# phylo42/IPK

Hardware: AMD Instinct MI355X
Metric: scored phylo-k-mers/sec (higher is better)
Workload: dtype f32

## Files before the change

ipk_amd/csrc/ipkgpu.hip:

```cpp
#include <cstring>
#include <hip/hip_runtime.h>
#include <rocprim/rocprim.hpp>

#include <algorithm>
#include <cmath>
#include <cstdarg>
#include <cstdio>
#include <cstring>
#include <new>
#include <string>
#include <type_traits>
#include <unordered_map>
#include <memory>
#include <vector>

#include "../../include/ipkgpu.h"
#include "dcla_device.hpp"
#include "kernels_score.hpp"
#include "kernels_quad.hpp"
#include "kernels_compact.hpp"
#include "kernels_keymajor.hpp"
#include "kernels_reduce_pipe.hpp"
#include "kernels_filter.hpp"
#include "kernels_dbfile.hpp"
// ... 393 lines not shown
    ctx->pend.sw.reset();
    for (hipEvent_t e : ctx->events.free_ev) (void)hipEventDestroy(e);
    ctx->events.free_ev.clear();
    if (ctx->h_rb) (void)hipHostFree(ctx->h_rb);
    if (ctx->up_done) (void)hipEventDestroy(ctx->up_done);
    (void)hipStreamDestroy(ctx->stream);
    delete ctx;
}

int ipkgpu_set_option(ipkgpu_ctx* ctx, const char* name, int64_t value)
{
    if (!ctx || !name) return IPKGPU_ERR_INVALID;
    if (!strcmp(name, "workspace_bytes")) {
        if (value <= 0) return fail(ctx, IPKGPU_ERR_INVALID, "workspace_bytes must be positive");
        ctx->workspace_bytes = value;
        return IPKGPU_OK;
    }
    if (!strcmp(name, "device_budget_bytes")) {
        if (value < 0) return fail(ctx, IPKGPU_ERR_INVALID, "device_budget_bytes must not be negative (0 = no budget)");
        ctx->budget = value;
        return IPKGPU_OK;
    }
    if (!strcmp(name, "release_workspaces")) {
        HIP_TRY(ctx, hipSetDevice(ctx->device));
        HIP_TRY(ctx, hipStreamSynchronize(ctx->stream));
        ctx->up_pending = false;
        for (DevBuf* b : all_workspaces(ctx)) if (b->p) { (void)dev_free(ctx, b->p, b->cap); b->p = nullptr; b->cap = 0; }
        drop_cache(ctx);
        ctx->mask_valid = false; ctx->pend.active = false; ctx->pend.sw.reset();
        return IPKGPU_OK;
    }
    if (!strcmp(name, "slice_long_lists")) {
        if (value != 0 && value != 1) return fail(ctx, IPKGPU_ERR_INVALID, "slice_long_lists is 0 or 1");
        ctx->opt_slice = value;
        return IPKGPU_OK;
    }
    if (!strcmp(name, "variant")) { ctx->opt_variant = value; return IPKGPU_OK; }
    if (!strcmp(name, "debug_flags")) { ctx->opt_flags = value; return IPKGPU_OK; }
    if (!strcmp(name, "debug_pool_chunks")) { ctx->opt_pool_chunks = value; return IPKGPU_OK; }
    if (!strcmp(name, "debug_pool_limit_bytes")) { ctx->opt_pool_limit = value; return IPKGPU_OK; }
    if (!strcmp(name, "debug_wg_chunks2")) { ctx->opt_wg_chunks2 = value; return IPKGPU_OK; }
    if (!strcmp(name, "debug_rounds")) { ctx->opt_rounds = value; return IPKGPU_OK; }
    if (!strcmp(name, "debug_kmc_pass")) { ctx->opt_kmc_pass = value; return IPKGPU_OK; }
    if (!strcmp(name, "debug_prefix_mats")) { ctx->opt_prefix_mats = value; return IPKGPU_OK; }
    return fail(ctx, IPKGPU_ERR_INVALID, "unknown option '%s'", name);
}

}

namespace {

constexpr int TW = 128;
constexpr int NW = 8;

#ifndef IPK_QCAP
#define IPK_QCAP 160
#endif
#ifndef IPK_AACAP
#define IPK_AACAP 512
#endif
#ifndef IPK_QCAP12
#define IPK_QCAP12 384
#endif
#ifndef IPK_QNW12
#define IPK_QNW12 4
#endif
#ifndef IPK_QTW12
#define IPK_QTW12 32
#endif
template <int SIGMA, int K> constexpr int fast_cap()
{
    if (SIGMA == 4) return K <= 10 ? IPK_QCAP : IPK_QCAP12;
    return IPK_AACAP;
}

template <int SIGMA, int K, bool POS = false>
int launch_score(ipkgpu_ctx* ctx, const ScoreParams& p)
{
    constexpr int CAP = fast_cap<SIGMA, K>();
    constexpr size_t lds = TileGeo<SIGMA, K, TW>::HEAD_BYTES + (size_t)NW * wave_scratch_entries<SIGMA, K, CAP>() * 8;
    static_assert(lds <= 160 * 1024, "fast-path LDS budget");
    auto kern = score_tiles_kernel<SIGMA, K, CAP, TW, NW, POS>;
    if (lds > 64 * 1024)
        HIP_TRY(ctx, hipFuncSetAttribute(reinterpret_cast<const void*>(kern), hipFuncAttributeMaxDynamicSharedMemorySize, (int)lds));
    const uint64_t blocks = (uint64_t)p.n_batch_mats * p.tiles_per_mat;
    if (blocks > 0x7fffffffull) return fail(ctx, IPKGPU_ERR_INVALID, "batch too large for one launch");
    hipLaunchKernelGGL(kern, dim3((uint32_t)blocks), dim3(NW * 64), lds, ctx->stream, p);
    HIP_TRY(ctx, hipGetLastError());
    return IPKGPU_OK;
}

template <int SIGMA, int K, bool POS = false>
int launch_overflow(ipkgpu_ctx* ctx, const ScoreParams& p)
{
    if constexpr (Geo<SIGMA, K, 1 << 30>::DIRECT || ipow(SIGMA, K - K / 2) <= (uint32_t)fast_cap<SIGMA, K>()) {
        (void)ctx; (void)p;
        return IPKGPU_OK;
    } else {
        constexpr size_t lds = TileGeo<SIGMA, K, 1>::HEAD_BYTES + (size_t)wave_scratch_entries<SIGMA, K, big_capf<SIGMA, K>()>() * 8;
        static_assert(lds <= 160 * 1024, "big-list LDS budget");
        auto kern = score_overflow_kernel<SIGMA, K, POS>;
        if (lds > 64 * 1024)
            HIP_TRY(ctx, hipFuncSetAttribute(reinterpret_cast<const void*>(kern), hipFuncAttributeMaxDynamicSharedMemorySize, (int)lds));
        const uint32_t per_cu = (uint32_t)std::max<size_t>(1, std::min<size_t>(32 / OVF_NW, (160 * 1024) / (lds + 64)));
        hipLaunchKernelGGL(kern, dim3(ctx->num_cu * per_cu), dim3(OVF_NW * 64), lds, ctx->stream, p);
        HIP_TRY(ctx, hipGetLastError());
        return IPKGPU_OK;
    }
}

template <int SIGMA, int K, bool POS>
int launch_both(ipkgpu_ctx* ctx, const ScoreParams& p)
{
    RC_TRY((launch_score<SIGMA, K, POS>(ctx, p)));
    return launch_overflow<SIGMA, K, POS>(ctx, p);
}


template <int SIGMA, int K> constexpr uint32_t stream_tbl()
{
    constexpr uint64_t T = ipow(SIGMA, K);
    if (Geo<SIGMA, K, 1 << 30>::DIRECT) return 0;
    if (SIGMA == 4 && K >= 13) return 0;
    if (SIGMA == 4) return T <= 16384 ? (uint32_t)T : (K <= 10 ? 16384u : 32768u);
    if (K <= 3) return (uint32_t)T;
    if (K <= 5) return 32000u;
    return 0;
}

template <int SIGMA, int K> constexpr int stream_nw() { return NW; }
template <int SIGMA, int K> constexpr int stream_tw() { return TW; }

template <int SIGMA, int K>
int launch_stream_pass1(ipkgpu_ctx* ctx, const StreamParams& sp, uint32_t n_wg)
{
    constexpr uint32_t TBL = stream_tbl<SIGMA, K>();
    if constexpr (TBL == 0) { (void)sp; (void)n_wg; return fail(ctx, IPKGPU_ERR_INVALID, "stream variant unsupported for this sigma/k"); }
    else {
        constexpr int CAP = fast_cap<SIGMA, K>();
        constexpr uint32_t T = ipow(SIGMA, K);
        constexpr uint32_t NB = (T + TBL - 1) / TBL;
        constexpr int SNW = stream_nw<SIGMA, K>(), STW = stream_tw<SIGMA, K>();
        constexpr size_t lds = TileGeo<SIGMA, K, STW>::HEAD_BYTES + (size_t)SNW * stream_wave_scratch<SIGMA, K, CAP>() * 8 + (size_t)SNW * 2 * NB * SUB * 4;
        static_assert(lds <= 160 * 1024, "stream pass-1 LDS budget");
        auto kern = score_stream_kernel<SIGMA, K, CAP, STW, SNW, TBL>;
        if (lds > 64 * 1024)
            HIP_TRY(ctx, hipFuncSetAttribute(reinterpret_cast<const void*>(kern), hipFuncAttributeMaxDynamicSharedMemorySize, (int)lds));
        hipLaunchKernelGGL(kern, dim3(n_wg), dim3(SNW * 64), lds, ctx->stream, sp);
        HIP_TRY(ctx, hipGetLastError());
        return IPKGPU_OK;
    }
}

template <int SIGMA, int K>
int launch_stream_overflow(ipkgpu_ctx* ctx, const StreamParams& sp)
{
    constexpr uint32_t TBL = stream_tbl<SIGMA, K>();
    if constexpr (TBL == 0 || ipow(SIGMA, K - K / 2) <= (uint32_t)fast_cap<SIGMA, K>()) {
        (void)ctx; (void)sp;
        return IPKGPU_OK;
    } else {
        constexpr uint32_t NB = (uint32_t)((ipow(SIGMA, K) + TBL - 1) / TBL);
        constexpr size_t lds = TileGeo<SIGMA, K, 1>::HEAD_BYTES + (size_t)wave_scratch_entries<SIGMA, K, big_capf<SIGMA, K>()>() * 8 +
                               (size_t)OVF_NW * 2 * NB * SUB * 4;
        static_assert(lds + 64 <= 160 * 1024, "big-list (stream) LDS budget");
        auto kern = score_overflow_stream_kernel<SIGMA, K, TBL>;
        if (lds > 64 * 1024)
            HIP_TRY(ctx, hipFuncSetAttribute(reinterpret_cast<const void*>(kern), hipFuncAttributeMaxDynamicSharedMemorySize, (int)lds));
        const uint32_t per_cu = (uint32_t)std::max<size_t>(1, std::min<size_t>(32 / OVF_NW, (160 * 1024) / (lds + 64)));
        hipLaunchKernelGGL(kern, dim3(ctx->num_cu * per_cu), dim3(OVF_NW * 64), lds, ctx->stream, sp);
        HIP_TRY(ctx, hipGetLastError());
        return IPKGPU_OK;
    }
}

#ifndef IPK_RPIPE_DEFAULT
#define IPK_RPIPE_DEFAULT 1
#endif
#ifndef IPK_RPIPE_D
#define IPK_RPIPE_D 2
#endif
template <int SIGMA, int K>
int launch_stream_pass2(ipkgpu_ctx* ctx, uint32_t n_gb, uint64_t T, uint32_t* table, bool compress)
{
    constexpr uint32_t TBL = stream_tbl<SIGMA, K>();
    if constexpr (TBL == 0) { (void)n_gb; (void)T; (void)table; (void)compress; return fail(ctx, IPKGPU_ERR_INVALID, "stream variant unsupported"); }
    else {
        constexpr uint32_t NB = (uint32_t)((ipow(SIGMA, K) + TBL - 1) / TBL);
        constexpr int NT = TBL <= 16384 ? 512 : 1024;
        const size_t lds = compress ? (size_t)comp_padded_slots<TBL, NT>() * 4 + (NT / 64 + 1) * 4 : (size_t)TBL * 4;
        auto launch = [&](auto kern) -> int {
            if (lds > 64 * 1024)
                HIP_TRY(ctx, hipFuncSetAttribute(reinterpret_cast<const void*>(kern), hipFuncAttributeMaxDynamicSharedMemorySize, (int)lds));
            hipLaunchKernelGGL(kern, dim3(n_gb), dim3(NT), lds, ctx->stream, ctx->pool.as<uint2>(),
                               ctx->gboff.as<uint64_t>(), ctx->clist.as<uint2>(), NB, T, table, ctx->mask.as<uint32_t>(), ctx->mask_words,
                               ctx->cvals.as<uint2>(), ctx->coff.as<uint64_t>(), ctx->rank.as<uint32_t>(), ctx->vaddr.as<uint64_t>(), ctx->ucnt.as<uint32_t>());
            HIP_TRY(ctx, hipGetLastError());
            return IPKGPU_OK;
        };
        if constexpr (TBL * 4 > 80 * 1024) {
            if (compress && ((IPK_RPIPE_DEFAULT != 0) != ((ctx->opt_flags & 2048) != 0))) {
                constexpr int PD = IPK_RPIPE_D;
                auto kern = reduce_buckets_pipe_kernel<TBL, NT, PD>;
                HIP_TRY(ctx, hipFuncSetAttribute(reinterpret_cast<const void*>(kern), hipFuncAttributeMaxDynamicSharedMemorySize, (int)lds));
                hipLaunchKernelGGL(kern, dim3(std::min<uint32_t>(n_gb, (uint32_t)ctx->num_cu)), dim3(NT), lds, ctx->stream, ctx->pool.as<uint2>(),
                                   ctx->gboff.as<uint64_t>(), ctx->clist.as<uint2>(), n_gb, NB, T, ctx->mask.as<uint32_t>(), ctx->mask_words,
                                   ctx->cvals.as<uint2>(), ctx->coff.as<uint64_t>(), ctx->rank.as<uint32_t>(), ctx->vaddr.as<uint64_t>(), ctx->ucnt.as<uint32_t>());
                HIP_TRY(ctx, hipGetLastError());
                return IPKGPU_OK;
            }
        }
        return compress ? launch(reduce_buckets_kernel<TBL, NT, true>) : launch(reduce_buckets_kernel<TBL, NT, false>);
    }
}

template <int SIGMA, int K> size_t stream_lds() {
    constexpr uint32_t TBL = stream_tbl<SIGMA, K>();
    if constexpr (TBL == 0) return 0;
    else {
        constexpr int CAP = fast_cap<SIGMA, K>();
        constexpr uint32_t NB = (uint32_t)((ipow(SIGMA, K) + TBL - 1) / TBL);
        return TileGeo<SIGMA, K, stream_tw<SIGMA, K>()>::HEAD_BYTES + (size_t)stream_nw<SIGMA, K>() * stream_wave_scratch<SIGMA, K, CAP>() * 8 +
               (size_t)stream_nw<SIGMA, K>() * 2 * NB * SUB * 4;
    }
}
template <int SIGMA, int K> uint32_t stream_nb() {
    constexpr uint32_t TBL = stream_tbl<SIGMA, K>();
    if constexpr (TBL == 0) return 0; else return (uint32_t)((ipow(SIGMA, K) + TBL - 1) / TBL);
}

template <int SIGMA, int K> constexpr bool quad_ok() { return QuadGeo<SIGMA, K>::OK && stream_tbl<SIGMA, K>() != 0; }
#ifndef IPK_QNW
#define IPK_QNW 4
#endif
#ifndef IPK_QTW
#define IPK_QTW 40
#endif
template <int SIGMA, int K> constexpr int quad_nw() { return K <= 10 ? IPK_QNW : IPK_QNW12; }
template <int SIGMA, int K> constexpr int quad_tw() { return K <= 10 ? IPK_QTW : IPK_QTW12; }
#ifndef IPK_QROWLANE12
#define IPK_QROWLANE12 1
#endif
#ifndef IPK_QROWLANE
#define IPK_QROWLANE 0
#endif
template <int SIGMA, int K> constexpr bool quad_rowlane() { return K <= 10 ? IPK_QROWLANE != 0 : IPK_QROWLANE12 != 0; }
#ifndef IPK_QONEWIN12
#define IPK_QONEWIN12 1
#endif
template <int SIGMA, int K> constexpr bool quad_onewin() { return K >= 11 && IPK_QONEWIN12 != 0 && quad_rowlane<SIGMA, K>(); }
template <int SIGMA, int K> size_t quad_lds()
{
    if constexpr (!quad_ok<SIGMA, K>()) return 0;
    else {
        constexpr int CAP = fast_cap<SIGMA, K>();
        constexpr uint32_t TBL = stream_tbl<SIGMA, K>();
        constexpr uint32_t NB = (uint32_t)((ipow(SIGMA, K) + TBL - 1) / TBL);
        return QuadTile<SIGMA, K, quad_tw<SIGMA, K>()>::HEAD_BYTES + (size_t)quad_nw<SIGMA, K>() * quad_wave_entries<SIGMA, K, CAP, quad_onewin<SIGMA, K>()>() * 8 +
               (size_t)quad_nw<SIGMA, K>() * NB * 8;
    }
}
template <int SIGMA, int K, bool COUNT_ONLY = false>
int launch_quad_pass1(ipkgpu_ctx* ctx, const StreamParams& sp, uint32_t n_wg)
{
    if constexpr (!quad_ok<SIGMA, K>()) { (void)sp; (void)n_wg; return fail(ctx, IPKGPU_ERR_INVALID, "quad kernel unsupported for this sigma/k"); }
    else {
        constexpr int CAP = fast_cap<SIGMA, K>();
        constexpr uint32_t TBL = stream_tbl<SIGMA, K>();
        constexpr int QNW = quad_nw<SIGMA, K>(), QTW = quad_tw<SIGMA, K>();
        const size_t lds = quad_lds<SIGMA, K>();
        auto kern = score_quad_kernel<SIGMA, K, CAP, QTW, QNW, TBL, COUNT_ONLY, quad_rowlane<SIGMA, K>(), quad_onewin<SIGMA, K>()>;
        if (lds > 64 * 1024)
            HIP_TRY(ctx, hipFuncSetAttribute(reinterpret_cast<const void*>(kern), hipFuncAttributeMaxDynamicSharedMemorySize, (int)lds));
        hipLaunchKernelGGL(kern, dim3(n_wg), dim3(QNW * 64), lds, ctx->stream, sp);
        HIP_TRY(ctx, hipGetLastError());
        return IPKGPU_OK;
    }
}

#ifndef IPK_XPNW
#define IPK_XPNW 11
#endif
#ifndef IPK_XPTW
#define IPK_XPTW 128
#endif
constexpr int XP_TW = IPK_XPTW;
template <int SIGMA, int K> constexpr int xp_nw() { return SIGMA == 20 ? IPK_XPNW : 11; }
template <int SIGMA, int K> constexpr uint32_t xp_tbl()
{
    if (SIGMA == 20 && K == 6) return 16000u;
    if (SIGMA == 4 && K >= 13) return 32768u;
    return stream_tbl<SIGMA, K>();
}
template <int SIGMA, int K, int KK = K> uint32_t xp_nb() {
    constexpr uint32_t TBL = xp_tbl<SIGMA, K>();
    if constexpr (TBL == 0) return 0; else return (uint32_t)((ipow(SIGMA, KK) + TBL - 1) / TBL);
}
template <int SIGMA, int K, int KK = K> size_t xp_lds() {
    constexpr uint32_t TBL = xp_tbl<SIGMA, K>();
    if constexpr (TBL == 0) return 0;
    else {
        constexpr int CAP = fast_cap<SIGMA, K>();
        constexpr uint32_t NB = (uint32_t)((ipow(SIGMA, KK) + TBL - 1) / TBL);
        return TileGeo<SIGMA, K, XP_TW>::HEAD_BYTES + (size_t)xp_nw<SIGMA, K>() * stream_wave_scratch<SIGMA, K, CAP>() * 8 + (size_t)NB * 4;
    }
}
template <int SIGMA, int K, bool WRITE, int KK = K, bool POS = false>
int launch_xp(ipkgpu_ctx* ctx, const XpParams& xp, uint32_t n_wg)
{
    constexpr uint32_t TBL = xp_tbl<SIGMA, K>();
    if constexpr (TBL == 0) { (void)xp; (void)n_wg; return fail(ctx, IPKGPU_ERR_INVALID, "exact-partition variant unsupported for this sigma/k"); }
    else {
        constexpr int CAP = fast_cap<SIGMA, K>();
        constexpr uint32_t NB = (uint32_t)((ipow(SIGMA, KK) + TBL - 1) / TBL);
        constexpr size_t lds = TileGeo<SIGMA, K, XP_TW>::HEAD_BYTES + (size_t)xp_nw<SIGMA, K>() * stream_wave_scratch<SIGMA, K, CAP>() * 8 + (size_t)NB * 4;
        static_assert(lds <= 160 * 1024, "exact-partition LDS budget");
        static_assert((TileGeo<SIGMA, K, XP_TW>::HEAD_BYTES + (size_t)xp_nw<SIGMA, K>() * stream_wave_scratch<SIGMA, K, CAP>() * 8) % 8 == 0, "cursor alignment");
        auto kern = score_xp_kernel<SIGMA, K, CAP, XP_TW, xp_nw<SIGMA, K>(), TBL, WRITE, KK, POS>;
        if (lds > 64 * 1024)
            HIP_TRY(ctx, hipFuncSetAttribute(reinterpret_cast<const void*>(kern), hipFuncAttributeMaxDynamicSharedMemorySize, (int)lds));
        hipLaunchKernelGGL(kern, dim3(n_wg), dim3(xp_nw<SIGMA, K>() * 64), lds, ctx->stream, xp);
        HIP_TRY(ctx, hipGetLastError());
        return IPKGPU_OK;
    }
}
template <int SIGMA, int K, bool WRITE, int KK = K, bool POS = false>
int launch_xp_overflow(ipkgpu_ctx* ctx, const XpParams& xp)
{
    constexpr uint32_t TBL = xp_tbl<SIGMA, K>();
    if constexpr (TBL == 0 || ipow(SIGMA, K - K / 2) <= (uint32_t)fast_cap<SIGMA, K>()) {
        (void)ctx; (void)xp;
        return IPKGPU_OK;
    } else {
        constexpr size_t lds = TileGeo<SIGMA, K, 1>::HEAD_BYTES + (size_t)wave_scratch_entries<SIGMA, K, big_capf<SIGMA, K>()>() * 8;
        static_assert(lds + 64 <= 160 * 1024, "big-list (exact partition) LDS budget");
        auto kern = score_overflow_xp_kernel<SIGMA, K, TBL, WRITE, KK, POS>;
        if (lds > 64 * 1024)
            HIP_TRY(ctx, hipFuncSetAttribute(reinterpret_cast<const void*>(kern), hipFuncAttributeMaxDynamicSharedMemorySize, (int)lds));
        const uint32_t per_cu = (uint32_t)std::max<size_t>(1, std::min<size_t>(32 / OVF_NW, (160 * 1024) / (lds + 64)));
        hipLaunchKernelGGL(kern, dim3(ctx->num_cu * per_cu), dim3(OVF_NW * 64), lds, ctx->stream, xp);
        HIP_TRY(ctx, hipGetLastError());
        return IPKGPU_OK;
    }
}
template <int SIGMA, int K, bool COMPRESS, int KK = K>
int launch_xp_reduce(ipkgpu_ctx* ctx, uint32_t n_gb, uint32_t S, uint64_t T, const uint64_t* off, uint32_t* table)
{
    constexpr uint32_t TBL = xp_tbl<SIGMA, K>();
    if constexpr (TBL == 0) { (void)n_gb; (void)S; (void)T; (void)off; (void)table; return fail(ctx, IPKGPU_ERR_INVALID, "exact-partition variant unsupported"); }
    else {
        constexpr uint32_t NB = (uint32_t)((ipow(SIGMA, KK) + TBL - 1) / TBL);
        static_assert(!COMPRESS || NB == 1 || TBL % 64 == 0, "a 64-slot block must not straddle two buckets");
        constexpr int NT = TBL <= 16384 ? 512 : 1024;
        constexpr size_t lds = COMPRESS ? (size_t)comp_padded_slots<TBL, NT>() * 4 + (NT / 64 + 1) * 4 : (size_t)TBL * 4;
        auto kern = reduce_ranges_kernel<TBL, NT, COMPRESS>;
        if (lds > 64 * 1024)
            HIP_TRY(ctx, hipFuncSetAttribute(reinterpret_cast<const void*>(kern), hipFuncAttributeMaxDynamicSharedMemorySize, (int)lds));
        hipLaunchKernelGGL(kern, dim3(n_gb), dim3(NT), lds, ctx->stream, ctx->pool.as<uint2>(), off, S, NB, T, table,
                           ctx->mask.as<uint32_t>(), ctx->mask_words, ctx->rank.as<uint32_t>(), ctx->vaddr.as<uint64_t>(), ctx->ucnt.as<uint32_t>());
        HIP_TRY(ctx, hipGetLastError());
        return IPKGPU_OK;
    }
}
template <int SIGMA, int K>
int launch_xp_reduce_pos(ipkgpu_ctx* ctx, uint32_t n_gb, uint32_t S, uint64_t T, const uint64_t* off, uint32_t nwin)
{
    constexpr uint32_t TBL = xp_tbl<SIGMA, K>();
    if constexpr (TBL == 0) { (void)n_gb; (void)S; (void)T; (void)off; (void)nwin; return fail(ctx, IPKGPU_ERR_INVALID, "exact-partition variant unsupported"); }
    else {
        constexpr uint32_t NB = (uint32_t)((ipow(SIGMA, K) + TBL - 1) / TBL);
        static_assert(NB == 1 || TBL % 64 == 0, "a 64-slot block must not straddle two buckets");
        constexpr int NT = pos_sub_slots<TBL>() <= 4096 ? 256 : 1024;
        constexpr size_t lds = (size_t)pos_sub_blocks<TBL>() * 64 * 8 + (pos_sub_blocks<TBL>() + 1) * 4;
        static_assert(lds <= 160 * 1024, "positions reduce LDS budget");
        auto kern = reduce_ranges_pos_kernel<TBL, NT>;
        if (lds > 64 * 1024)
            HIP_TRY(ctx, hipFuncSetAttribute(reinterpret_cast<const void*>(kern), hipFuncAttributeMaxDynamicSharedMemorySize, (int)lds));
        hipLaunchKernelGGL(kern, dim3(n_gb), dim3(NT), lds, ctx->stream, ctx->pool.as<uint2>(), ctx->seq.as<uint32_t>(), off, S, NB, T, nwin,
                           ctx->mask_words, ctx->pvals.as<uint32_t>(), ctx->pvaddr.as<uint64_t>());
        HIP_TRY(ctx, hipGetLastError());
        return IPKGPU_OK;
    }
}
template <int V> using int_c = std::integral_constant<int, V>;

template <int SIGMA, int K, int KMAX, class F> int with_k(ipkgpu_ctx* ctx, uint32_t k, F& f)
{
    if (k == (uint32_t)K) return f(int_c<SIGMA>{}, int_c<K>{});
    if constexpr (K < KMAX) return with_k<SIGMA, K + 1, KMAX>(ctx, k, f);
    else return fail(ctx, IPKGPU_ERR_INVALID, "unsupported sigma/k (%u/%u)", (uint32_t)SIGMA, k);
}
template <class F> int with_sigma_k(ipkgpu_ctx* ctx, uint32_t sigma, uint32_t k, F&& f)
{
    if (sigma == 4) return with_k<4, 2, 14>(ctx, k, f);
    if (sigma == 20) return with_k<20, 2, 6>(ctx, k, f);
    return fail(ctx, IPKGPU_ERR_INVALID, "unsupported sigma/k (%u/%u)", sigma, k);
}

bool keyrange_supported(uint32_t sigma, uint32_t k, uint32_t lead)
{
    return sigma == 4 && lead >= 1 && k > lead && k - lead >= 13 && k - lead <= 14 && k <= 16;
}
template <class F> int with_xp_shape(ipkgpu_ctx* ctx, uint32_t sigma, uint32_t k, uint32_t lead, F&& f)
{
    if (!lead) return with_sigma_k(ctx, sigma, k, [&](auto S_, auto K_) { return f(S_, K_, K_); });
    if (sigma == 4) {
        switch (k * 8 + lead) {
            case 14 * 8 + 1: return f(int_c<4>{}, int_c<14>{}, int_c<13>{});
            case 15 * 8 + 1: return f(int_c<4>{}, int_c<15>{}, int_c<14>{});
            case 15 * 8 + 2: return f(int_c<4>{}, int_c<15>{}, int_c<13>{});
            case 16 * 8 + 2: return f(int_c<4>{}, int_c<16>{}, int_c<14>{});
            case 16 * 8 + 3: return f(int_c<4>{}, int_c<16>{}, int_c<13>{});
        }
    }
    return fail(ctx, IPKGPU_ERR_INVALID, "unsupported key range");
}

struct Geometry {
    uint32_t fast_cap = 0;
    uint32_t stream_nb = 0, stream_tbl = 0;
    uint32_t stream_nw = NW, stream_tw = TW;
    size_t stream_lds = 0;
    bool quad = false;
    uint32_t quad_nw = NW, quad_tw = TW;
    size_t quad_lds = 0;
    uint32_t xp_nb = 0, xp_tbl = 0;
    size_t xp_lds = 0;
};

int fill_geometry(ipkgpu_ctx* ctx, uint32_t sigma, uint32_t k, uint32_t lead, Geometry& g)
{
    if (!lead)
        RC_TRY(with_sigma_k(ctx, sigma, k, [&](auto S_, auto K_) {
            g.fast_cap = fast_cap<S_, K_>();
            g.stream_nb = stream_nb<S_, K_>(); g.stream_tbl = stream_tbl<S_, K_>();
            g.stream_nw = stream_nw<S_, K_>(); g.stream_tw = stream_tw<S_, K_>(); g.stream_lds = stream_lds<S_, K_>();
            g.quad = quad_ok<S_, K_>();
            g.quad_nw = quad_nw<S_, K_>(); g.quad_tw = quad_tw<S_, K_>(); g.quad_lds = quad_lds<S_, K_>();
            return IPKGPU_OK;
        }));
    return with_xp_shape(ctx, sigma, k, lead, [&](auto S_, auto K_, auto KK_) {
        g.xp_nb = xp_nb<S_, K_, KK_>(); g.xp_tbl = xp_tbl<S_, K_>(); g.xp_lds = xp_lds<S_, K_, KK_>();
        return IPKGPU_OK;
    });
}

#ifndef IPK_KMC_RUNS_DEFAULT
#define IPK_KMC_RUNS_DEFAULT 1
#endif
#ifndef IPK_KMC_PASS
#define IPK_KMC_PASS 256
#endif
#define KM_LAUNCH(KERN, CAPV, ...)                                                                                        \
    do {                                                                                                                  \
        if (P == 1) hipLaunchKernelGGL((KERN<true, CAPV>), dim3((uint32_t)(per_xcd * 8)), dim3(256), 0, ctx->stream, __VA_ARGS__); \
        else hipLaunchKernelGGL((KERN<false, CAPV>), dim3((uint32_t)(per_xcd * 8)), dim3(256), 0, ctx->stream, __VA_ARGS__);     \
    } while (0)

CompTable comp_table(const ipkgpu_ctx* ctx)
{
    CompTable ct;
    ct.mask = ctx->mask.as<uint32_t>(); ct.rank = ctx->rank.as<uint32_t>(); ct.vaddr = ctx->vaddr.as<uint64_t>();
    ct.pool = ctx->comp_own_vals ? ctx->cvals.as<uint2>() : ctx->pool.as<uint2>();
    ct.off = ctx->comp_own_vals ? ctx->coff.as<uint64_t>() : ctx->gboff.as<uint64_t>(); ct.mask_words = ctx->mask_words;
    ct.NB = ctx->comp_nb; ct.stride = ctx->comp_stride; ct.TBL = ctx->comp_tbl;
    return ct;
}

}

namespace {

constexpr int IPKGPU_RETRY_SMALLER = 100;
constexpr int IPKGPU_RETRY_AGAIN = 101;
#ifndef IPK_OVF_POOL_RATIO
#define IPK_OVF_POOL_RATIO 500
#endif

enum class PassKind { tiles, stream, quad, xp };
struct Pass {
    PassKind kind = PassKind::tiles;
    bool positions = false;
    bool compress = false;
    bool seq = false;
    double slot_bytes() const { return positions ? 8.0 : kind == PassKind::xp && compress ? 0.3125 : 4.0; }
};

Pass choose_pass(int64_t variant, uint32_t sigma, uint32_t lead, bool positions, bool km_positions, const Geometry& g)
{
    Pass ps;
    ps.positions = positions;
    if (positions) return ps;
    if (km_positions) { ps.kind = PassKind::xp; ps.compress = true; ps.seq = true; return ps; }
    const int64_t v = variant;
    if (g.xp_nb != 0 && (v == 3 || v == 4 || (v == 0 && g.stream_nb == 0) || lead != 0)) {
        ps.kind = PassKind::xp;
        ps.compress = v != 3;
    } else if (g.stream_nb != 0 && g.stream_nb <= 2048 && (v == 0 || v == 2 || v == 5 || v == 6 || v == 7)) {
        ps.kind = v != 2 && g.quad ? PassKind::quad : PassKind::stream;
        ps.compress = v == 6 || (v == 0 && g.stream_tbl == 32768u && sigma == 4);
    }
    return ps;
}

struct Plan {
    uint32_t n_mats = 0, sites = 0, sigma = 0, k = 0;
    float eps = 0;
    std::vector<uint32_t> group_ids;
    std::vector<uint32_t> slot_of;
    uint32_t n_groups = 0, nwin = 0, tiles_per_mat = 0, chunks_per_group = 0;
    uint64_t table_size = 0, gpb = 1;
    uint32_t lead = 0, lead_c = 0;
    Geometry geo;
    Pass pass;
    const uint32_t* mat_rank = nullptr;
};

int make_plan(ipkgpu_ctx* ctx, const void* logp, uint32_t n_mats, uint32_t sites, uint32_t sigma,
              const uint32_t* mat_group, uint32_t k, float log_eps, Plan& pl, uint32_t lead = 0, uint32_t lead_c = 0,
              bool positions = false, bool km_positions = false)
{
    if (!logp || !mat_group) return fail(ctx, IPKGPU_ERR_INVALID, "null input pointer");
    if (sigma != 4 && sigma != 20) return fail(ctx, IPKGPU_ERR_INVALID, "unsupported alphabet size %u (4 or 20)", sigma);
    if (lead == 0 && (k < 2 || k > ipkgpu_max_k(sigma)))
        return fail(ctx, IPKGPU_ERR_INVALID, "k=%u out of range [2, %u] for sigma=%u", k, ipkgpu_max_k(sigma), sigma);
    if (lead != 0 && !keyrange_supported(sigma, k, lead))
        return fail(ctx, IPKGPU_ERR_INVALID, "no key-range pass of k=%u with %u leading symbols for sigma=%u", k, lead, sigma);
    pl.lead = lead; pl.lead_c = lead_c;
    if (n_mats == 0) return fail(ctx, IPKGPU_ERR_INVALID, "no matrices");
    if (sites < k) return fail(ctx, IPKGPU_ERR_INVALID, "alignment has %u sites, fewer than k=%u", sites, k);
    pl.n_mats = n_mats; pl.sites = sites; pl.sigma = sigma; pl.k = k; pl.eps = log_eps;
    RC_TRY(fill_geometry(ctx, sigma, k, lead, pl.geo));
    if (km_positions && (lead != 0 || pl.geo.xp_nb == 0))
        return fail(ctx, IPKGPU_ERR_INVALID, "no positioned database for sigma=%u k=%u: the call takes the exact partition, which needs more than 64 keys "
                                             "and no key-range pass", sigma, k);
    pl.pass = choose_pass(ctx->opt_variant, sigma, lead, positions, km_positions, pl.geo);
    pl.slot_of.resize(n_mats);
    std::unordered_map<uint32_t, uint32_t> index;
    index.reserve(n_mats);
    for (uint32_t i = 0; i < n_mats; ++i) {
        auto it = index.find(mat_group[i]);
        if (it == index.end()) {
            it = index.emplace(mat_group[i], (uint32_t)pl.group_ids.size()).first;
            pl.group_ids.push_back(mat_group[i]);
        }
        pl.slot_of[i] = it->second;
    }
    pl.n_groups = (uint32_t)pl.group_ids.size();
    pl.table_size = ipow(sigma, (int)(k - lead));
    pl.chunks_per_group = (uint32_t)((pl.table_size + CHUNK - 1) / CHUNK);
    pl.nwin = sites - k + 1;
    {
        const double ppw = ctx->pairs_per_window > 0 ? ctx->pairs_per_window : 256.0;
        const double pool_per_group = (double)n_mats / (double)pl.n_groups * (double)pl.nwin * ppw * (pl.pass.seq ? 16.0 : 8.0) * 1.25;
        const double per_group = (double)pl.table_size * pl.pass.slot_bytes() + pool_per_group;
        pl.gpb = std::max<uint64_t>(1, (uint64_t)((double)ctx->workspace_bytes / per_group));
    }
    pl.gpb = std::min<uint64_t>(pl.gpb, pl.n_groups);
    while (pl.gpb > 1 && pl.gpb * pl.chunks_per_group > 0x7fffffffull) pl.gpb /= 2;
    pl.tiles_per_mat = (pl.nwin + TW - 1) / TW;
    return IPKGPU_OK;
}

int run_prefix(ipkgpu_ctx* ctx, const Plan& pl, const float* logp_dev)
{
    RC_TRY(ensure(ctx, ctx->best, (size_t)pl.n_mats * (pl.sites + 1) * 4));
    HIP_TRY(ctx, hipMemsetAsync(ctx->small, 0, SMALL_BYTES, ctx->stream));
    uint32_t M = 1;
    while (M < 8 && (pl.n_mats + M - 1) / M > (uint32_t)ctx->num_cu * 4) M *= 2;
    if (ctx->opt_prefix_mats == 1 || ctx->opt_prefix_mats == 2 || ctx->opt_prefix_mats == 4 || ctx->opt_prefix_mats == 8) M = (uint32_t)ctx->opt_prefix_mats;
    const dim3 grid((pl.n_mats + M - 1) / M);
#define IPK_PREFIX(SG, MM) hipLaunchKernelGGL((prefix_max_kernel<SG, MM>), grid, dim3(256), 0, ctx->stream, logp_dev, pl.n_mats, pl.sites, ctx->best.as<float>())
    if (pl.sigma == 4) { if (M == 1) IPK_PREFIX(4, 1); else if (M == 2) IPK_PREFIX(4, 2); else if (M == 4) IPK_PREFIX(4, 4); else IPK_PREFIX(4, 8); }
    else { if (M == 1) IPK_PREFIX(20, 1); else if (M == 2) IPK_PREFIX(20, 2); else if (M == 4) IPK_PREFIX(20, 4); else IPK_PREFIX(20, 8); }
#undef IPK_PREFIX
    HIP_TRY(ctx, hipGetLastError());
    return IPKGPU_OK;
}

int scan_u32(ipkgpu_ctx* ctx, const uint32_t* in, uint64_t n, uint64_t* out);

int score_batch_xp(ipkgpu_ctx* ctx, const Plan& pl, const float* logp_dev, uint32_t gb, ScoreParams& p)
{
    const uint32_t XNB = pl.geo.xp_nb;
    const bool compress = pl.pass.compress;
    const uint32_t tiles_per_mat = (pl.nwin + XP_TW - 1) / XP_TW;
    const size_t lds_bytes = pl.geo.xp_lds;
    const uint64_t wg_per_cu = std::max<uint64_t>(1, std::min<uint64_t>(32 / (pl.sigma == 20 ? IPK_XPNW : 11), (160 * 1024) / std::max<size_t>(lds_bytes, 1)));
    const uint64_t slots = (uint64_t)ctx->num_cu * wg_per_cu;
    const uint32_t S = (uint32_t)std::max<uint64_t>(1, std::min<uint64_t>((slots * 4) / gb, tiles_per_mat));
    const uint64_t n_gb = (uint64_t)gb * XNB;
    const uint32_t stride = S + 1;
    const uint64_t n_units = n_gb * stride;
    if (n_gb > 0x7fffffffull || (uint64_t)gb * S > 0x7fffffffull) return fail(ctx, IPKGPU_ERR_INVALID, "batch too large for one launch");
    RC_TRY(ensure(ctx, ctx->gbcnt, n_units * 4));
    RC_TRY(ensure(ctx, ctx->gboff, (n_units + 1) * 8));
    RC_TRY(ensure(ctx, ctx->gbcur, n_gb * 4));
    HIP_TRY(ctx, hipMemsetAsync(ctx->gbcnt.p, 0, n_units * 4, ctx->stream));
    HIP_TRY(ctx, hipMemsetAsync(ctx->gbcur.p, 0, n_gb * 4, ctx->stream));

    XpParams xp;
    StreamParams& sp = xp.s;
    sp.logp = logp_dev; sp.best = ctx->best.as<float>();
    sp.gm_off = ctx->gm.as<uint32_t>(); sp.gm_list = ctx->gm.as<uint32_t>() + gb + 1;
    sp.sites = pl.sites; sp.nwin = pl.nwin; sp.tiles_per_mat = tiles_per_mat; sp.S = S;
    sp.eps = pl.eps;
    sp.pool = nullptr; sp.pool_cap = 0; sp.pool_next = nullptr; sp.desc = nullptr; sp.pool_ovf = nullptr; sp.pre_chunks = 0;
    sp.emitted = p.emitted; sp.ovf_queue = p.ovf_queue; sp.ovf_count = p.ovf_count; sp.mat_slot = p.mat_slot; sp.big_ovf = p.big_ovf;
    sp.slice_lists = p.slice_lists;
    sp.flags = (uint32_t)(ctx->opt_flags) & 4u;
    xp.cnt = ctx->gbcnt.as<uint32_t>();
    xp.off = ctx->gboff.as<uint64_t>();
    xp.stride = stride;
    xp.ovcur = ctx->gbcur.as<uint32_t>();
    xp.start = nullptr;
    xp.lead_c = pl.lead_c;

    const bool seq = pl.pass.seq;
    auto xp_kernel = [&](bool write) {
        if (write && seq)
            return with_sigma_k(ctx, pl.sigma, pl.k, [&](auto S_, auto K_) { return launch_xp<S_, K_, true, K_, true>(ctx, xp, gb * S); });
        return with_xp_shape(ctx, pl.sigma, pl.k, pl.lead, [&](auto S_, auto K_, auto KK_) {
            return write ? launch_xp<S_, K_, true, KK_>(ctx, xp, gb * S) : launch_xp<S_, K_, false, KK_>(ctx, xp, gb * S);
        });
    };
    auto xp_overflow = [&](bool write) {
        if (write && seq)
            return with_sigma_k(ctx, pl.sigma, pl.k, [&](auto S_, auto K_) { return launch_xp_overflow<S_, K_, true, K_, true>(ctx, xp); });
        return with_xp_shape(ctx, pl.sigma, pl.k, pl.lead, [&](auto S_, auto K_, auto KK_) {
            return write ? launch_xp_overflow<S_, K_, true, KK_>(ctx, xp) : launch_xp_overflow<S_, K_, false, KK_>(ctx, xp);
        });
    };
    Stopwatch sw(ctx->stream, &ctx->events);
    const int ev_a = sw.mark();
    RC_TRY(xp_kernel(false));
    const int ev_a2 = sw.mark();
    RC_TRY(xp_overflow(false));
    RC_TRY(scan_u32(ctx, xp.cnt, n_units, ctx->gboff.as<uint64_t>()));
    uint64_t total = 0;
    HIP_TRY(ctx, hipMemcpyAsync(&total, ctx->gboff.as<uint64_t>() + n_units, 8, hipMemcpyDeviceToHost, ctx->stream));
    HIP_TRY(ctx, hipStreamSynchronize(ctx->stream));
    {
        const size_t free_b = mem_free_bytes(ctx);
        const bool over_limit = ctx->opt_pool_limit > 0 && total * 8 > (uint64_t)ctx->opt_pool_limit;
        const uint64_t side = seq ? total * 8 + 512 : 0;
        const uint64_t side_have = seq ? ctx->seq.cap + ctx->pvals.cap : 0;
        if (over_limit || (total * 8 > ctx->pool.cap && total * 8 > free_b + ctx->pool.cap) ||
            (side > side_have && total * 8 + side > free_b + ctx->pool.cap + side_have)) {
            if (gb > 1) return IPKGPU_RETRY_SMALLER;
            return fail(ctx, IPKGPU_ERR_NOMEM, "the pair pool of ONE branch group (%llu pairs) does not fit device memory", (unsigned long long)total);
        }
    }
// ... 47 lines not shown
    ctx->acc_main_ms += sw.ms(ev_a, ev_a2) + sw.ms(ev_c, ev_d0);
    ctx->acc_count_ms += sw.ms(ev_a, ev_a2); ctx->acc_write_ms += sw.ms(ev_c, ev_d0);
    ctx->acc_reduce_ms += sw.ms(ev_d, ev_e);
    ctx->main_kernel = "score_xp_kernel";
    return IPKGPU_OK;
}

int stream_batch_check(ipkgpu_ctx* ctx)
{
    ipkgpu_ctx::Pending& pd = ctx->pend;
    if (!pd.active) return IPKGPU_OK;
    pd.active = false;
    std::unique_ptr<Stopwatch> sw(pd.sw.release());
    const uint32_t n_ovf = ctx->h_rb[SMALL_OVF_COUNT / 4], pool_exhausted = ctx->h_rb[SMALL_POOL_OVF / 4];
    if (pool_exhausted) {
        if (pd.cap >= pd.max_chunks) {
            ctx->pool_want_min = 0;
            if (pd.gb > 1) return IPKGPU_RETRY_SMALLER;
            return fail(ctx, IPKGPU_ERR_NOMEM, "the pair pool of ONE branch group is exhausted at the device-memory limit");
        }
        ctx->pool_want_min = pd.cap * 2;
        return IPKGPU_RETRY_AGAIN;
    }
    ctx->pool_want_min = 0;
    memcpy(&ctx->emitted_host, ctx->h_rb + SMALL_EMITTED / 4, 8);
    ctx->emitted_fetched = true;
    ctx->spec_skip_wait = !(n_ovf > 0 && (uint64_t)n_ovf * IPK_OVF_POOL_RATIO >= pd.windows && pd.pool_ovf_ok);
    if (sw) { ctx->acc_main_ms += sw->ms(pd.ev_a, pd.ev_b); ctx->acc_reduce_ms += sw->ms(pd.ev_c, pd.ev_d); }
    return IPKGPU_OK;
}

int arm_capped(ipkgpu_ctx* ctx, uint32_t sigma, uint32_t k, ScoreParams& p)
{
    static_assert(SMALL_SLICED + 4 == SMALL_BIG_OVF, "the count and the flag are cleared and read together");
    const bool capped_lists = sigma == 4 && k >= 13;
    p.big_ovf = capped_lists ? small_at(ctx, SMALL_BIG_OVF) : nullptr;
    p.slice_lists = capped_lists && ctx->opt_slice ? 1u : 0u;
    if (capped_lists) HIP_TRY(ctx, hipMemsetAsync(p.big_ovf - 1, 0, 8, ctx->stream));
    return IPKGPU_OK;
}

int check_capped(ipkgpu_ctx* ctx, uint32_t k, const ScoreParams& p)
{
    if (!p.big_ovf) return IPKGPU_OK;
    uint32_t word[2] = {0, 0};
    HIP_TRY(ctx, hipMemcpyAsync(word, p.big_ovf - 1, 8, hipMemcpyDeviceToHost, ctx->stream));
    HIP_TRY(ctx, hipStreamSynchronize(ctx->stream));
    ctx->sliced_windows += word[0];
    const uint32_t hit = word[1];
    if (hit) return fail(ctx, IPKGPU_ERR_INVALID, "a window's half list exceeds %d entries: beyond the capacity of this engine at k = %u "
                                                  "(the lists of k >= 13 are capped; lower omega's reach or k)", BIG_CAP_ENTRIES, k);
    return IPKGPU_OK;
}

int score_batch_impl(ipkgpu_ctx* ctx, const Plan& pl, const float* logp_dev, uint32_t g0, uint32_t gb, bool defer)
{
    const uint32_t n_mats = pl.n_mats;
    uint32_t nb = 0;
    for (uint32_t i = 0; i < n_mats; ++i) nb += (pl.slot_of[i] >= g0 && pl.slot_of[i] < g0 + gb);
    const size_t gm_words = (size_t)gb + 1 + nb;
    void* stage = nullptr;
    RC_TRY(upload_stage(ctx, ((size_t)n_mats * 2 + gm_words) * 4, &stage));
    uint32_t* mat_list_h = reinterpret_cast<uint32_t*>(stage);
    uint32_t* mat_slot_h = mat_list_h + n_mats;
    uint32_t* gm = mat_slot_h + n_mats;
    nb = 0;
    for (uint32_t i = 0; i < n_mats; ++i) {
        mat_slot_h[i] = 0;
        if (pl.slot_of[i] >= g0 && pl.slot_of[i] < g0 + gb) { mat_list_h[nb++] = i; mat_slot_h[i] = pl.slot_of[i] - g0; }
    }
    for (uint32_t i = nb; i < n_mats; ++i) mat_list_h[i] = 0;
    for (size_t i = 0; i < gm_words; ++i) gm[i] = 0;
    for (uint32_t i = 0; i < n_mats; ++i)
        if (pl.slot_of[i] >= g0 && pl.slot_of[i] < g0 + gb) gm[pl.slot_of[i] - g0 + 1]++;
    for (uint32_t g = 0; g < gb; ++g) gm[g + 1] += gm[g];
    {
        std::vector<uint32_t> cur(gm, gm + gb);
        for (uint32_t i = 0; i < n_mats; ++i)
            if (pl.slot_of[i] >= g0 && pl.slot_of[i] < g0 + gb) gm[(size_t)gb + 1 + cur[pl.slot_of[i] - g0]++] = i;
    }
    RC_TRY(ensure(ctx, ctx->idx, (size_t)n_mats * 8));
    RC_TRY(ensure(ctx, ctx->ovfq, (size_t)nb * pl.nwin * 8));
    RC_TRY(ensure(ctx, ctx->gm, gm_words * 4));
    HIP_TRY(ctx, hipMemcpyAsync(ctx->idx.p, mat_list_h, (size_t)n_mats * 8, hipMemcpyHostToDevice, ctx->stream));
    HIP_TRY(ctx, hipMemcpyAsync(ctx->gm.p, gm, gm_words * 4, hipMemcpyHostToDevice, ctx->stream));
    RC_TRY(upload_staged(ctx));

    const Pass& ps = pl.pass;
    ScoreParams p;
    p.logp = logp_dev;
    p.best = ctx->best.as<float>();
    p.mat_list = ctx->idx.as<uint32_t>();
    p.mat_slot = ctx->idx.as<uint32_t>() + n_mats;
    p.n_batch_mats = nb; p.sites = pl.sites; p.nwin = pl.nwin; p.tiles_per_mat = pl.tiles_per_mat;
    p.eps = pl.eps;
    p.table = ctx->table.p;
    p.mat_rank = pl.mat_rank;
    p.table_size = pl.table_size;
    p.emitted = small_at<unsigned long long>(ctx, SMALL_EMITTED);
    p.ovf_queue = ctx->ovfq.as<unsigned long long>();
    p.ovf_count = small_at(ctx, SMALL_OVF_COUNT);
    p.flags = (uint32_t)(!ps.positions && ctx->opt_variant == 99 ? 1 : 0);
    p.mask = nullptr; p.mask_words = 0;
    RC_TRY(arm_capped(ctx, pl.sigma, pl.k, p));
    ctx->mask_valid = false;
    ctx->table_compressed = false;
    ctx->comp_own_vals = false;
    const bool use_stream = ps.kind == PassKind::stream || ps.kind == PassKind::quad;
    const bool use_quad = ps.kind == PassKind::quad;
    if (!use_stream) {
        HIP_TRY(ctx, hipMemsetAsync(p.emitted, 0, 8, ctx->stream));
        HIP_TRY(ctx, hipMemsetAsync(p.ovf_count, 0, 4, ctx->stream));
    }
    if (ps.kind == PassKind::tiles) {
        const size_t table_bytes = (size_t)gb * pl.table_size * (ps.positions ? 8 : 4);
        RC_TRY(ensure(ctx, ctx->table, table_bytes));
        p.table = ctx->table.p;
        HIP_TRY(ctx, hipMemsetAsync(ctx->table.p, 0, table_bytes, ctx->stream));
        Stopwatch sw(ctx->stream, &ctx->events);
        const int a = sw.mark();
        RC_TRY(with_sigma_k(ctx, pl.sigma, pl.k, [&](auto S_, auto K_) {
            if (ps.positions) return launch_both<S_, K_, true>(ctx, p);
            if constexpr (S_ == 4 && K_ > 12) return fail(ctx, IPKGPU_ERR_INVALID, "unsupported sigma/k (%u/%u)", pl.sigma, pl.k);
            else return launch_both<S_, K_, false>(ctx, p);
        }));
        const int b = sw.mark();
        HIP_TRY(ctx, hipStreamSynchronize(ctx->stream));
        ctx->acc_main_ms += sw.ms(a, b);
        ctx->main_kernel = "score_tiles_kernel";
        return check_capped(ctx, pl.k, p);
    }

    ctx->mask_words = 2 * ((pl.table_size + 63) / 64);
    RC_TRY(ensure(ctx, ctx->mask, (size_t)gb * ctx->mask_words * 4));
    p.mask = ctx->mask.as<uint32_t>(); p.mask_words = ctx->mask_words;
    if (ps.kind == PassKind::xp) {
        if (!ps.compress) {
            RC_TRY(ensure(ctx, ctx->table, (size_t)gb * pl.table_size * 4));
            p.table = ctx->table.p;
        }
        const int rc = score_batch_xp(ctx, pl, logp_dev, gb, p);
        return rc ? rc : check_capped(ctx, pl.k, p);
    }

    const bool pool_ovf_ok = gb < (1u << 22) && n_mats < (1u << 21) && pl.nwin < (1u << 21);
    bool s_compress = pool_ovf_ok && ps.compress;
    const uint32_t NBK = pl.geo.stream_nb, TBL = pl.geo.stream_tbl;
    const uint32_t SNW = use_quad ? pl.geo.quad_nw : pl.geo.stream_nw;
    const uint32_t STW = use_quad ? pl.geo.quad_tw : pl.geo.stream_tw;
    const uint32_t s_tiles_per_mat = (pl.nwin + STW - 1) / STW;
    auto pass1 = [&](const StreamParams& sp, uint32_t n_wg, bool count_only) {
        return with_sigma_k(ctx, pl.sigma, pl.k, [&](auto S_, auto K_) {
            if (!use_quad) return launch_stream_pass1<S_, K_>(ctx, sp, n_wg);
            return count_only ? launch_quad_pass1<S_, K_, true>(ctx, sp, n_wg) : launch_quad_pass1<S_, K_, false>(ctx, sp, n_wg);
        });
    };

    const uint64_t windows = (uint64_t)nb * pl.nwin;
    if (ctx->pairs_per_window <= 0) {
        const uint32_t n_s = std::min<uint32_t>(gb, std::max<uint32_t>(2, gb / 64));
        const uint32_t stride_g = gb / n_s;
        std::vector<uint32_t> sgm((size_t)n_s + 1, 0), slist;
        for (uint32_t j = 0; j < n_s; ++j) {
            const uint32_t g = j * stride_g;
            for (uint32_t m = gm[g]; m < gm[g + 1]; ++m) slist.push_back(gm[(size_t)gb + 1 + m]);
            sgm[j + 1] = (uint32_t)slist.size();
        }
        std::vector<uint32_t> both(sgm);
        both.insert(both.end(), slist.begin(), slist.end());
        RC_TRY(ensure(ctx, ctx->tmp_a, both.size() * 4));
        HIP_TRY(ctx, hipMemcpyAsync(ctx->tmp_a.p, both.data(), both.size() * 4, hipMemcpyHostToDevice, ctx->stream));
        HIP_TRY(ctx, hipMemsetAsync(p.emitted, 0, 8, ctx->stream));
        HIP_TRY(ctx, hipMemsetAsync(p.ovf_count, 0, 4, ctx->stream));
        StreamParams ss;
        ss.logp = logp_dev; ss.best = ctx->best.as<float>();
        ss.gm_off = ctx->tmp_a.as<uint32_t>(); ss.gm_list = ctx->tmp_a.as<uint32_t>() + n_s + 1;
        ss.sites = pl.sites; ss.nwin = pl.nwin; ss.tiles_per_mat = s_tiles_per_mat;
        ss.S = (uint32_t)std::max<uint64_t>(1, std::min<uint64_t>(s_tiles_per_mat, (uint64_t)ctx->num_cu * 4 / n_s));
        ss.eps = pl.eps;
        ss.pool = nullptr; ss.pool_cap = 0; ss.pool_next = nullptr; ss.desc = nullptr; ss.pool_ovf = nullptr; ss.pre_chunks = 0;
        ss.emitted = p.emitted; ss.ovf_queue = p.ovf_queue; ss.ovf_count = p.ovf_count; ss.mat_slot = p.mat_slot;
        ss.flags = 2u;
        RC_TRY(pass1(ss, n_s * ss.S, true));
        unsigned long long se = 0; uint32_t so = 0;
        HIP_TRY(ctx, hipMemcpyAsync(&se, p.emitted, 8, hipMemcpyDeviceToHost, ctx->stream));
        HIP_TRY(ctx, hipMemcpyAsync(&so, p.ovf_count, 4, hipMemcpyDeviceToHost, ctx->stream));
        HIP_TRY(ctx, hipStreamSynchronize(ctx->stream));
        const uint64_t s_windows = (uint64_t)slist.size() * pl.nwin;
        const double cap_pairs = 0.25 * (double)pl.geo.fast_cap * (double)pl.geo.fast_cap;
        if (s_windows) ctx->pairs_per_window = std::max(1.0, ((double)se + (double)so * cap_pairs) / (double)s_windows * 1.15);
    }
    const double ppw_est = ctx->pairs_per_window > 0 ? ctx->pairs_per_window : 256.0;
    if (!s_compress && pool_ovf_ok && ctx->opt_variant == 0 && pl.table_size >= (1u << 16) &&
        (double)windows * ppw_est < 0.5 * (double)gb * (double)pl.table_size)
        s_compress = true;
    if (!s_compress) {
        RC_TRY(ensure(ctx, ctx->table, (size_t)gb * pl.table_size * 4));
        p.table = ctx->table.p;
    }
    const size_t lds_bytes = use_quad ? pl.geo.quad_lds : pl.geo.stream_lds;
    const uint64_t wg_per_cu = std::max<uint64_t>(1, std::min<uint64_t>(32 / SNW, (160 * 1024) / std::max<size_t>(lds_bytes, 1)));
    const uint64_t slots = (uint64_t)ctx->num_cu * wg_per_cu;
    const uint32_t CH = chunk_pairs_rt(TBL);
    const uint64_t expected_chunks = (uint64_t)((double)windows * ppw_est / CH);
#ifndef IPK_WG_CHUNKS2
#define IPK_WG_CHUNKS2 2
#endif
    const uint64_t wg_chunks2 = ctx->opt_wg_chunks2 > 0 ? (uint64_t)ctx->opt_wg_chunks2 : (uint64_t)IPK_WG_CHUNKS2;
    const uint64_t max_wg = std::max<uint64_t>(slots, expected_chunks * 2 / wg_chunks2 / ((uint64_t)SNW * NBK * SUB));
#ifndef IPK_ROUNDS
#define IPK_ROUNDS 8
#endif
    const uint64_t rounds = std::max<uint64_t>(1, std::min<uint64_t>(ctx->opt_rounds > 0 ? (uint64_t)ctx->opt_rounds : (uint64_t)IPK_ROUNDS, max_wg / slots));
    uint64_t S64 = std::max<uint64_t>(1, (slots * rounds) / gb);
    uint32_t S = (uint32_t)std::max<uint64_t>(1, std::min<uint64_t>(S64, s_tiles_per_mat));
    const uint32_t n_wg = gb * S;
    const uint64_t n_waves = (uint64_t)n_wg * SNW;
    const uint64_t n_gb = (uint64_t)gb * NBK;

    const size_t free_b = mem_free_bytes(ctx);
    uint64_t max_chunks = std::min<uint64_t>(0xFFFFFFF0ull, (uint64_t)(free_b + ctx->pool.cap + ctx->desc.cap) * 9 / 10 / (CH * 8 + 8));
    if (ctx->opt_pool_limit > 0) max_chunks = std::min<uint64_t>(max_chunks, (uint64_t)ctx->opt_pool_limit / (CH * 8 + 8));
    const double ppw = ctx->pairs_per_window > 0 ? ctx->pairs_per_window : 256.0;
    const uint64_t ovf_waves = (uint64_t)ctx->num_cu * 4 * OVF_NW;
    const uint64_t slack = 2 * (n_waves + ovf_waves) * NBK * SUB + (n_waves + ovf_waves) * ALLOC_BATCH + 1024;
    uint64_t want = (uint64_t)((double)windows * ppw * 1.25 / CH) + slack;
    {
        const uint64_t have = std::min<uint64_t>(std::max<uint64_t>(ctx->pool.cap / (CH * 8), 1) - 1, ctx->desc.cap / 8);
        const uint64_t need = (uint64_t)((double)windows * ppw * 1.1 / CH) + (n_waves + ovf_waves) * (NBK * SUB + ALLOC_BATCH) + 1024;
        if (have >= need) want = have;
    }
    want = std::max<uint64_t>(want, ctx->pool_want_min);
    for (int attempt = 0; attempt < 6; ++attempt) {
        uint64_t cap = std::min<uint64_t>(want, max_chunks);
        const bool forced = attempt == 0 && ctx->opt_pool_chunks > 0 && ctx->pool_want_min == 0;
        if (forced) cap = (uint64_t)ctx->opt_pool_chunks;
        else if (cap < n_waves * NBK * SUB) {
            if (gb > 1) return IPKGPU_RETRY_SMALLER;
            return fail(ctx, IPKGPU_ERR_NOMEM, "the pair pool of ONE branch group does not fit device memory");
        }
        RC_TRY(ensure(ctx, ctx->pool, (cap + 1) * CH * 8));
        RC_TRY(ensure(ctx, ctx->desc, cap * 8));
        if (!forced) cap = std::min<uint64_t>(ctx->pool.cap / (CH * 8) - 1, ctx->desc.cap / 8);
        RC_TRY(ensure(ctx, ctx->gbcnt, 2 * n_gb * 4));
        uint32_t* const d_gbcur = ctx->gbcnt.as<uint32_t>() + n_gb;
        RC_TRY(ensure(ctx, ctx->gboff, (n_gb + 1) * 8));
        uint32_t* d_pool_next = small_at(ctx, SMALL_POOL_NEXT);
        uint32_t* d_pool_ovf = small_at(ctx, SMALL_POOL_OVF);
        const bool pre_ok = use_quad && n_waves * NBK + 1024 <= cap && !(ctx->opt_flags & 32);
        const uint32_t pre_chunks = pre_ok ? (uint32_t)(n_waves * NBK) : 0u;
        uint32_t* d_tile_next = nullptr;
        if (use_quad && !(ctx->opt_flags & 128) && ((uint64_t)nb * s_tiles_per_mat >= 4ull * gb * S || (ctx->opt_flags & 256))) {
            RC_TRY(ensure(ctx, ctx->tile_next, (size_t)gb * 4));
            d_tile_next = ctx->tile_next.as<uint32_t>();
        }
        hipLaunchKernelGGL(small_reset_kernel, dim3((std::max<uint32_t>(gb, SMALL_XP_TOO_BIG / 4) + 255) / 256), dim3(256), 0, ctx->stream,
                           reinterpret_cast<uint32_t*>(ctx->small), pre_chunks, d_tile_next, gb, S);
        HIP_TRY(ctx, hipGetLastError());
        HIP_TRY(ctx, hipMemsetAsync(ctx->desc.p, 0, cap * 8, ctx->stream));

        StreamParams sp;
        sp.logp = logp_dev; sp.best = ctx->best.as<float>();
        sp.gm_off = ctx->gm.as<uint32_t>(); sp.gm_list = ctx->gm.as<uint32_t>() + gb + 1;
        sp.sites = pl.sites; sp.nwin = pl.nwin; sp.tiles_per_mat = s_tiles_per_mat; sp.S = S;
        sp.eps = pl.eps;
        sp.pool = ctx->pool.as<uint2>(); sp.pool_cap = (uint32_t)cap; sp.pool_next = d_pool_next;
        sp.desc = ctx->desc.as<unsigned long long>(); sp.pool_ovf = d_pool_ovf;
        sp.emitted = p.emitted; sp.ovf_queue = p.ovf_queue; sp.ovf_count = p.ovf_count; sp.mat_slot = p.mat_slot;
        sp.flags = (uint32_t)(ctx->opt_flags);
        sp.pre_chunks = pre_chunks;
        sp.tile_next = d_tile_next;
        std::unique_ptr<Stopwatch> sw_own(new Stopwatch(ctx->stream, &ctx->events));
        Stopwatch& sw = *sw_own;
        const int ev_a = sw.mark();
        RC_TRY(pass1(sp, n_wg, false));
        const int ev_b = sw.mark();
        const bool spec = ctx->spec_skip_wait && !s_compress && !(ctx->opt_flags & 64);
        uint32_t n_ovf = 0;
        uint32_t h[2] = {0, 0};
        if (!spec) {
            HIP_TRY(ctx, hipMemcpyAsync(ctx->h_rb, ctx->small, SMALL_BYTES, hipMemcpyDeviceToHost, ctx->stream));
            HIP_TRY(ctx, hipStreamSynchronize(ctx->stream));
            n_ovf = ctx->h_rb[SMALL_OVF_COUNT / 4]; h[0] = ctx->h_rb[SMALL_POOL_NEXT / 4]; h[1] = ctx->h_rb[SMALL_POOL_OVF / 4];
        }
        const bool ovf_in_pool = n_ovf > 0 && ((uint64_t)n_ovf * IPK_OVF_POOL_RATIO >= windows || s_compress) && pool_ovf_ok;
        if (ovf_in_pool) {
            RC_TRY(ensure(ctx, ctx->tmp_a, (size_t)n_ovf * 8));
            RC_TRY(ensure(ctx, ctx->tmp_b, (size_t)n_ovf * 8));
            hipLaunchKernelGGL(ovf_group_keys_kernel, dim3((n_ovf + 255) / 256), dim3(256), 0, ctx->stream,
                               p.ovf_queue, n_ovf, p.mat_slot, ctx->tmp_a.as<unsigned long long>());
            HIP_TRY(ctx, hipGetLastError());
            size_t tmp_bytes = 0;
            HIP_TRY(ctx, rocprim::radix_sort_keys(nullptr, tmp_bytes, ctx->tmp_a.as<unsigned long long>(), ctx->tmp_b.as<unsigned long long>(),
                                                  (size_t)n_ovf, 0, 64, ctx->stream));
            RC_TRY(ensure(ctx, ctx->tmp_c, tmp_bytes));
            HIP_TRY(ctx, rocprim::radix_sort_keys(ctx->tmp_c.p, tmp_bytes, ctx->tmp_a.as<unsigned long long>(), ctx->tmp_b.as<unsigned long long>(),
                                                  (size_t)n_ovf, 0, 64, ctx->stream));
            StreamParams so = sp;
            so.ovf_queue = ctx->tmp_b.as<unsigned long long>();
            if (use_quad) so.emitted = small_at<unsigned long long>(ctx, SMALL_OVF_EMITTED);
            RC_TRY(with_sigma_k(ctx, pl.sigma, pl.k, [&](auto S_, auto K_) { return launch_stream_overflow<S_, K_>(ctx, so); }));
        }
        if (ovf_in_pool) {
            HIP_TRY(ctx, hipMemcpyAsync(ctx->h_rb, ctx->small, SMALL_BYTES, hipMemcpyDeviceToHost, ctx->stream));
            HIP_TRY(ctx, hipStreamSynchronize(ctx->stream));
            h[0] = ctx->h_rb[SMALL_POOL_NEXT / 4]; h[1] = ctx->h_rb[SMALL_POOL_OVF / 4];
        }
        if (h[1] != 0) {
            if (cap >= max_chunks) {
                if (gb > 1) return IPKGPU_RETRY_SMALLER;
                return fail(ctx, IPKGPU_ERR_NOMEM, "the pair pool of ONE branch group is exhausted at the device-memory limit");
            }
            want = std::max<uint64_t>(cap * 2, want);
            continue;
        }
        const uint32_t n_used = spec ? (uint32_t)cap : (uint32_t)std::min<uint64_t>(h[0], cap);
        const uint32_t* n_used_dev = spec ? d_pool_next : nullptr;
        HIP_TRY(ctx, hipMemsetAsync(ctx->gbcnt.p, 0, 2 * n_gb * 4, ctx->stream));
        RC_TRY(ensure(ctx, ctx->clist, ((uint64_t)n_used + 16) * 8));
        if (s_compress) {
            RC_TRY(ensure(ctx, ctx->croom, 2 * n_gb * 4));
            HIP_TRY(ctx, hipMemsetAsync(ctx->croom.p, 0, n_gb * 4, ctx->stream));
        }
        if (n_used) {
            hipLaunchKernelGGL(chunk_hist_kernel, dim3(std::min<uint32_t>((n_used + 255) / 256, 2048u)), dim3(256), 0, ctx->stream,
                               ctx->desc.as<unsigned long long>(), n_used, ctx->gbcnt.as<uint32_t>(),
                               use_quad ? p.emitted : (unsigned long long*)nullptr, s_compress ? ctx->croom.as<uint32_t>() : (uint32_t*)nullptr,
                               n_used_dev);
            HIP_TRY(ctx, hipGetLastError());
        }
        RC_TRY(scan_u32(ctx, ctx->gbcnt.as<uint32_t>(), n_gb, ctx->gboff.as<uint64_t>()));
        if (s_compress) {
            hipLaunchKernelGGL(comp_slice_room_kernel, dim3((uint32_t)((n_gb + 255) / 256)), dim3(256), 0, ctx->stream,
                               ctx->croom.as<uint32_t>(), (uint32_t)n_gb, NBK, pl.table_size, TBL, ctx->croom.as<uint32_t>() + n_gb);
            HIP_TRY(ctx, hipGetLastError());
            RC_TRY(ensure(ctx, ctx->coff, (n_gb + 1) * 8));
            RC_TRY(scan_u32(ctx, ctx->croom.as<uint32_t>() + n_gb, n_gb, ctx->coff.as<uint64_t>()));
            const uint64_t max_vals = std::min<uint64_t>((uint64_t)n_used * CH, (uint64_t)gb * pl.table_size);
            RC_TRY(ensure(ctx, ctx->cvals, (max_vals / 2 + n_gb + 1) * 8 + 256));
            RC_TRY(ensure(ctx, ctx->rank, (size_t)gb * (ctx->mask_words / 2) * 4));
            RC_TRY(ensure(ctx, ctx->vaddr, (size_t)gb * (ctx->mask_words / 2) * 8));
            RC_TRY(ensure(ctx, ctx->ucnt, n_gb * 4));
        }
        if (n_used) {
            const uint64_t n_grid = spec ? std::min<uint64_t>(n_used, expected_chunks * 2 + n_waves * NBK + 4096) : n_used;
            hipLaunchKernelGGL(chunk_scatter_kernel, dim3((uint32_t)std::min<uint64_t>((n_grid + 255) / 256, 1u << 16)), dim3(256), 0, ctx->stream,
                               ctx->desc.as<unsigned long long>(), n_used, ctx->gboff.as<uint64_t>(), d_gbcur,
                               ctx->clist.as<uint2>(), n_used_dev);
            HIP_TRY(ctx, hipGetLastError());
        }
        const int ev_c = sw.mark();
        RC_TRY(with_sigma_k(ctx, pl.sigma, pl.k, [&](auto S_, auto K_) {
            return launch_stream_pass2<S_, K_>(ctx, (uint32_t)n_gb, pl.table_size, ctx->table.as<uint32_t>(), s_compress);
        }));
        const int ev_d = sw.mark();
        if ((spec || n_ovf > 0) && !ovf_in_pool)
            RC_TRY(with_sigma_k(ctx, pl.sigma, pl.k, [&](auto S_, auto K_) { return launch_overflow<S_, K_, false>(ctx, p); }));
        if (s_compress) {
            ctx->table_compressed = true; ctx->comp_own_vals = true;
            ctx->comp_nb = NBK; ctx->comp_stride = 1; ctx->comp_tbl = TBL;
        }
        ctx->mask_valid = true;
        ctx->main_kernel = use_quad ? "score_quad_kernel" : "score_stream_kernel";
        HIP_TRY(ctx, hipMemcpyAsync(ctx->h_rb, ctx->small, SMALL_BYTES, hipMemcpyDeviceToHost, ctx->stream));
        ipkgpu_ctx::Pending& pd = ctx->pend;
        pd.sw.reset(sw_own.release());
        pd.ev_a = ev_a; pd.ev_b = ev_b; pd.ev_c = ev_c; pd.ev_d = ev_d;
        pd.cap = cap; pd.max_chunks = max_chunks; pd.windows = windows; pd.gb = gb; pd.pool_ovf_ok = pool_ovf_ok; pd.use_quad = use_quad;
        pd.active = true;
        if (defer) return IPKGPU_OK;
        HIP_TRY(ctx, hipStreamSynchronize(ctx->stream));
        const int rcf = stream_batch_check(ctx);
        if (rcf == IPKGPU_RETRY_AGAIN) { want = std::max<uint64_t>(want, ctx->pool_want_min); continue; }
        return rcf;
    }
    return fail(ctx, IPKGPU_ERR_NOMEM, "pair pool could not be sized");
}

int score_batch_finish(ipkgpu_ctx* ctx, const Plan& pl, uint32_t g0, uint32_t gb, uint64_t* emitted_acc)
{
    if (ctx->pend.active) RC_TRY(stream_batch_check(ctx));
    unsigned long long e = ctx->emitted_host;
    if (!ctx->emitted_fetched) {
        HIP_TRY(ctx, hipMemcpyAsync(ctx->h_rb, small_at(ctx, SMALL_EMITTED), 8, hipMemcpyDeviceToHost, ctx->stream));
        HIP_TRY(ctx, hipStreamSynchronize(ctx->stream));
        memcpy(&e, ctx->h_rb, 8);
    }
    *emitted_acc += e;
    if (pl.pass.positions) return IPKGPU_OK;
    uint64_t nb = 0;
    for (uint32_t i = 0; i < pl.n_mats; ++i) nb += (pl.slot_of[i] >= g0 && pl.slot_of[i] < g0 + gb);
    if (nb) ctx->pairs_per_window = (double)e / ((double)nb * pl.nwin);
    return IPKGPU_OK;
}

int score_batch(ipkgpu_ctx* ctx, const Plan& pl, const float* logp_dev, uint32_t g0, uint32_t gb, uint64_t* emitted_acc, bool defer = false)
{
    ctx->emitted_fetched = false;
    ctx->pend.active = false; ctx->pend.sw.reset();
    RC_TRY(score_batch_impl(ctx, pl, logp_dev, g0, gb, defer));
    if (ctx->pend.active) return IPKGPU_OK;
    return score_batch_finish(ctx, pl, g0, gb, emitted_acc);
}

#if defined(__HIP_DEVICE_COMPILE__)
#define IPK_GLOBAL_U32(p) ((ipkgpu::global_u32_ptr)(p))
#else
#define IPK_GLOBAL_U32(p) (p)
#endif
struct ScanU32In {
    const uint32_t* in; uint64_t n;
    __host__ __device__ uint64_t operator()(uint64_t i) const { return i < n ? (uint64_t)IPK_GLOBAL_U32(in)[i] : 0ull; }
};
struct ScanNonzeroIn {
    const uint32_t* in; uint64_t n;
    __host__ __device__ uint64_t operator()(uint64_t i) const { return i < n ? (uint64_t)(IPK_GLOBAL_U32(in)[i] != 0u) : 0ull; }
};
int scan_nonzero_u32(ipkgpu_ctx* ctx, const uint32_t* in, uint64_t n, uint64_t* out)
{
    if (n == 0) { HIP_TRY(ctx, hipMemsetAsync(out, 0, 8, ctx->stream)); return IPKGPU_OK; }
    auto it = rocprim::make_transform_iterator(rocprim::make_counting_iterator<uint64_t>(0), ScanNonzeroIn{in, n});
    size_t bytes = 0;
    HIP_TRY(ctx, rocprim::exclusive_scan(nullptr, bytes, it, out, (uint64_t)0, (size_t)(n + 1), rocprim::plus<uint64_t>(), ctx->stream));
    RC_TRY(ensure(ctx, ctx->scan_sums, bytes));
    HIP_TRY(ctx, rocprim::exclusive_scan(ctx->scan_sums.p, bytes, it, out, (uint64_t)0, (size_t)(n + 1), rocprim::plus<uint64_t>(), ctx->stream));
    return IPKGPU_OK;
}
struct ScanRowsIn {
    const uint32_t* const* rows; uint64_t slots, n;
    __host__ __device__ uint64_t operator()(uint64_t i) const
    {
#if defined(__HIP_DEVICE_COMPILE__)
        typedef const uint32_t* const __attribute__((address_space(1)))* rows_ptr;
        return i < n ? (uint64_t)IPK_GLOBAL_U32(((rows_ptr)rows)[i / slots])[i % slots] : 0ull;
#else
        return i < n ? (uint64_t)rows[i / slots][i % slots] : 0ull;
#endif
    }
};
int scan_rows_u32(ipkgpu_ctx* ctx, const uint32_t* const* rows, uint32_t S, uint64_t slots, uint64_t* out)
{
    const uint64_t n = (uint64_t)S * slots;
    if (n == 0) { HIP_TRY(ctx, hipMemsetAsync(out, 0, 8, ctx->stream)); return IPKGPU_OK; }
    auto it = rocprim::make_transform_iterator(rocprim::make_counting_iterator<uint64_t>(0), ScanRowsIn{rows, slots, n});
    size_t bytes = 0;
    HIP_TRY(ctx, rocprim::exclusive_scan(nullptr, bytes, it, out, (uint64_t)0, (size_t)(n + 1), rocprim::plus<uint64_t>(), ctx->stream));
    RC_TRY(ensure(ctx, ctx->scan_sums, bytes));
    HIP_TRY(ctx, rocprim::exclusive_scan(ctx->scan_sums.p, bytes, it, out, (uint64_t)0, (size_t)(n + 1), rocprim::plus<uint64_t>(), ctx->stream));
    return IPKGPU_OK;
}
int scan_u32(ipkgpu_ctx* ctx, const uint32_t* in, uint64_t n, uint64_t* out)
{
    if (n == 0) { HIP_TRY(ctx, hipMemsetAsync(out, 0, 8, ctx->stream)); return IPKGPU_OK; }
    auto it = rocprim::make_transform_iterator(rocprim::make_counting_iterator<uint64_t>(0), ScanU32In{in, n});
    size_t bytes = 0;
    HIP_TRY(ctx, rocprim::exclusive_scan(nullptr, bytes, it, out, (uint64_t)0, (size_t)(n + 1), rocprim::plus<uint64_t>(), ctx->stream));
    RC_TRY(ensure(ctx, ctx->scan_sums, bytes));
    HIP_TRY(ctx, rocprim::exclusive_scan(ctx->scan_sums.p, bytes, it, out, (uint64_t)0, (size_t)(n + 1), rocprim::plus<uint64_t>(), ctx->stream));
    return IPKGPU_OK;
}

int group_major(ipkgpu_ctx* ctx, const float* logp_dev, uint32_t n_mats, uint32_t sites, uint32_t sigma, const uint32_t* mat_group,
                uint32_t k, float log_eps, bool positions, ipkgpu_result** out)
{
    if (!ctx) return IPKGPU_ERR_INVALID;
    if (!out) return fail(ctx, IPKGPU_ERR_INVALID, "null out pointer");
    *out = nullptr;
    Plan pl;
    RC_TRY(make_plan(ctx, logp_dev, n_mats, sites, sigma, mat_group, k, log_eps, pl, 0, 0, positions));
    HIP_TRY(ctx, hipSetDevice(ctx->device));
    const uint32_t n_groups = pl.n_groups, cpg = pl.chunks_per_group;
    if (positions) {
        if ((uint64_t)n_mats * pl.nwin >= 0xFFFFFFFFull) return fail(ctx, IPKGPU_ERR_INVALID, "too many windows per group for the position code");
        std::vector<uint32_t> rank(n_mats), seen(n_groups, 0);
        for (uint32_t i = 0; i < n_mats; ++i) rank[i] = seen[pl.slot_of[i]]++;
        RC_TRY(ensure(ctx, ctx->branch, (size_t)n_mats * 4));
        HIP_TRY(ctx, hipMemcpy(ctx->branch.p, rank.data(), (size_t)n_mats * 4, hipMemcpyHostToDevice));
        pl.mat_rank = ctx->branch.as<uint32_t>();
    }

    ipkgpu_result* res = new (std::nothrow) ipkgpu_result();
    if (!res) return fail(ctx, IPKGPU_ERR_NOMEM, "out of host memory");
    res->ctx = ctx;
    res->group_ids = pl.group_ids;
    res->offsets.assign((size_t)n_groups + 1, 0);
    struct Guard { ipkgpu_result* r; ~Guard() { if (r) ipkgpu_result_free(r); } } guard{res};
    void** const arrays[3] = {(void**)&res->d_keys, (void**)&res->d_scores, (void**)&res->d_positions};
    const int n_arrays = positions ? 3 : 2;

    RC_TRY(ensure(ctx, ctx->counts, (size_t)(pl.gpb * cpg) * 4));
    RC_TRY(ensure(ctx, ctx->offsets, (size_t)(pl.gpb * cpg + 1) * 8));
    RC_TRY(ensure(ctx, ctx->goff, (size_t)(pl.gpb + 1) * 8));

    ctx->acc_main_ms = ctx->acc_reduce_ms = ctx->acc_count_ms = ctx->acc_write_ms = ctx->acc_km_ms = 0;
    Stopwatch sw(ctx->stream, &ctx->events);
    const int t_begin = sw.mark();
    RC_TRY(run_prefix(ctx, pl, logp_dev));
    const int t_pre = sw.mark();
    std::vector<std::pair<int, int>> ev_score, ev_compact;
    uint64_t total_entries = 0;
    uint32_t gpb_now = (uint32_t)pl.gpb, gb = 0;
    for (uint32_t g0 = 0; g0 < n_groups; g0 += gb) {
        gb = std::min<uint32_t>(gpb_now, n_groups - g0);
        const int s0 = sw.mark();
        const int rcb = score_batch(ctx, pl, logp_dev, g0, gb, &res->emitted);
        if (rcb == IPKGPU_RETRY_SMALLER) { gpb_now = std::max<uint32_t>(1, gb / 2); gb = 0; continue; }
// ... 1066 lines not shown
    double t_dev = 0, t_file = 0;
    auto since = [](std::chrono::steady_clock::time_point t0) { return std::chrono::duration<double>(std::chrono::steady_clock::now() - t0).count(); };
    FileOut out;
    out.f = fopen(path, "wb");
    if (!out.f) return fail(ctx, IPKGPU_ERR_INVALID, "cannot create %s", path);
    setvbuf(out.f, nullptr, _IONBF, 0);
    const uint64_t n = db->n_keys;
    const std::vector<uint8_t> head = ipkfmt::file_head(h->sequence_type, h->tree_index_size, h->tree_num_nodes, h->tree_subtree_length, h->newick,
                                                        h->kmer_size, h->omega, n, db->n_entries, positioned);
    uint64_t total = head.size();
    { const auto t0 = std::chrono::steady_clock::now(); if (!out.put(head.data(), head.size())) return fail(ctx, IPKGPU_ERR_INVALID, "write failed"); t_file += since(t0); }
    if (n) {
        RC_TRY(ensure(ctx, ctx->tmp_a, n * 4));
        RC_TRY(ensure(ctx, ctx->tmp_b, (n + 1) * 8));
        const auto t0 = std::chrono::steady_clock::now();
        uint32_t* d_big = small_at(ctx, SMALL_REC_BIG);
        HIP_TRY(ctx, hipMemsetAsync(d_big, 0, 4, ctx->stream));
        hipLaunchKernelGGL(db_record_sizes_kernel, dim3((uint32_t)((n + 255) / 256)), dim3(256), 0, ctx->stream, db->d_order, db->d_key_off, n,
                           ctx->tmp_a.as<uint32_t>(), d_big, positioned);
        HIP_TRY(ctx, hipGetLastError());
        RC_TRY(scan_u32(ctx, ctx->tmp_a.as<uint32_t>(), n, ctx->tmp_b.as<uint64_t>()));
        std::vector<uint64_t> rec_off(n + 1);
        uint32_t h_big = 0;
        HIP_TRY(ctx, hipMemcpyAsync(rec_off.data(), ctx->tmp_b.p, (n + 1) * 8, hipMemcpyDeviceToHost, ctx->stream));
        HIP_TRY(ctx, hipMemcpyAsync(&h_big, d_big, 4, hipMemcpyDeviceToHost, ctx->stream));
        HIP_TRY(ctx, hipStreamSynchronize(ctx->stream));
        if (h_big) return fail(ctx, IPKGPU_ERR_INVALID, "a k-mer with 2^28 entries or more: record sizes are 32-bit");
        t_dev += since(t0);
        uint64_t max_rec = 0;
        for (uint64_t i = 0; i < n; ++i) max_rec = std::max(max_rec, rec_off[i + 1] - rec_off[i]);
        const uint64_t PIECE = std::max<uint64_t>((uint64_t)256 << 20, max_rec);
        void* d_stage[2] = {nullptr, nullptr};
        void* h_stage[2] = {nullptr, nullptr};
        hipEvent_t ev[2] = {nullptr, nullptr};
        struct Cleanup { ipkgpu_ctx* c; void** d; void** h; hipEvent_t* e;
            ~Cleanup() { for (int i = 0; i < 2; ++i) { ctx_release(c, d[i]); if (h[i]) (void)hipHostFree(h[i]); if (e[i]) (void)hipEventDestroy(e[i]); } } } cleanup{ctx, d_stage, h_stage, ev};
        const uint64_t body = rec_off[n];
        const uint64_t stage_bytes = std::min<uint64_t>(PIECE, body);
        for (int i = 0; i < 2; ++i) {
            HIP_TRY(ctx, ctx_alloc(ctx, &d_stage[i], std::max<uint64_t>(stage_bytes, 16)));
            HIP_TRY(ctx, hipHostMalloc(&h_stage[i], std::max<uint64_t>(stage_bytes, 16), hipHostMallocDefault));
            HIP_TRY(ctx, hipEventCreate(&ev[i]));
        }
        struct Piece { uint64_t lo, hi; };
        std::vector<Piece> pieces;
        for (uint64_t lo = 0; lo < n;) {
            const uint64_t hi = (uint64_t)(std::upper_bound(rec_off.begin() + lo, rec_off.end(), rec_off[lo] + PIECE) - rec_off.begin()) - 1;
            pieces.push_back({lo, std::max(hi, lo + 1)});
            lo = pieces.back().hi;
        }
        auto launch = [&](size_t j) -> int {
            const Piece pc = pieces[j];
            const int b = (int)(j & 1);
            if (positioned)
                hipLaunchKernelGGL(db_pack_positions_kernel, dim3((uint32_t)((pc.hi - pc.lo + 3) / 4)), dim3(256), 0, ctx->stream, db->d_order, db->d_keys,
                                   db->d_key_off, db->d_entries, db->d_positions, db->d_fv32, ctx->tmp_b.as<uint64_t>(), pc.lo, pc.hi, (unsigned char*)d_stage[b]);
            else
                hipLaunchKernelGGL(db_pack_kernel, dim3((uint32_t)((pc.hi - pc.lo + 3) / 4)), dim3(256), 0, ctx->stream, db->d_order, db->d_keys, db->d_key_off,
                                   db->d_entries, db->d_fv32, ctx->tmp_b.as<uint64_t>(), pc.lo, pc.hi, (unsigned char*)d_stage[b]);
            HIP_TRY(ctx, hipGetLastError());
            HIP_TRY(ctx, hipMemcpyAsync(h_stage[b], d_stage[b], rec_off[pc.hi] - rec_off[pc.lo], hipMemcpyDeviceToHost, ctx->stream));
            HIP_TRY(ctx, hipEventRecord(ev[b], ctx->stream));
            return IPKGPU_OK;
        };
        if (!pieces.empty()) RC_TRY(launch(0));
        for (size_t j = 0; j < pieces.size(); ++j) {
            if (j + 1 < pieces.size()) RC_TRY(launch(j + 1));
            const auto tw = std::chrono::steady_clock::now();
            HIP_TRY(ctx, hipEventSynchronize(ev[j & 1]));
            t_dev += since(tw);
            const auto tf = std::chrono::steady_clock::now();
            const uint64_t nb = rec_off[pieces[j].hi] - rec_off[pieces[j].lo];
            if (!out.put(h_stage[j & 1], nb)) return fail(ctx, IPKGPU_ERR_INVALID, "write failed");
            t_file += since(tf);
            total += nb;
        }
    }
    { const auto t0 = std::chrono::steady_clock::now(); const int rc = fclose(out.f); out.f = nullptr; if (rc != 0) return fail(ctx, IPKGPU_ERR_INVALID, "close failed"); t_file += since(t0); }
    ctx->t_write_total = since(t_begin); ctx->t_write_device = t_dev; ctx->t_write_file = t_file;
    if (bytes_written) *bytes_written = total;
    return IPKGPU_OK;
}

}

namespace {

constexpr size_t SPILL_STAGE = (size_t)64 << 20;

int spill_stage(ipkgpu_ctx* ctx, size_t want)
{
    want = std::min(std::max<size_t>(want, 1 << 16), SPILL_STAGE);
    for (int i = 0; i < 2; ++i)
        if (!ctx->ev_spill[i]) HIP_TRY(ctx, hipEventCreateWithFlags(&ctx->ev_spill[i], hipEventDisableTiming));
    if (ctx->h_spill_cap >= want) return IPKGPU_OK;
    for (int i = 0; i < 2; ++i) { if (ctx->h_spill[i]) (void)hipHostFree(ctx->h_spill[i]); ctx->h_spill[i] = nullptr; }
    ctx->h_spill_cap = 0;
    for (int i = 0; i < 2; ++i) HIP_TRY(ctx, hipHostMalloc(&ctx->h_spill[i], want, hipHostMallocDefault));
    ctx->h_spill_cap = want;
    return IPKGPU_OK;
}

struct SpillSeg { uint64_t at, bytes; const void* src; const void* dev; };

std::string spill_block_path(const char* dir, uint32_t piece, uint32_t owner)
{
    char name[64];
    snprintf(name, sizeof name, "/p%u_b%u.blk", piece, owner);
    return std::string(dir) + name;
}

struct SpillFile {
    std::string path; ipkspill::Head head; uint64_t key_base = 0, entry_base = 0;
};

int spill_check_files(ipkgpu_ctx* ctx, uint32_t sigma, uint32_t k, uint32_t owner, uint32_t n_owners, const char* const* paths, uint32_t n_blocks,
                      uint64_t slots, std::vector<SpillFile>& files)
{
    files.resize(n_blocks);
    uint64_t keys = 0, entries = 0;
    for (uint32_t s = 0; s < n_blocks; ++s) {
        if (!paths[s]) return fail(ctx, IPKGPU_ERR_INVALID, "null path of block %u", s);
        SpillFile& f = files[s];
        f.path = paths[s];
        FILE* fh = fopen(paths[s], "rb");
        if (!fh) return fail(ctx, IPKGPU_ERR_INVALID, "cannot open spill block %s", paths[s]);
        struct stat st;
        const bool stat_ok = fstat(fileno(fh), &st) == 0;
        memset(&f.head, 0, sizeof f.head);
        const size_t got = fread(&f.head, 1, sizeof f.head, fh);
        fclose(fh);
        if (!stat_ok) return fail(ctx, IPKGPU_ERR_INVALID, "cannot stat spill block %s", paths[s]);
        const char* what = got < sizeof f.head ? "shorter than a block's head"
                                               : ipkspill::check_head(f.head, (uint64_t)st.st_size, sigma, k, n_owners, owner, slots);
        if (what) return fail(ctx, IPKGPU_ERR_INVALID, "spill block %s: %s", paths[s], what);
        f.key_base = keys; f.entry_base = entries;
        keys += f.head.n_keys; entries += f.head.n_entries;
    }
    return IPKGPU_OK;
}

}

extern "C" {

int ipkgpu_get_option(const ipkgpu_ctx* ctx, const char* name, int64_t* value)
{
    if (!ctx || !name || !value) return IPKGPU_ERR_INVALID;
    if (!strcmp(name, "workspace_bytes")) { *value = ctx->workspace_bytes; return IPKGPU_OK; }
    if (!strcmp(name, "device_budget_bytes")) { *value = ctx->budget; return IPKGPU_OK; }
    if (!strcmp(name, "last_refused_bytes")) { *value = (int64_t)ctx->refused_need; return IPKGPU_OK; }
    if (!strcmp(name, "slice_long_lists")) { *value = ctx->opt_slice; return IPKGPU_OK; }
    if (!strcmp(name, "debug_sliced_windows")) { *value = (int64_t)ctx->sliced_windows; return IPKGPU_OK; }
    return IPKGPU_ERR_INVALID;
}

int ipkgpu_mem_stats(ipkgpu_ctx* ctx, uint64_t* held, uint64_t* held_peak, int reset_peak)
{
    if (!ctx) return IPKGPU_ERR_INVALID;
    if (held) *held = ctx->held;
    if (held_peak) *held_peak = ctx->held_peak;
    if (reset_peak) ctx->held_peak = ctx->held;
    return IPKGPU_OK;
}

int ipkgpu_parts_spill(ipkgpu_ctx* ctx, ipkgpu_parts* parts, const char* dir, uint32_t piece, uint64_t* bytes_written)
{
    if (!ctx) return IPKGPU_ERR_INVALID;
    if (!parts || parts->ctx != ctx || !dir) return fail(ctx, IPKGPU_ERR_INVALID, "bad argument");
    if (parts->d_positions) return fail(ctx, IPKGPU_ERR_INVALID, "positioned parts are not spilled: the on-disk build keeps no positions (as the reference's, db_builder.cpp:469)");
    if (parts->lead != 0) return fail(ctx, IPKGPU_ERR_INVALID, "key-range parts are not spilled: a key-range pass already bounds the device");
    if (!parts->d_counts || !parts->d_entries) return fail(ctx, IPKGPU_ERR_INVALID, "these parts' arrays have moved into a database");
    HIP_TRY(ctx, hipSetDevice(ctx->device));
    const uint32_t B = parts->n_owners;
    const uint64_t slots = parts->slots, W = ipkspill::bit_words(slots), n_words = (uint64_t)B * W;
    if (W > 0xFFFFFFFFull || (n_words + 3) / 4 > 0x7FFFFFFFull) return fail(ctx, IPKGPU_ERR_INVALID, "too many key slots to spill");
    RC_TRY(ensure(ctx, ctx->sp_bits, n_words * 8));
    RC_TRY(ensure(ctx, ctx->sp_pops, n_words * 4));
    RC_TRY(ensure(ctx, ctx->sp_rank, (n_words + 1) * 8));
    RC_TRY(ensure(ctx, ctx->goff, ((size_t)B + 1) * 8));
    uint32_t* d_big = small_at(ctx, SMALL_REC_BIG);
    HIP_TRY(ctx, hipMemsetAsync(d_big, 0, 4, ctx->stream));
    const uint32_t grid = (uint32_t)((n_words + 3) / 4);
    hipLaunchKernelGGL(spill_bits_kernel, dim3(grid), dim3(256), 0, ctx->stream, parts->d_counts, slots, W, n_words,
                       ctx->sp_bits.as<unsigned long long>(), ctx->sp_pops.as<uint32_t>(), d_big);
    HIP_TRY(ctx, hipGetLastError());
    RC_TRY(scan_u32(ctx, ctx->sp_pops.as<uint32_t>(), n_words, ctx->sp_rank.as<uint64_t>()));
    hipLaunchKernelGGL(gather_offsets_kernel, dim3((B + 1 + 255) / 256), dim3(256), 0, ctx->stream, ctx->sp_rank.as<uint64_t>(), (uint32_t)W, B + 1,
                       ctx->goff.as<uint64_t>());
    HIP_TRY(ctx, hipGetLastError());
    std::vector<uint64_t> key_base((size_t)B + 1);
    uint32_t h_big = 0;
    HIP_TRY(ctx, hipMemcpyAsync(key_base.data(), ctx->goff.p, ((size_t)B + 1) * 8, hipMemcpyDeviceToHost, ctx->stream));
    HIP_TRY(ctx, hipMemcpyAsync(&h_big, d_big, 4, hipMemcpyDeviceToHost, ctx->stream));
    HIP_TRY(ctx, hipStreamSynchronize(ctx->stream));
    if (h_big) return fail(ctx, IPKGPU_ERR_INVALID, "a key with more than %u entries in one piece: a spill block's counts are 16-bit (pieces of at most %u groups)",
                           ipkspill::COUNT_MAX, ipkspill::COUNT_MAX);
    RC_TRY(ensure(ctx, ctx->sp_c16, key_base[B] * 2));
    hipLaunchKernelGGL(spill_pack_kernel, dim3(grid), dim3(256), 0, ctx->stream, parts->d_counts, slots, W, n_words, ctx->sp_rank.as<uint64_t>(),
                       ctx->sp_c16.as<uint16_t>());
    HIP_TRY(ctx, hipGetLastError());

    uint64_t largest = 0;
    for (uint32_t o = 0; o < B; ++o)
        largest = std::max(largest, ipkspill::file_bytes(slots, key_base[o + 1] - key_base[o], parts->owner_off[o + 1] - parts->owner_off[o]));
    RC_TRY(spill_stage(ctx, largest));
    const uint64_t cap = ctx->h_spill_cap;
    struct Chunk { uint32_t owner = 0; uint64_t bytes = 0; bool first = false, last = false, pending = false; } chunk[2];
    FILE* fh = nullptr;
    std::string tmp_path, final_path;
    uint64_t total = 0;
    auto abandon = [&]() { if (fh) { fclose(fh); fh = nullptr; } if (!tmp_path.empty()) (void)remove(tmp_path.c_str()); (void)hipStreamSynchronize(ctx->stream); };
    auto write_chunk = [&](int b) -> int {
        Chunk& c = chunk[b];
        if (!c.pending) return IPKGPU_OK;
        c.pending = false;
        HIP_TRY(ctx, hipEventSynchronize(ctx->ev_spill[b]));
        if (c.first) {
            final_path = spill_block_path(dir, piece, c.owner);
            tmp_path = final_path + ".tmp";
            fh = fopen(tmp_path.c_str(), "wb");
            if (!fh) { const std::string p = tmp_path; tmp_path.clear(); return fail(ctx, IPKGPU_ERR_INVALID, "cannot create %s", p.c_str()); }
            setvbuf(fh, nullptr, _IONBF, 0);
        }
        if (fwrite(ctx->h_spill[b], 1, c.bytes, fh) != c.bytes) return fail(ctx, IPKGPU_ERR_INVALID, "write failed: %s", tmp_path.c_str());
        total += c.bytes;
        if (c.last) {
            const int rc = fclose(fh);
            fh = nullptr;
            if (rc != 0) return fail(ctx, IPKGPU_ERR_INVALID, "close failed: %s", tmp_path.c_str());
            if (rename(tmp_path.c_str(), final_path.c_str()) != 0) return fail(ctx, IPKGPU_ERR_INVALID, "cannot rename %s", tmp_path.c_str());
            tmp_path.clear();
        }
        return IPKGPU_OK;
    };
    uint64_t n_chunks = 0;
    int rc = IPKGPU_OK;
    for (uint32_t o = 0; o < B && rc == IPKGPU_OK; ++o) {
        const uint64_t nk = key_base[o + 1] - key_base[o], ne = parts->owner_off[o + 1] - parts->owner_off[o];
        const ipkspill::Head head = ipkspill::make_head(parts->sigma, parts->k, B, o, piece, slots, nk, ne);
        const SpillSeg segs[4] = {
            {0, sizeof head, &head, nullptr},
            {ipkspill::bits_at(), ipkspill::bits_bytes(slots), nullptr, ctx->sp_bits.as<unsigned long long>() + (uint64_t)o * W},
            {ipkspill::counts_at(slots), nk * 2, nullptr, ctx->sp_c16.as<uint16_t>() + key_base[o]},
            {ipkspill::entries_at(slots, nk), ipkspill::entries_bytes(ne), nullptr, parts->d_entries + parts->owner_off[o]}};
        const uint64_t size = ipkspill::file_bytes(slots, nk, ne);
        for (uint64_t lo = 0; lo < size && rc == IPKGPU_OK; lo += cap) {
            const uint64_t hi = std::min(size, lo + cap);
            const int b = (int)(n_chunks++ & 1);
            if ((rc = write_chunk(b)) != IPKGPU_OK) break;
            char* dst = static_cast<char*>(ctx->h_spill[b]);
            memset(dst, 0, hi - lo);
            for (const SpillSeg& sg : segs) {
                const uint64_t a = std::max(lo, sg.at), e = std::min(hi, sg.at + sg.bytes);
                if (a >= e) continue;
                if (sg.src) memcpy(dst + (a - lo), static_cast<const char*>(sg.src) + (a - sg.at), e - a);
                else if (hipMemcpyAsync(dst + (a - lo), static_cast<const char*>(sg.dev) + (a - sg.at), e - a, hipMemcpyDeviceToHost, ctx->stream) != hipSuccess)
                    rc = fail(ctx, IPKGPU_ERR_HIP, "copy of a spill block off the device failed");
            }
            if (rc == IPKGPU_OK && hipEventRecord(ctx->ev_spill[b], ctx->stream) != hipSuccess) rc = fail(ctx, IPKGPU_ERR_HIP, "hipEventRecord failed");
            chunk[b].owner = o; chunk[b].bytes = hi - lo; chunk[b].first = lo == 0; chunk[b].last = hi == size; chunk[b].pending = rc == IPKGPU_OK;
        }
    }
    if (rc == IPKGPU_OK) rc = write_chunk((int)(n_chunks & 1));
    if (rc == IPKGPU_OK) rc = write_chunk((int)((n_chunks + 1) & 1));
    if (rc != IPKGPU_OK) { abandon(); return rc; }
    HIP_TRY(ctx, hipStreamSynchronize(ctx->stream));
    if (bytes_written) *bytes_written = total;
    return IPKGPU_OK;
}

int ipkgpu_spill_merge(ipkgpu_ctx* ctx, uint32_t sigma, uint32_t k, uint32_t owner, uint32_t n_owners, const char* const* block_paths,
                       uint32_t n_blocks, ipkgpu_db** out)
{
    if (out) *out = nullptr;
    if (!block_paths || n_blocks == 0) return fail(ctx, IPKGPU_ERR_INVALID, "no spill blocks given");
    if ((sigma != 4 && sigma != 20) || k < 2 || k > ipkgpu_max_k(sigma)) return fail(ctx, IPKGPU_ERR_INVALID, "unsupported sigma/k");
    if (n_owners == 0 || owner >= n_owners) return fail(ctx, IPKGPU_ERR_INVALID, "bad owner/source counts");
    const uint64_t T = ipow(sigma, (int)k);
    const uint64_t slots = (T + n_owners - 1) / n_owners, W = ipkspill::bit_words(slots);
    std::vector<SpillFile> files;
    RC_TRY(spill_check_files(ctx, sigma, k, owner, n_owners, block_paths, n_blocks, slots, files));
    if (!ctx) return IPKGPU_ERR_INVALID;
    if (!out) return fail(ctx, IPKGPU_ERR_INVALID, "null out pointer");
    const uint32_t S = n_blocks;
    const uint64_t n_words = (uint64_t)S * W;
    if ((n_words + 3) / 4 > 0x7FFFFFFFull) return fail(ctx, IPKGPU_ERR_INVALID, "too many key slots in the blocks of one batch");
    const uint64_t nk_all = files.back().key_base + files.back().head.n_keys, ne_all = files.back().entry_base + files.back().head.n_entries;
    HIP_TRY(ctx, hipSetDevice(ctx->device));
    ipkgpu_db* db = new (std::nothrow) ipkgpu_db();
    if (!db) return fail(ctx, IPKGPU_ERR_NOMEM, "out of host memory");
    db->ctx = ctx;
    struct Guard { ipkgpu_db* r; ~Guard() { if (r) ipkgpu_db_free(r); } } guard{db};
    uint32_t* d_rows = nullptr; uint2* d_ent = nullptr;
    struct BGuard { ipkgpu_ctx* c; uint32_t*& a; uint2*& b; ~BGuard() { (void)hipStreamSynchronize(c->stream); ctx_release(c, a); ctx_release(c, b); } } bguard{ctx, d_rows, d_ent};
    HIP_TRY(ctx, ctx_alloc(ctx, (void**)&d_rows, (size_t)S * slots * 4));
    HIP_TRY(ctx, ctx_alloc(ctx, (void**)&d_ent, std::max<uint64_t>(ne_all, 1) * 8));
    RC_TRY(ensure(ctx, ctx->sp_bits, n_words * 8));
    RC_TRY(ensure(ctx, ctx->sp_pops, n_words * 4));
    RC_TRY(ensure(ctx, ctx->sp_rank, (n_words + 1) * 8));
    RC_TRY(ensure(ctx, ctx->sp_c16, nk_all * 2));
    uint64_t largest = 0;
    for (const SpillFile& f : files) largest = std::max(largest, ipkspill::file_bytes(slots, f.head.n_keys, f.head.n_entries));
    RC_TRY(spill_stage(ctx, largest));
    const uint64_t cap = ctx->h_spill_cap;

// ... 60 lines not shown
```

ipk_amd/csrc/kernels_quad.hpp:

```cpp
#pragma once
#include "kernels_score.hpp"

namespace ipkgpu {

struct QuadNode { int J, H, TH, OFF; uint32_t F, CMUL; };
struct QuadStep { int H, A, B; };

template <int SIGMA, int K>
struct QuadGeo {
    using D = HalvesDD<SIGMA, K>;
    static constexpr int HL = D::HL, HR = D::HR, LA = D::LA, LB = D::LB, RA = D::RA, RB = D::RB;
    static constexpr bool OK = SIGMA == 4 && D::OK && LA >= 2 && LA <= 3 && LB >= 2 && LB <= 3 && RA >= 2 && RA <= 3 && RB >= 2 && RB <= 3;
    static constexpr uint32_t FLA = D::FLA, FLB = D::FLB, FRA = D::FRA, FRB = D::FRB;
    static constexpr uint32_t mulR = ipow(SIGMA, K - K / 2);
    static constexpr uint32_t CW = FLA + FLB + FRA + FRB;
    static constexpr int th_n(int h) { return h == 2 ? 3 : 5; }
    static constexpr int TH0 = 2, TH1 = TH0 + th_n(LA), TH2 = TH1 + th_n(LB), TH3 = TH2 + th_n(RA);
    static constexpr int TH_F = TH3 + th_n(RB);
    static constexpr int PADW = 1;
    static constexpr QuadNode node(int n)
    {
        return n == 0 ? QuadNode{0, LA, TH0, 0, FLA, 1u}
             : n == 1 ? QuadNode{LA, LB, TH1, (int)FLA, FLB, mulR}
             : n == 2 ? QuadNode{HL, RA, TH2, (int)(FLA + FLB), FRA, 1u}
                      : QuadNode{HL + RA, RB, TH3, (int)(FLA + FLB + FRA), FRB, 1u};
    }
    static constexpr int count_h(int h) { int c = 0; for (int n = 0; n < 4; ++n) c += node(n).H == h; return c; }
    static constexpr int nth_h(int h, int i) { for (int n = 0; n < 4; ++n) if (node(n).H == h) { if (i == 0) return n; --i; } return -1; }
    static constexpr int NS2 = (count_h(2) + 1) / 2, NS3 = (count_h(3) + 1) / 2, NSTEPS = NS2 + NS3;
    static constexpr QuadStep step(int s)
    {
        return s < NS2 ? QuadStep{2, nth_h(2, 2 * s), nth_h(2, 2 * s + 1)} : QuadStep{3, nth_h(3, 2 * (s - NS2)), nth_h(3, 2 * (s - NS2) + 1)};
    }
    static constexpr int step_of(int n) { for (int s = 0; s < NSTEPS; ++s) if (step(s).A == n || step(s).B == n) return s; return -1; }
    static constexpr int slot_of(int n) { return step(step_of(n)).B == n ? 1 : 0; }
    static constexpr int NS1 = (count_h(2) > 0 ? 1 : 0) + (count_h(3) > 0 ? 1 : 0);
    static constexpr int step1_h(int s) { return (s == 0 && count_h(2) > 0) ? 2 : 3; }
    static constexpr int step1_node(int s, int slot) { return nth_h(step1_h(s), slot); }
    static constexpr int step1_of(int n) { return node(n).H == 2 ? 0 : (count_h(2) > 0 ? 1 : 0); }
    static constexpr int slot1_of(int n) { int c = 0; for (int m = 0; m < n; ++m) c += node(m).H == node(n).H; return c; }
};

template <int SIGMA, int K, int TW>
struct QuadTile {
    static constexpr int TC = TW + K - 1 + QuadGeo<SIGMA, K>::PADW;
    static constexpr int COLS_F = TC * SIGMA;
    static constexpr int BEST_F = ((TC + 1 + 3) / 4) * 4;
    static constexpr int TH_FLOATS = (((TW + QuadGeo<SIGMA, K>::PADW) * QuadGeo<SIGMA, K>::TH_F + 3) / 4) * 4;
    static constexpr int HEAD_BYTES = (COLS_F + BEST_F + TH_FLOATS) * 4;
};

template <int SIGMA, int K, int CAP, bool ONEWIN = false>
constexpr uint32_t quad_wave_entries()
{
    using Q = QuadGeo<SIGMA, K>;
    return (ONEWIN ? 1 : 2) * Q::CW + Geo<SIGMA, Q::HL, CAP>::CAPH + Geo<SIGMA, Q::HR, CAP>::CAPH;
}

template <int J, int H>
__device__ __forceinline__ void quad_node_thresholds(const float* bs, float e, float* out)
{
    out[0] = e;
    if constexpr (H == 2) {
        out[1] = e - (bs[J + 2] - bs[J + 1]);
        out[2] = e - (bs[J + 1] - bs[J]);
    } else {
        static_assert(H == 3, "child nodes have 2 or 3 symbols");
        const float e_leaf = e - (bs[J + 3] - bs[J + 1]);
        const float e_pair = e - (bs[J + 1] - bs[J]);
        out[1] = e_leaf;
        out[2] = e_pair;
        out[3] = e_pair - (bs[J + 3] - bs[J + 2]);
        out[4] = e_pair - (bs[J + 2] - bs[J + 1]);
    }
}

template <int H>
__device__ __forceinline__ void quad_step(const float* cols, uint32_t base, bool valid, uint64_t vmask, const float* th, uint2* list,
                                          uint32_t l16, uint32_t slot, uint32_t lt16, uint32_t code16, uint32_t cmul, uint32_t& count)
{
    const float e = th[0];
    if constexpr (H == 2) {
        const float sl = cols[base + (l16 >> 2)], sr = cols[base + 4 + (l16 & 3u)];
        const float s = sl + sr;
        const bool c1 = sl > th[1], c2 = sr > th[2], c3 = s > e;
        const bool pass = valid & c1 & c2 & c3;
        const uint64_t m = vmask & ballot64(c1) & ballot64(c2) & ballot64(c3);
        const uint32_t x = (uint32_t)(m >> (16u * slot));
        const uint32_t pos = (uint32_t)__popc(x & lt16);
        if (pass) list[pos] = make_uint2(code16, __float_as_uint(s));
        count = (uint32_t)__popc(x & 0xFFFFu);
    } else {
        const float sj = cols[base + 4 + (l16 >> 2)], sl2 = cols[base + 8 + (l16 & 3u)];
        const float s2 = sj + sl2;
        const bool d1 = sj > th[3], d2 = sl2 > th[4], d3 = s2 > th[2];
        const bool okp = valid & d1 & d2 & d3;
        const uint64_t mp = vmask & ballot64(d1) & ballot64(d2) & ballot64(d3);
        uint32_t run = 0;
#pragma unroll
        for (int i = 0; i < 4; ++i) {
            const float si = cols[base + i];
            const float s = si + s2;
            const bool c1 = si > th[1], c2 = s > e;
            const bool pass = okp & c1 & c2;
            const uint64_t m = mp & ballot64(c1) & ballot64(c2);
            const uint32_t x = (uint32_t)(m >> (16u * slot));
            const uint32_t pos = (uint32_t)__popc(x & lt16) + run;
            if (pass) list[pos] = make_uint2(__umul24(cmul, (uint32_t)i * 16u) + code16, __float_as_uint(s));
            run += (uint32_t)__popc(x & 0xFFFFu);
        }
        count = run;
    }
}

__device__ __forceinline__ void pool_store(uint2* wave_base, uint32_t byte_off, uint2 val)
{
    const unsigned long long data = ((unsigned long long)val.y << 32) | val.x;
    asm volatile("global_store_dwordx2 %0, %1, %2" : : "v"(byte_off), "v"(data), "s"(wave_base) : "memory");
}
__device__ __forceinline__ uint32_t lshl3_add(uint32_t x, uint32_t y)
{
    uint32_t r;
    asm("v_lshl_add_u32 %0, %1, 3, %2" : "=v"(r) : "v"(x), "v"(y));
    return r;
}
__device__ __forceinline__ void pool_store_lanes(uint2* wave_base, uint32_t byte_off, uint2 val, uint64_t mask)
{
    const unsigned long long data = ((unsigned long long)val.y << 32) | val.x;
    IPK_ASSERT_FULL_EXEC();
    asm volatile("s_mov_b64 exec, %3\n\tglobal_store_dwordx2 %0, %1, %2\n\ts_mov_b64 exec, -1"
                 : : "v"(byte_off), "v"(data), "s"(wave_base), "s"(mask) : "memory");
}

__device__ __forceinline__ uint64_t pool_store_inside(uint2* wave_base, uint32_t byte_off, uint2 val, uint32_t v, uint64_t pass, uint32_t CH)
{
    const unsigned long long data = ((unsigned long long)val.y << 32) | val.x;
    uint64_t outside;
    IPK_ASSERT_FULL_EXEC();
    asm volatile("s_mov_b64 exec, %5\n\t"
                 "v_cmpx_gt_u32_e32 vcc, %6, %4\n\t"
                 "global_store_dwordx2 %1, %2, %3\n\t"
                 "s_andn2_b64 %0, %5, exec\n\t"
                 "s_mov_b64 exec, -1"
                 : "=&s"(outside) : "v"(byte_off), "v"(data), "s"(wave_base), "v"(v), "s"(pass), "s"(CH) : "memory", "vcc");
    return outside;
}

constexpr uint32_t QUAD_SPAN_BYTES_LOG2 = 32;
constexpr uint32_t QUAD_SPAN_TEST = 8;

__device__ __forceinline__ uint32_t div_small(float x_plus_half, float rn) { return (uint32_t)(x_plus_half * rn); }

template <uint32_t NB, uint32_t CH>
struct RowAppender {
    static constexpr uint32_t NONE = 0xFFFFFFFFu;
    static constexpr uint32_t CHUNK_BYTES = CH * 8u;
    static constexpr uint32_t SPAN_CHUNKS = (uint32_t)((1ull << QUAD_SPAN_BYTES_LOG2) / CHUNK_BYTES);
    const StreamParams& p;
    unsigned long long* st;
    uint32_t g;
    uint32_t chunk_next = 0, chunk_end = 0;
    uint32_t base_id = 0;
    uint2* base = nullptr;

    __device__ __forceinline__ void init(uint32_t wave_gid)
    {
        const uint32_t first = wave_gid * NB;
        const bool pre = p.pre_chunks != 0 && first + NB <= p.pre_chunks && first + NB <= p.pool_cap;
        for (uint32_t b = lane_id(); b < NB; b += 64)
            st[b] = pre ? ((unsigned long long)(b * CHUNK_BYTES) << 32) : (((unsigned long long)NONE << 32) | (unsigned long long)CH);
        base = p.pool;
        if (pre) {
            base_id = first;
            const unsigned long long a = (unsigned long long)(p.pool + (size_t)first * CH);
            base = reinterpret_cast<uint2*>(((unsigned long long)to_sgpr((uint32_t)(a >> 32)) << 32) | to_sgpr((uint32_t)a));
        }
    }
    __device__ __forceinline__ void write_desc(uint32_t b, unsigned long long s)
    {
        const uint32_t where = (uint32_t)(s >> 32);
        if (where == NONE) return;
        const uint32_t id = base_id + where / CHUNK_BYTES;
        if (id < p.pool_cap) p.desc[id] = ((unsigned long long)(g * NB + b) << 32) | (unsigned long long)min((uint32_t)s, CH);
    }
    __device__ __forceinline__ void rebase(uint32_t nid)
    {
        wave_lds_sync();
        for (uint32_t b = lane_id(); b < NB; b += 64) {
            const unsigned long long s = st[b];
            write_desc(b, s);
            st[b] = ((unsigned long long)NONE << 32) | (unsigned long long)max((uint32_t)s, CH);
        }
        wave_lds_sync();
        base_id = nid;
        const unsigned long long a = (unsigned long long)(p.pool + (size_t)nid * CH);
        base = reinterpret_cast<uint2*>(((unsigned long long)to_sgpr((uint32_t)(a >> 32)) << 32) | to_sgpr((uint32_t)a));
    }
    __device__ __forceinline__ uint32_t roll(uint32_t b)
    {
        const uint32_t lane = lane_id();
        if (chunk_next == chunk_end) {
            uint32_t first = 0;
            if (lane == 0) first = atomicAdd(p.pool_next, ALLOC_BATCH);
            chunk_next = (uint32_t)__builtin_amdgcn_readfirstlane((int)first);
            chunk_end = chunk_next + ALLOC_BATCH;
        }
        uint32_t nid = to_sgpr(chunk_next);
        chunk_next = nid + 1;
        if (nid >= p.pool_cap && lane == 0) atomicOr(p.pool_ovf, 1u);
        nid = min(nid, p.pool_cap);
        if (nid - base_id >= ((p.flags & 8u) ? QUAD_SPAN_TEST : SPAN_CHUNKS)) rebase(nid);
        const uint32_t where = (nid - base_id) * CHUNK_BYTES;
        wave_lds_sync();
        const unsigned long long old = st[b];
        wave_lds_sync();
        if (lane == 0) {
            write_desc(b, old);
            st[b] = ((unsigned long long)where << 32) | (unsigned long long)((uint32_t)old - CH);
        }
        wave_lds_sync();
        return where;
    }
    __device__ __forceinline__ void close()
    {
        wave_lds_sync();
        for (uint32_t b = lane_id(); b < NB; b += 64) write_desc(b, st[b]);
    }
};

template <uint32_t NB, uint32_t CH>
struct LaneAppender {
    static constexpr uint32_t NONE = 0xFFFFFFFFu;
    const StreamParams& p;
    unsigned long long* st;
    uint32_t g;
    uint32_t chunk_next = 0, chunk_end = 0;

    __device__ __forceinline__ void init(uint32_t wave_gid)
    {
        const uint32_t first = wave_gid * NB;
        const bool pre = p.pre_chunks != 0 && first + NB <= p.pre_chunks && first + NB <= p.pool_cap;
        for (uint32_t b = lane_id(); b < NB; b += 64)
            st[b] = pre ? ((unsigned long long)(first + b) << 32) : (((unsigned long long)NONE << 32) | (unsigned long long)CH);
    }
    __device__ __forceinline__ uint32_t roll_at(uint32_t b, uint32_t x)
    {
        const uint32_t lane = lane_id();
        if (chunk_next == chunk_end) {
            uint32_t first = 0;
            if (lane == 0) first = atomicAdd(p.pool_next, ALLOC_BATCH);
            chunk_next = (uint32_t)__builtin_amdgcn_readfirstlane((int)first);
            chunk_end = chunk_next + ALLOC_BATCH;
        }
        uint32_t nid = to_sgpr(chunk_next);
        chunk_next = nid + 1;
        if (nid >= p.pool_cap && lane == 0) atomicOr(p.pool_ovf, 1u);
        nid = min(nid, p.pool_cap);
        wave_lds_sync();
        const unsigned long long old = st[b];
        wave_lds_sync();
        if (lane == 0) {
            const uint32_t oid = (uint32_t)(old >> 32);
            if (oid < p.pool_cap) p.desc[oid] = ((unsigned long long)(g * NB + b) << 32) | (unsigned long long)x;
            st[b] = ((unsigned long long)nid << 32) | (unsigned long long)((uint32_t)old - x);
        }
        wave_lds_sync();
        return nid;
    }
    __device__ __forceinline__ void close()
    {
        wave_lds_sync();
        for (uint32_t b = lane_id(); b < NB; b += 64) {
            const unsigned long long s = st[b];
            const uint32_t id = (uint32_t)(s >> 32);
            if (id < p.pool_cap) p.desc[id] = ((unsigned long long)(g * NB + b) << 32) | (unsigned long long)min((uint32_t)s, CH);
        }
    }
};

__device__ __forceinline__ void store_pair_if_gt(unsigned long long& cursor, uint32_t x, float s, float eps)
{
    u32x2_t data; data.x = x; data.y = __float_as_uint(s);
    IPK_ASSERT_FULL_EXEC();
    asm volatile("v_cmpx_lt_f32_e32 vcc, %3, %2\n\t"
                 "global_store_dwordx2 %0, %1, off\n\t"
                 "v_lshl_add_u64 %0, %0, 0, 8\n\t"
                 "s_mov_b64 exec, -1"
                 : "+v"(cursor) : "v"(data), "v"(s), "s"(eps) : "vcc");
}

template <int SIGMA, int K, int CAP, int TW, int NW, uint32_t TBL, bool COUNT_ONLY = false, bool ROWLANE = false, bool ONEWIN = false>
__global__ __launch_bounds__(NW * 64) void score_quad_kernel(StreamParams p)
{
    extern __shared__ __align__(16) unsigned char smem[];
    using Q = QuadGeo<SIGMA, K>;
    using QT = QuadTile<SIGMA, K, TW>;
    static_assert(Q::OK, "quad kernel: DNA k = 8..12");
    constexpr uint32_t T = ipow(SIGMA, K);
    constexpr uint32_t NB = (T + TBL - 1) / TBL;
    constexpr uint32_t CH = chunk_pairs<TBL>();
    constexpr uint32_t mulR = Q::mulR;
    static_assert(TBL % mulR == 0, "a row of the final join must stay inside one bucket");
    constexpr uint32_t CAPL = Geo<SIGMA, Q::HL, CAP>::CAPH, CAPR = Geo<SIGMA, Q::HR, CAP>::CAPH;
    constexpr uint32_t WS = quad_wave_entries<SIGMA, K, CAP, ONEWIN>();
    constexpr uint32_t WPW = ONEWIN ? 1u : 2u;
    constexpr int NST = ONEWIN ? Q::NS1 : Q::NSTEPS;
    float* cols = reinterpret_cast<float*>(smem);
    float* best = cols + QT::COLS_F;
    float* thr = best + QT::BEST_F;
    uint2* scratch_all = reinterpret_cast<uint2*>(smem + QT::HEAD_BYTES);
    unsigned long long* state_all = reinterpret_cast<unsigned long long*>(scratch_all + (size_t)NW * WS);

    const uint32_t lane = lane_id();
    const uint32_t wave = (uint32_t)__builtin_amdgcn_readfirstlane((int)(threadIdx.x >> 6));
    const uint32_t g = blockIdx.x / p.S, seg = blockIdx.x - g * p.S;
    const uint32_t m0 = p.gm_off[g], nm = p.gm_off[g + 1] - m0;
    const uint32_t total_tiles = nm * p.tiles_per_mat;
    const uint32_t t_lo = (uint32_t)(((uint64_t)total_tiles * seg) / p.S);
    const uint32_t t_hi = (uint32_t)(((uint64_t)total_tiles * (seg + 1)) / p.S);

    uint2* child = scratch_all + (size_t)wave * WS;
    uint2* lp = child + WPW * Q::CW;
    uint2* rp = lp + CAPL;
    using Appender = std::conditional_t<ROWLANE, LaneAppender<NB, CH>, RowAppender<NB, CH>>;
    Appender app{p, state_all + (size_t)wave * NB, g};
    app.init(blockIdx.x * NW + wave);
    unsigned long long emitted = 0;

    const uint32_t l16 = lane & 15u, slot = lane >> 4, half = ONEWIN ? 0u : lane >> 5, sb = slot & 1u;
    const uint32_t lt16 = (1u << l16) - 1u;
    const float lane_h = (float)lane + 0.5f;
    const float eps = p.eps;
    constexpr bool count_only = COUNT_ONLY;
    uint32_t st_j4[NST], st_th[NST], st_off[NST], st_cmul[NST], st_code[NST];
    bool st_on[NST];
#pragma unroll
    for (int s = 0; s < NST; ++s) {
        constexpr QuadNode none{0, 2, 0, 0, 0, 1u};
        if constexpr (ONEWIN) {
            QuadNode nd = none;
            bool on = false;
#pragma unroll
            for (int sl = 0; sl < 4; ++sl) {
                const int n = Q::step1_node(s, sl);
                if (n >= 0 && slot == (uint32_t)sl) { nd = Q::node(n); on = true; }
            }
            st_j4[s] = (uint32_t)nd.J * 4u; st_th[s] = (uint32_t)nd.TH; st_off[s] = (uint32_t)nd.OFF; st_cmul[s] = nd.CMUL;
            st_code[s] = l16 * st_cmul[s]; st_on[s] = on;
        } else {
            const QuadStep qs = Q::step(s);
            const QuadNode na = Q::node(qs.A), nb = qs.B >= 0 ? Q::node(qs.B) : none;
            st_j4[s] = sb ? (uint32_t)nb.J * 4u : (uint32_t)na.J * 4u;
            st_th[s] = sb ? (uint32_t)nb.TH : (uint32_t)na.TH;
            st_off[s] = (sb ? (uint32_t)nb.OFF : (uint32_t)na.OFF) + half * Q::CW;
            st_cmul[s] = sb ? nb.CMUL : na.CMUL;
            st_code[s] = l16 * st_cmul[s];
            st_on[s] = sb ? qs.B >= 0 : true;
        }
    }

    __shared__ uint32_t sh_tile;
    const bool draw = p.tile_next != nullptr;
    uint32_t t = t_lo, t_end = t_hi;
    if (draw) { t = seg; t_end = total_tiles; }
    while (t < t_end) {
        const uint32_t q = t / p.tiles_per_mat, tile = t - q * p.tiles_per_mat;
        const uint32_t mat = p.gm_list[m0 + q];
        const uint32_t t0 = tile * TW;
        const uint32_t nw = min((uint32_t)TW, p.nwin - t0);
        const uint32_t ncol = nw + K - 1;
        __syncthreads();
        uint32_t t_drawn = 0;
        if (draw && threadIdx.x == 0) t_drawn = atomicAdd(&p.tile_next[g], 1u);
        {
            const float4* src = reinterpret_cast<const float4*>(p.logp + ((size_t)mat * p.sites + t0) * SIGMA);
            float4* dst = reinterpret_cast<float4*>(cols);
            const uint32_t n4 = ncol * (SIGMA / 4);
            for (uint32_t i = threadIdx.x; i < n4; i += NW * 64) dst[i] = src[i];
            const float* bsrc = p.best + (size_t)mat * (p.sites + 1) + t0;
            for (uint32_t i = threadIdx.x; i <= ncol; i += NW * 64) best[i] = bsrc[i];
        }
        if (draw && threadIdx.x == 0) sh_tile = t_drawn;
        __syncthreads();
        for (uint32_t w = threadIdx.x; w < nw; w += NW * 64) {
            const float* bs = best + w;
            float* o = thr + w * Q::TH_F;
            const float eps_l = eps - (bs[K] - bs[Q::HL]);
            const float eps_r = eps - (bs[Q::HL] - bs[0]);
            o[0] = eps_l; o[1] = eps_r;
            quad_node_thresholds<0, Q::LA>(bs, eps_l - (bs[Q::HL] - bs[Q::LA]), o + Q::node(0).TH);
            quad_node_thresholds<Q::LA, Q::LB>(bs, eps_l - (bs[Q::LA] - bs[0]), o + Q::node(1).TH);
            quad_node_thresholds<Q::HL, Q::RA>(bs, eps_r - (bs[K] - bs[Q::HL + Q::RA]), o + Q::node(2).TH);
            quad_node_thresholds<Q::HL + Q::RA, Q::RB>(bs, eps_r - (bs[Q::HL + Q::RA] - bs[Q::HL]), o + Q::node(3).TH);
        }
        __syncthreads();

        const uint32_t npair = (nw + WPW - 1) / WPW;
        const float* thw = thr + __umul24(wave * WPW + half, (uint32_t)Q::TH_F);
        for (uint32_t pr = wave; pr < npair; pr += NW, thw += WPW * NW * Q::TH_F) {
            const uint32_t wq = pr * WPW;
            const uint32_t wl = wq + half;
            const bool wvalid = wl < nw;
            uint32_t counts[3] = {0, 0, 0};
            wave_lds_sync();
            auto run_step = [&](auto S) {
                constexpr int s = decltype(S)::value;
                if constexpr (s < NST) {
                    const bool valid = wvalid && st_on[s];
                    const uint64_t vmask = ballot64(valid);
                    const uint32_t base = wl * 4 + st_j4[s];
                    constexpr int H = ONEWIN ? Q::step1_h(s) : Q::step(s < Q::NSTEPS ? s : 0).H;
                    quad_step<H>(cols, base, valid, vmask, thw + st_th[s], child + st_off[s], l16, slot, lt16, st_code[s], st_cmul[s], counts[s]);
                }
            };
            run_step(std::integral_constant<int, 0>{});
            run_step(std::integral_constant<int, 1>{});
            run_step(std::integral_constant<int, 2>{});
            wave_lds_sync();
            const uint32_t nwp = min(WPW, nw - wq);

#pragma unroll 1
            for (uint32_t gw = 0; gw < nwp; ++gw) {
                const uint32_t w = wq + gw;
                constexpr int so0 = ONEWIN ? Q::step1_of(0) : Q::step_of(0), so1 = ONEWIN ? Q::step1_of(1) : Q::step_of(1);
                constexpr int so2 = ONEWIN ? Q::step1_of(2) : Q::step_of(2), so3 = ONEWIN ? Q::step1_of(3) : Q::step_of(3);
                constexpr int sl0 = ONEWIN ? Q::slot1_of(0) : Q::slot_of(0), sl1 = ONEWIN ? Q::slot1_of(1) : Q::slot_of(1);
                constexpr int sl2 = ONEWIN ? Q::slot1_of(2) : Q::slot_of(2), sl3 = ONEWIN ? Q::slot1_of(3) : Q::slot_of(3);
                const uint32_t wbase = ONEWIN ? 0u : gw * 32u;
                const uint32_t nla = (uint32_t)__builtin_amdgcn_readlane((int)counts[so0], (int)(wbase + sl0 * 16));
                const uint32_t nlb = (uint32_t)__builtin_amdgcn_readlane((int)counts[so1], (int)(wbase + sl1 * 16));
                const uint32_t nra = (uint32_t)__builtin_amdgcn_readlane((int)counts[so2], (int)(wbase + sl2 * 16));
                const uint32_t nrb = (uint32_t)__builtin_amdgcn_readlane((int)counts[so3], (int)(wbase + sl3 * 16));
                if (nla * nlb * nra * nrb == 0) continue;
                const uint2* cw = child + gw * Q::CW;
                const uint2 *la = cw + Q::node(0).OFF, *lb = cw + Q::node(1).OFF, *ra = cw + Q::node(2).OFF, *rb = cw + Q::node(3).OFF;
                const float eps_l = thr[w * Q::TH_F], eps_r = thr[w * Q::TH_F + 1];
                const uint32_t tl = nla * nlb, tr = nra * nrb;
                uint32_t nL, nR;
                constexpr bool SLICE = ROWLANE;
                constexpr uint32_t SAFE_L = CAPL / Q::FLB, SAFE_R = CAPR / Q::FRB;
                static_assert(SAFE_L >= 1 && SAFE_R >= 1, "a slice of one row of the first child must fit the list");
                const bool one_step = tl <= 64 && tr <= 64;
                uint32_t sla = nla, sra = nra, ia = 0, ir = 0;
                bool keep_l = false;
                for (;;) {
                wave_lds_sync();
                if (one_step) {
                    const float rnl = __builtin_amdgcn_rcpf((float)nlb), rnr = __builtin_amdgcn_rcpf((float)nrb);
                    const uint32_t il = div_small(lane_h, rnl), jl = (uint32_t)(__mul24((int)il, -(int)nlb) + (int)lane);
                    const uint32_t ir = div_small(lane_h, rnr), jr = (uint32_t)(__mul24((int)ir, -(int)nrb) + (int)lane);
                    const uint2 a0 = la[il], b0 = lb[jl], a1 = ra[ir], b1 = rb[jr];
                    const float s0 = __uint_as_float(a0.y) + __uint_as_float(b0.y);
                    const float s1 = __uint_as_float(a1.y) + __uint_as_float(b1.y);
                    const bool v0 = lane < tl, v1 = lane < tr, c0 = s0 > eps_l, c1 = s1 > eps_r;
                    const bool p0 = v0 && c0, p1 = v1 && c1;
                    const uint64_t h0 = ballot64(v0) & ballot64(c0), h1 = ballot64(v1) & ballot64(c1);
                    if (p0) lp[mbcnt(h0)] = make_uint2(a0.x * (Q::FLB * mulR) + b0.x, __float_as_uint(s0));
                    if (p1) rp[mbcnt(h1)] = make_uint2(a1.x * Q::FRB + b1.x, __float_as_uint(s1));
                    nL = (uint32_t)__popcll(h0); nR = (uint32_t)__popcll(h1);
                } else {
                    if (!keep_l)
                        nL = (uint32_t)__builtin_amdgcn_readfirstlane((int)join_to_list(la + ia, min(sla, nla - ia), lb, nlb, eps_l, Q::FLB * mulR, lp, CAPL));
                    if constexpr (SLICE) {
                        if (nL == LIST_OVERFLOW) { sla = SAFE_L; continue; }
                    }
                    nR = nL == LIST_OVERFLOW || nL == 0 ? nL : (uint32_t)__builtin_amdgcn_readfirstlane((int)join_to_list(ra + ir, min(sra, nra - ir), rb, nrb, eps_r, Q::FRB, rp, CAPR));
                    if constexpr (SLICE) {
                        if (nR == LIST_OVERFLOW) { sra = SAFE_R; keep_l = true; continue; }
                    } else if (nL == LIST_OVERFLOW || nR == LIST_OVERFLOW) {
                        if (lane == 0) {
                            const uint32_t qi = atomicAdd(p.ovf_count, 1u);
                            p.ovf_queue[qi] = ((unsigned long long)mat << 32) | (unsigned long long)(t0 + w);
                        }
                        __builtin_amdgcn_wave_barrier();
                        break;
                    }
                }
                if (nL != 0 && nR != 0) {
                wave_lds_sync();
                if (p.flags & 4u) emitted += nL + nR;
                else
                if constexpr (ROWLANE) {
                    constexpr uint32_t CB = 64;
                    static_assert(CB <= CH, "row-per-lane join: a run must fit a chunk");
                    for (uint32_t ib = 0; ib < nL; ib += 64) {
                        const uint2 a = lp[ib + lane];
                        const bool rv = ib + lane < nL;
                        const float ay = rv ? __uint_as_float(a.y) : -__builtin_inff();
                        const uint32_t bk = a.x / TBL;
                        for (uint32_t jb = 0; jb < nR; jb += CB) {
                            const uint32_t nc = min(CB, nR - jb);
                            const uint2* rj = rp + jb;
                            uint32_t cnt = 0;
                            if constexpr (count_only) {
                                for (uint32_t j = 0; j < nc; ++j) emitted += (uint32_t)__popcll(ballot64(ay + __uint_as_float(rj[j].y) > eps));
                            } else {
                                auto count8 = [&](auto NC, uint32_t j0, uint32_t& n, float e) {
                                    constexpr uint32_t N = decltype(NC)::value;
                                    float by[N];
#pragma unroll
                                    for (uint32_t u = 0; u < N; ++u) by[u] = __uint_as_float(rj[j0 + u].y);
#pragma unroll
                                    for (uint32_t u = 0; u < N; ++u) {
                                        const float sj = ay + by[u];
                                        asm("v_cmp_lt_f32_e32 vcc, %2, %1\n\tv_addc_co_u32_e32 %0, vcc, 0, %0, vcc" : "+v"(n) : "v"(sj), "s"(e) : "vcc");
                                    }
                                };
                                uint32_t j0 = 0;
                                for (; j0 + 8 <= nc; j0 += 8) count8(std::integral_constant<uint32_t, 8>{}, j0, cnt, eps);
                                if (j0 + 4 <= nc) { count8(std::integral_constant<uint32_t, 4>{}, j0, cnt, eps); j0 += 4; }
                                for (; j0 < nc; ++j0) count8(std::integral_constant<uint32_t, 1>{}, j0, cnt, eps);
                            }
                            if constexpr (!count_only) {
                                const bool has = cnt != 0;
                                if (ballot64(has) == 0) continue;
                                if (p.flags & 16u) { emitted += cnt; continue; }
                                unsigned long long got;
                                asm volatile("" : "=v"(got));
                                if (has) got = atomicAdd(&app.st[bk], (unsigned long long)cnt);
                                uint32_t pre = (uint32_t)got, id = (uint32_t)(got >> 32);
                                for (;;) {
                                    uint64_t X = ballot64(has && pre <= CH && pre + cnt > CH);
                                    if (X == 0) break;
                                    do {
                                        const int ls = __ffsll((long long)X) - 1;
                                        const uint32_t bb = (uint32_t)__builtin_amdgcn_readlane((int)bk, ls);
                                        const uint32_t xv = (uint32_t)__builtin_amdgcn_readlane((int)pre, ls);
                                        const uint32_t xid = (uint32_t)__builtin_amdgcn_readlane((int)id, ls);
                                        const uint32_t nid = app.roll_at(bb, xv);
                                        const bool sel = has && bk == bb && id == xid && pre >= xv;
                                        id = sel ? nid : id;
                                        pre = sel ? pre - xv : pre;
                                        X &= X - 1ull;
                                    } while (X);
                                }
                                unsigned long long run = reinterpret_cast<unsigned long long>(p.pool) + (((unsigned long long)id * CH + pre) << 3);
                                if (p.flags & 2u) continue;
                                auto emit8 = [&](auto NC, uint32_t j0) {
                                    constexpr uint32_t N = decltype(NC)::value;
                                    uint2 b[N];
#pragma unroll
                                    for (uint32_t u = 0; u < N; ++u) b[u] = rj[j0 + u];
#pragma unroll
                                    for (uint32_t u = 0; u < N; ++u)
                                        store_pair_if_gt(run, a.x + b[u].x, ay + __uint_as_float(b[u].y), eps);
                                };
                                uint32_t j0 = 0;
                                for (; j0 + 8 <= nc; j0 += 8) emit8(std::integral_constant<uint32_t, 8>{}, j0);
                                if (j0 + 4 <= nc) { emit8(std::integral_constant<uint32_t, 4>{}, j0); j0 += 4; }
                                for (; j0 < nc; ++j0) emit8(std::integral_constant<uint32_t, 1>{}, j0);
                            }
                        }
                    }
                } else
                for (uint32_t jb = 0; jb < nR; jb += 64) {
                    const uint32_t nRb = min(64u, nR - jb);
                    const float rn = __builtin_amdgcn_rcpf((float)nRb);
                    const uint32_t rps = to_sgpr(div_small(64.5f, rn));
                    const uint32_t rsel = div_small(lane_h, rn), rfirst = __umul24(rsel, nRb), col = lane - rfirst;
                    const bool lane_ok = rsel < rps;
                    const uint2 b = rp[jb + col];
                    const float by = __uint_as_float(b.y);
                    const bool is_head = lane_ok && col == 0;
                    const uint64_t okmask = ballot64(lane_ok);
                    const uint64_t rowbits = nRb >= 64 ? ~0ull : ((1ull << nRb) - 1ull);
                    const uint64_t rowmask = lane_ok ? (rowbits << rfirst) : 0ull;
                    const uint32_t rm_lo = (uint32_t)rowmask, rm_hi = (uint32_t)(rowmask >> 32);
                    const int head_addr = (int)(rfirst << 2);
                    const uint2* ap = lp + rsel;
                    auto trip = [&](auto NSC, auto FULLC, uint32_t i0) {
                        constexpr int NS = decltype(NSC)::value;
                        constexpr bool FULL = decltype(FULLC)::value;
                        uint2 a[NS]; float s[NS]; bool live[NS]; uint64_t m[NS]; uint64_t any = 0;
#pragma unroll
                        for (int u = 0; u < NS; ++u) a[u] = ap[i0 + u * rps];
#pragma unroll
                        for (int u = 0; u < NS; ++u) {
                            s[u] = __uint_as_float(a[u].y) + by;
                            const bool c = s[u] > eps;
                            if constexpr (FULL) { live[u] = lane_ok; m[u] = okmask & ballot64(c); }
                            else {
                                const uint32_t nv = min(rps, nL - i0 - u * rps) * nRb;
                                live[u] = lane < nv; m[u] = ballot64(live[u]) & ballot64(c);
                            }
                            any |= m[u];
                        }
#ifndef IPK_QNOANY
                        if (any == 0) return;
#endif
                        if constexpr (count_only) {
#pragma unroll
                            for (int u = 0; u < NS; ++u) emitted += (uint32_t)__popcll(m[u]);
                            return;
                        } else {
                        uint32_t rank[NS], bk[NS], rc[NS]; unsigned long long got[NS];
#pragma unroll
                        for (int u = 0; u < NS; ++u) {
                            const uint32_t xl = (uint32_t)m[u] & rm_lo, xh = (uint32_t)(m[u] >> 32) & rm_hi;
                            rank[u] = __builtin_amdgcn_mbcnt_hi(xh, __builtin_amdgcn_mbcnt_lo(xl, 0u));
                            rc[u] = (uint32_t)__popc(xl) + (uint32_t)__popc(xh);
                            bk[u] = a[u].x / TBL;
                            asm volatile("" : "=v"(got[u]));
                        }
                        if constexpr (FULL) {
                            if (is_head) {
#pragma unroll
                                for (int u = 0; u < NS; ++u) got[u] = atomicAdd(&app.st[bk[u]], (unsigned long long)rc[u]);
                            }
                        } else {
#pragma unroll
                            for (int u = 0; u < NS; ++u)
                                if (is_head && live[u]) got[u] = atomicAdd(&app.st[bk[u]], (unsigned long long)rc[u]);
                        }
                        uint32_t v[NS]; uint2 val[NS]; uint64_t ovf[NS]; uint64_t anyo = 0;
#pragma unroll
                        for (int u = 0; u < NS; ++u) {
                            const uint32_t fill = (uint32_t)__builtin_amdgcn_ds_bpermute(head_addr, (int)(uint32_t)got[u]);
                            const uint32_t where = (uint32_t)__builtin_amdgcn_ds_bpermute(head_addr, (int)(uint32_t)(got[u] >> 32));
                            v[u] = fill + rank[u];
                            val[u] = make_uint2(a[u].x + b.x, __float_as_uint(s[u]));
                            ovf[u] = pool_store_inside(app.base, lshl3_add(v[u], where), val[u], v[u], m[u], CH);
                            anyo |= ovf[u];
                        }
                        while (anyo) {
                            uint32_t bb = 0;
                            bool found = false;
#pragma unroll
                            for (int u = 0; u < NS; ++u)
                                if (!found && ovf[u]) { bb = (uint32_t)__builtin_amdgcn_readlane((int)bk[u], (int)(__ffsll((long long)ovf[u]) - 1)); found = true; }
                            const uint32_t nwhere = app.roll(bb);
                            anyo = 0;
#pragma unroll
                            for (int u = 0; u < NS; ++u) {
                                const bool h = ((ovf[u] >> lane) & 1ull) != 0 && bk[u] == bb;
                                if (h) pool_store(app.base, nwhere + ((v[u] - CH) << 3), val[u]);
                                ovf[u] &= ~ballot64(h);
                                anyo |= ovf[u];
                            }
                        }
                        }
                    };
                    using I1 = std::integral_constant<int, 1>; using I2 = std::integral_constant<int, 2>;
                    uint32_t i0 = 0;
                    using I3 = std::integral_constant<int, 3>;
                    for (; i0 + 3 * rps <= nL; i0 += 3 * rps) trip(I3{}, std::true_type{}, i0);
                    for (; i0 + 2 * rps <= nL; i0 += 2 * rps) trip(I2{}, std::true_type{}, i0);
                    if (i0 + rps < nL) trip(I2{}, std::false_type{}, i0);
                    else if (i0 < nL) trip(I1{}, std::false_type{}, i0);
                }
                }
                if (!SLICE || one_step) break;
                ir += sra;
                if (nL != 0 && ir < nra) { keep_l = true; continue; }
                ir = 0; keep_l = false; ia += sla;
                if (ia >= nla) break;
                }
            }
        }
        t = draw ? sh_tile : t + 1;
    }
    if (!count_only) app.close();
    if (lane == 0 && emitted) atomicAdd(p.emitted, emitted);
}

}
```

ipk_amd/csrc/kernels_score.hpp:

```cpp
#pragma once
#include <type_traits>
#include "dcla_device.hpp"

namespace ipkgpu {


template <int SIGMA, int M>
__global__ __launch_bounds__(256) void prefix_max_kernel(const float* __restrict__ logp, uint32_t n_mats, uint32_t sites,
                                                         float* __restrict__ best)
{
    constexpr int CH = 2048 / M;
    constexpr int ROW = CH + 4;
    static_assert(M == 1 || M == 2 || M == 4 || M == 8, "matrices per workgroup");
    __shared__ __align__(16) float cmbuf[2][M][ROW];
    const uint32_t mat0 = blockIdx.x * M;
    const uint32_t mv = min((uint32_t)M, n_mats - mat0);
    const bool chain = threadIdx.x < mv;
    const uint32_t my = mat0 + (chain ? threadIdx.x : 0u);
    float* b = best + (size_t)my * (sites + 1);
    if (chain) b[0] = 0.0f;
    float carry = 0.0f;
    auto maxima = [&](uint32_t c0, float (*cmw)[ROW], uint32_t t0, uint32_t nt) {
        const uint32_t n = min((uint32_t)CH, sites - c0);
        for (uint32_t mm = 0; mm < mv; ++mm) {
// ... 243 lines not shown
        const bool first = cl == 0 && cr == 0;
        if (cr == 0) {
            if (first) {
                nl = Node<SIGMA, 0, HL, CAP, LN>::build(c, eps_l, lp);
                l_over = nl == LIST_OVERFLOW; r_over = false;
                dead = nl == 0 || (l_over && (!slice_on || SL == 0));
            }
            if constexpr (SL > 0) {
                if (l_over && !dead) {
                    WinCtx cs = c;
                    cs.lead_c = c.lead_c * NCL + cl;
                    nl = Node<SIGMA, 0, HL, CAP, NLT>::build(cs, eps_l, lp);
                    add_base(lp, nl, cl * BASE_L);
                }
            }
            if (!dead && (first || (l_over && !r_over && nl != 0))) {
                nr = Node<SIGMA, HL, HR, CAP>::build(c, eps_r, rp);
                if (first) {
                    r_over = nr == LIST_OVERFLOW;
                    dead = nr == 0 || (r_over && (!slice_on || SR == 0));
                }
            }
        }
        if constexpr (SR > 0) {
            if (r_over && !dead && nl != 0) {
                WinCtx cs = c;
                cs.lead_c = cr;
                nr = Node<SIGMA, HL, HR, CAP, SR, HL>::build(cs, eps_r, rp);
                add_base(rp, nr, cr * BASE_R);
            }
        }
        if (dead) {
            nl = 0; nr = 0;
            if (first && (l_over || r_over) && lane_id() == 0 && big_ovf) atomicOr(big_ovf, 1u);
        }
        wave_lds_sync();
        uint32_t flags = 0;
        if (dead || !r_over || nl == 0 || cr + 1 == NCR) flags |= LAST_R;
        if (dead || !l_over || cl + 1 == NCL) flags |= LAST_L;
        if (first && !dead && (l_over || r_over)) flags |= SLICED;
        return flags;
    }
};

template <int SIGMA, int K, bool POS = false>
__global__ __launch_bounds__(OVF_NW * 64) void score_overflow_kernel(ScoreParams p)
{
    extern __shared__ __align__(16) unsigned char smem[];
    constexpr int CAPF = big_capf<SIGMA, K>();
    using TG = TileGeo<SIGMA, K, 1>;
    __shared__ uint32_t sh_n[2];
    float* cols = reinterpret_cast<float*>(smem);
    float* best = cols + TG::COLS_F;
    uint2* scratch = reinterpret_cast<uint2*>(smem + TG::HEAD_BYTES);
    const uint32_t n = *p.ovf_count;
    const uint32_t lane = lane_id(), wave = threadIdx.x >> 6;
    unsigned long long emitted = 0;
    constexpr uint32_t mulR = ipow(SIGMA, K - K / 2);
    using SH = SlicedHalves<SIGMA, K, CAPF, 0>;
    constexpr bool CAPPED = CAPF == BIG_CAP_ENTRIES;
    [[maybe_unused]] SH sh;
    [[maybe_unused]] uint32_t cl = 0, cr = 0;
    [[maybe_unused]] bool more = false;
    for (uint32_t q = blockIdx.x; q < n; q += CAPPED && more ? 0u : gridDim.x) {
        const unsigned long long e = p.ovf_queue[q];
        const uint32_t mat = (uint32_t)(e >> 32), start = (uint32_t)e;
        __syncthreads();
        const float* src = p.logp + ((size_t)mat * p.sites + start) * SIGMA;
        for (uint32_t i = threadIdx.x; i < K * SIGMA; i += OVF_NW * 64) cols[i] = src[i];
        const float* bsrc = p.best + (size_t)mat * (p.sites + 1) + start;
        for (uint32_t i = threadIdx.x; i <= K; i += OVF_NW * 64) best[i] = bsrc[i];
        __syncthreads();
        const size_t tab_off = (size_t)p.mat_slot[mat] * p.table_size;
        uint32_t* tab = reinterpret_cast<uint32_t*>(p.table) + tab_off;
        unsigned long long* tab64 = reinterpret_cast<unsigned long long*>(p.table) + tab_off;
        const uint32_t inv_seq = POS ? 0xFFFFFFFFu - (p.mat_rank[mat] * p.nwin + start) : 0u;
        const uint2 *L = scratch, *R = scratch + Geo<SIGMA, K / 2, CAPF>::CAPH;
        if (wave == 0) {
            WinCtx c{cols, best, 0};
            if constexpr (!CAPPED) {
                uint32_t nL = 0, nR = 0;
                const bool fits = build_halves<SIGMA, K, CAPF>(c, p.eps, scratch, L, nL, R, nR);
                if (!fits) { nL = 0; nR = 0; if (lane == 0 && p.big_ovf) atomicOr(p.big_ovf, 1u); }
                if (lane == 0) { sh_n[0] = nL; sh_n[1] = nR; }
            } else {
                const uint32_t f = sh.step(c, p.eps, scratch, cl, cr, p.slice_lists != 0, p.big_ovf);
                if (lane == 0) {
                    sh_n[0] = sh.nl | (f << 16); sh_n[1] = sh.nr;
                    if ((f & SH::SLICED) && p.big_ovf) atomicAdd(p.big_ovf - 1, 1u);
                }
            }
        }
        __syncthreads();
        const uint32_t nL = CAPPED ? sh_n[0] & 0xFFFFu : sh_n[0], nR = sh_n[1];
        if constexpr (CAPPED) {
            const uint32_t last = sh_n[0] >> 16;
            cr = (last & SH::LAST_R) ? 0u : cr + 1;
            if (last & SH::LAST_R) cl = (last & SH::LAST_L) ? 0u : cl + 1;
            more = (cl | cr) != 0;
        }
        if (nL == 0 || nR == 0) continue;
        uint32_t cnt = 0;
        constexpr uint32_t OVF_ROWS = 4;
        const bool no_put = (p.flags & 1u) != 0 || IPK_OVF_NOPUT;
        for (uint32_t jb = 0; jb < nR; jb += 64) {
            const uint32_t j = jb + lane;
            const bool valid = j < nR;
            uint2 b = make_uint2(0, 0);
            if (valid) b = R[j];
            const float by = __uint_as_float(b.y);
            for (uint32_t i0 = wave; i0 < nL; i0 += OVF_NW * OVF_ROWS) {
                uint2 a[OVF_ROWS];
#pragma unroll
                for (uint32_t u = 0; u < OVF_ROWS; ++u) a[u] = L[min(i0 + u * OVF_NW, nL - 1)];
#pragma unroll
                for (uint32_t u = 0; u < OVF_ROWS; ++u) {
                    const float s = __uint_as_float(a[u].y) + by;
                    const bool pass = valid && (i0 + u * OVF_NW < nL) && (s > p.eps);
                    if (pass && !no_put) {
                        const uint32_t idx = a[u].x * mulR + b.x;
                        if constexpr (POS) PutScorePos{tab64, inv_seq}(idx, __float_as_uint(s));
                        else {
#if IPK_OVF_UNCOND_OR
                            atomicMax(tab + idx, enc_score_bits(__float_as_uint(s)));
                            if (p.mask) atomicOr(p.mask + (size_t)p.mat_slot[mat] * p.mask_words + (idx >> 5), 1u << (idx & 31u));
#elif IPK_OVF_PEEK
                            const uint32_t enc = enc_score_bits(__float_as_uint(s));
                            if (__builtin_nontemporal_load(tab + idx) < enc) {
                                const uint32_t old = atomicMax(tab + idx, enc);
                                if (old == 0u && p.mask)
                                    atomicOr(p.mask + (size_t)p.mat_slot[mat] * p.mask_words + (idx >> 5), 1u << (idx & 31u));
                            }
#else
                            const uint32_t old = atomicMax(tab + idx, enc_score_bits(__float_as_uint(s)));
                            if (old == 0u && p.mask)
                                atomicOr(p.mask + (size_t)p.mat_slot[mat] * p.mask_words + (idx >> 5), 1u << (idx & 31u));
#endif
                        }
                    }
                    cnt += (uint32_t)__popcll(__ballot(pass));
                }
            }
        }
        emitted += cnt;
    }
    if (lane == 0 && emitted) atomicAdd(p.emitted, emitted);
}

#ifndef IPK_CH512_TBL
#define IPK_CH512_TBL 0u
#endif
template <uint32_t TBL> constexpr uint32_t chunk_pairs() { return (TBL == 16384 || TBL == IPK_CH512_TBL) ? 512u : 256u; }
inline uint32_t chunk_pairs_rt(uint32_t tbl) { return (tbl == 16384 || tbl == IPK_CH512_TBL) ? 512u : 256u; }
constexpr uint32_t CHUNK_NONE = 0xFFFFFFFFu;
constexpr uint32_t ALLOC_BATCH = 32;
constexpr uint32_t SUB = 1;

struct StreamParams {
    const float* logp;
    const float* best;
    const uint32_t* gm_off;
    const uint32_t* gm_list;
    uint32_t sites, nwin, tiles_per_mat, S;
    float eps;
    uint32_t slice_lists = 0;
    uint2* pool;
    uint32_t pool_cap;
    uint32_t* pool_next;
    unsigned long long* desc;
    uint32_t* pool_ovf;
    unsigned long long* emitted;
    unsigned long long* ovf_queue;
    uint32_t* ovf_count;
    const uint32_t* mat_slot;
    uint32_t flags;
    uint32_t pre_chunks;
    uint32_t* tile_next = nullptr;
    uint32_t* big_ovf = nullptr;
};

__device__ __constant__ uint32_t RCP16[65] = {
    0, 65536, 32768, 21846, 16384, 13108, 10923, 9363, 8192, 7282, 6554, 5958, 5462, 5042, 4682, 4370, 4096,
    3856, 3641, 3450, 3277, 3121, 2979, 2850, 2731, 2622, 2521, 2428, 2341, 2260, 2185, 2115, 2048,
    1986, 1928, 1873, 1821, 1772, 1725, 1681, 1639, 1599, 1561, 1525, 1490, 1457, 1425, 1395, 1366,
    1338, 1311, 1286, 1261, 1237, 1214, 1192, 1171, 1150, 1130, 1111, 1093, 1075, 1058, 1041, 1024};

template <int SIGMA, int K>
struct HalvesDD {
    static constexpr int HL = K / 2, HR = K - K / 2;
    static constexpr int LA = HL / 2, LB = HL - LA, RA = HR / 2, RB = HR - RA;
    static constexpr bool OK = ipow(SIGMA, HL) > 64 && ipow(SIGMA, LB) <= 64 && ipow(SIGMA, RB) <= 64;
    static constexpr uint32_t FLA = ipow(SIGMA, LA), FLB = ipow(SIGMA, LB), FRA = ipow(SIGMA, RA), FRB = ipow(SIGMA, RB);
};
template <int SIGMA, int K, int CAP>
constexpr uint32_t stream_wave_scratch()
{
    using D = HalvesDD<SIGMA, K>;
    if constexpr (D::OK)
        return Geo<SIGMA, D::HL, CAP>::CAPH + Geo<SIGMA, D::HR, CAP>::CAPH + D::FLA + D::FLB + D::FRA + D::FRB;
    else
        return wave_scratch_entries<SIGMA, K, CAP>();
}

template <int SIGMA, int K, int CAP>
__device__ __forceinline__ bool build_halves_dd(const WinCtx& c, float eps, uint2* scratch,
                                                const uint2*& Lp, uint32_t& nL, const uint2*& Rp, uint32_t& nR)
{
    using D = HalvesDD<SIGMA, K>;
    constexpr int HL = D::HL, HR = D::HR, LA = D::LA, LB = D::LB, RA = D::RA, RB = D::RB;
    using GL = Geo<SIGMA, HL, CAP>;
    using GR = Geo<SIGMA, HR, CAP>;
    const uint32_t lane = lane_id();
    const float* bs = c.best + c.w;
    const float eps_l = eps - (bs[K] - bs[HL]);
    const float eps_r = eps - (bs[HL] - bs[0]);
    const float eps_la = eps_l - (bs[HL] - bs[LA]);
    const float eps_lb = eps_l - (bs[LA] - bs[0]);
    const float eps_ra = eps_r - (bs[K] - bs[HL + RA]);
    const float eps_rb = eps_r - (bs[HL + RA] - bs[HL]);
    uint2* lp = scratch;
    uint2* rp = lp + GL::CAPH;
    uint2* la = rp + GR::CAPH;
    uint2* lb = la + D::FLA;
    uint2* ra = lb + D::FLB;
    uint2* rb = ra + D::FRA;
    Lp = lp; Rp = rp; nL = 0; nR = 0;

    float sla = 0.f, slb = 0.f, sra = 0.f, srb = 0.f;
    bool pla = false, plb = false, pra = false, prb = false;
    if (lane < D::FLA) pla = Direct<SIGMA, 0, LA>::eval(c, eps_la, lane, sla);
    if (lane < D::FLB) plb = Direct<SIGMA, LA, LB>::eval(c, eps_lb, lane, slb);
    if (lane < D::FRA) pra = Direct<SIGMA, HL, RA>::eval(c, eps_ra, lane, sra);
    if (lane < D::FRB) prb = Direct<SIGMA, HL + RA, RB>::eval(c, eps_rb, lane, srb);
    const uint64_t mla = __ballot(pla), mlb = __ballot(plb), mra = __ballot(pra), mrb = __ballot(prb);
    if (mla == 0 || mlb == 0 || mra == 0 || mrb == 0) return true;
    if (pla) la[mbcnt(mla)] = make_uint2(lane, __float_as_uint(sla));
    if (plb) lb[mbcnt(mlb)] = make_uint2(lane, __float_as_uint(slb));
    if (pra) ra[mbcnt(mra)] = make_uint2(lane, __float_as_uint(sra));
    if (prb) rb[mbcnt(mrb)] = make_uint2(lane, __float_as_uint(srb));
    const uint32_t nla = (uint32_t)__popcll(mla), nlb = (uint32_t)__popcll(mlb);
    const uint32_t nra = (uint32_t)__popcll(mra), nrb = (uint32_t)__popcll(mrb);
    wave_lds_sync();
    const uint32_t tl = nla * nlb, tr = nra * nrb;
    uint32_t cl, cr;
    if (tl <= 64 && tr <= 64) {
        const uint32_t il = (lane * RCP16[nlb]) >> 16, jl = lane - il * nlb;
        const uint32_t ir = (lane * RCP16[nrb]) >> 16, jr = lane - ir * nrb;
        uint2 a0 = make_uint2(0, 0), b0 = a0, a1 = a0, b1 = a0;
        if (lane < tl) { a0 = la[il]; b0 = lb[jl]; }
        if (lane < tr) { a1 = ra[ir]; b1 = rb[jr]; }
        const float s0 = __uint_as_float(a0.y) + __uint_as_float(b0.y);
        const float s1 = __uint_as_float(a1.y) + __uint_as_float(b1.y);
        const bool p0 = (lane < tl) && (s0 > eps_l);
        const bool p1 = (lane < tr) && (s1 > eps_r);
        const uint64_t m0 = __ballot(p0), m1 = __ballot(p1);
        if (p0) lp[mbcnt(m0)] = make_uint2(a0.x * D::FLB + b0.x, __float_as_uint(s0));
        if (p1) rp[mbcnt(m1)] = make_uint2(a1.x * D::FRB + b1.x, __float_as_uint(s1));
        cl = (uint32_t)__popcll(m0); cr = (uint32_t)__popcll(m1);
    } else {
        cl = join_to_list(la, nla, lb, nlb, eps_l, D::FLB, lp, GL::CAPH);
        if (cl == LIST_OVERFLOW) return false;
        if (cl == 0) return true;
        cr = join_to_list(ra, nra, rb, nrb, eps_r, D::FRB, rp, GR::CAPH);
        if (cr == LIST_OVERFLOW) return false;
    }
    nL = cl; nR = cr;
    wave_lds_sync();
    return true;
}

template <uint32_t TBL, uint32_t NB>
struct Appender {
    static constexpr uint32_t CH = chunk_pairs<TBL>();
    const StreamParams& p;
    uint32_t* cbase;
    uint32_t* cfill;
    uint32_t g;
    uint32_t chunk_next = 0, chunk_end = 0;

    __device__ __forceinline__ uint32_t roll(uint32_t bb)
    {
        const uint32_t lane = lane_id();
        if (chunk_next == chunk_end) {
            uint32_t base = 0;
            if (lane == 0) base = atomicAdd(p.pool_next, ALLOC_BATCH);
            chunk_next = (uint32_t)__builtin_amdgcn_readfirstlane((int)base);
            chunk_end = chunk_next + ALLOC_BATCH;
        }
        uint32_t nid = chunk_next++;
        if (nid >= p.pool_cap) { if (lane == 0) atomicOr(p.pool_ovf, 1u); nid = CHUNK_NONE; }
        wave_lds_sync();
        const uint32_t old_id = cbase[bb];
        wave_lds_sync();
        if (lane == 0) {
            if (old_id != CHUNK_NONE) p.desc[old_id] = ((unsigned long long)(g * NB + bb / SUB) << 32) | (unsigned long long)CH;
            cbase[bb] = nid;
            cfill[bb] = cfill[bb] - CH;
        }
        wave_lds_sync();
        return nid;
    }

    __device__ __forceinline__ void append2(bool pass0, uint32_t idx0, uint32_t sb0, bool pass1, uint32_t idx1, uint32_t sb1)
    {
        const uint32_t sub = lane_id() & (SUB - 1);
        const uint32_t bk0 = pass0 ? (idx0 / TBL) * SUB + sub : 0u, bk1 = pass1 ? (idx1 / TBL) * SUB + sub : 0u;
        uint32_t slot0 = 0, slot1 = 0, cb0 = CHUNK_NONE, cb1 = CHUNK_NONE;
        if (pass0) slot0 = atomicAdd(&cfill[bk0], 1u);
        if (pass1) slot1 = atomicAdd(&cfill[bk1], 1u);
        if (pass0) cb0 = cbase[bk0];
        if (pass1) cb1 = cbase[bk1];
        const bool st = !(p.flags & 1u);
        if (pass0 && slot0 < CH && cb0 != CHUNK_NONE && st) p.pool[(size_t)cb0 * CH + slot0] = make_uint2(idx0, sb0);
        if (pass1 && slot1 < CH && cb1 != CHUNK_NONE && st) p.pool[(size_t)cb1 * CH + slot1] = make_uint2(idx1, sb1);
        const bool o0 = pass0 && slot0 >= CH, o1 = pass1 && slot1 >= CH;
        uint64_t ovf0 = __ballot(o0), ovf1 = __ballot(o1);
        while (ovf0 | ovf1) {
            uint32_t bb;
            if (ovf0) bb = (uint32_t)__builtin_amdgcn_readlane((int)bk0, (int)(__ffsll((long long)ovf0) - 1));
            else      bb = (uint32_t)__builtin_amdgcn_readlane((int)bk1, (int)(__ffsll((long long)ovf1) - 1));
            const bool h0 = o0 && bk0 == bb, h1 = o1 && bk1 == bb;
            const uint64_t m0 = __ballot(h0), m1 = __ballot(h1);
            const uint32_t nid = roll(bb);
            if (h0 && nid != CHUNK_NONE && st) p.pool[(size_t)nid * CH + (slot0 - CH)] = make_uint2(idx0, sb0);
            if (h1 && nid != CHUNK_NONE && st) p.pool[(size_t)nid * CH + (slot1 - CH)] = make_uint2(idx1, sb1);
            ovf0 &= ~m0; ovf1 &= ~m1;
        }
    }
};

template <int SIGMA, int K, int CAP, int TW, int NW, uint32_t TBL>
__global__ __launch_bounds__(NW * 64) __attribute__((amdgpu_num_sgpr(80))) void score_stream_kernel(StreamParams p)
{
    extern __shared__ __align__(16) unsigned char smem[];
    constexpr uint32_t CH = chunk_pairs<TBL>();
    using TG = TileGeo<SIGMA, K, TW>;
    constexpr uint32_t T = ipow(SIGMA, K);
    constexpr uint32_t NB = (T + TBL - 1) / TBL;
    constexpr uint32_t WS = stream_wave_scratch<SIGMA, K, CAP>();
    float* cols = reinterpret_cast<float*>(smem);
    float* best = cols + TG::COLS_F;
    uint2* scratch_all = reinterpret_cast<uint2*>(smem + TG::HEAD_BYTES);
    uint32_t* state_all = reinterpret_cast<uint32_t*>(scratch_all + (size_t)NW * WS);

    const uint32_t lane = lane_id(), wave = threadIdx.x >> 6;
    const uint32_t g = blockIdx.x / p.S, seg = blockIdx.x - g * p.S;
    const uint32_t m0 = p.gm_off[g], nm = p.gm_off[g + 1] - m0;
    const uint32_t total_tiles = nm * p.tiles_per_mat;
    const uint32_t t_lo = (uint32_t)(((uint64_t)total_tiles * seg) / p.S);
    const uint32_t t_hi = (uint32_t)(((uint64_t)total_tiles * (seg + 1)) / p.S);

    uint2* scratch = scratch_all + (size_t)wave * WS;
    uint32_t* cbase = state_all + (size_t)wave * 2 * NB * SUB;
    uint32_t* cfill = cbase + NB * SUB;
    for (uint32_t b = lane; b < NB * SUB; b += 64) { cbase[b] = CHUNK_NONE; cfill[b] = CH; }
    Appender<TBL, NB> app{p, cbase, cfill, g};
    unsigned long long emitted = 0;
    constexpr uint32_t mulR = ipow(SIGMA, K - K / 2);

    for (uint32_t t = t_lo; t < t_hi; ++t) {
        const uint32_t q = t / p.tiles_per_mat, tile = t - q * p.tiles_per_mat;
        const uint32_t mat = p.gm_list[m0 + q];
        const uint32_t t0 = tile * TW;
        const uint32_t nw = min((uint32_t)TW, p.nwin - t0);
        const uint32_t ncol = nw + K - 1;
        __syncthreads();
        {
            const float4* src = reinterpret_cast<const float4*>(p.logp + ((size_t)mat * p.sites + t0) * SIGMA);
            float4* dst = reinterpret_cast<float4*>(cols);
            const uint32_t n4 = ncol * (SIGMA / 4);
            for (uint32_t i = threadIdx.x; i < n4; i += NW * 64) dst[i] = src[i];
            const float* bsrc = p.best + (size_t)mat * (p.sites + 1) + t0;
            for (uint32_t i = threadIdx.x; i <= ncol; i += NW * 64) best[i] = bsrc[i];
        }
        __syncthreads();
        for (uint32_t w = wave; w < nw; w += NW) {
            WinCtx c{cols, best, w};
            const uint2 *L, *R;
            uint32_t nL, nR;
            static_assert(!Geo<SIGMA, K, CAP>::DIRECT, "stream variant needs k with sigma^k > 64");
            bool ok;
            if constexpr (HalvesDD<SIGMA, K>::OK) ok = build_halves_dd<SIGMA, K, CAP>(c, p.eps, scratch, L, nL, R, nR);
            else ok = build_halves<SIGMA, K, CAP>(c, p.eps, scratch, L, nL, R, nR);
            if (!ok) {
                if (lane == 0) {
                    const uint32_t qi = atomicAdd(p.ovf_count, 1u);
                    p.ovf_queue[qi] = ((unsigned long long)mat << 32) | (unsigned long long)(t0 + w);
                }
                continue;
            }
            if (nL == 0 || nR == 0) continue;
            if (p.flags & 4u) { emitted += nL + nR; continue; }
            uint32_t cnt = 0;
            if (nR < 64) {
                const uint32_t total = nL * nR;
                const uint32_t M = RCP16[nR];
                const uint32_t q64 = (64u * M) >> 16, r64 = 64u - q64 * nR;
                uint32_t bi = 0, bj = 0;
                for (uint32_t base = 0; base < total; base += 128) {
                    uint32_t bi1 = bi + q64, bj1 = bj + r64;
                    if (bj1 >= nR) { bj1 -= nR; ++bi1; }
                    const uint32_t ta = bj + lane, tb = bj1 + lane;
                    const uint32_t qa = (ta * M) >> 16, qb = (tb * M) >> 16;
                    const bool va = base + lane < total, vb = base + 64 + lane < total;
                    uint2 a0 = make_uint2(0, 0), b0 = a0, a1 = a0, b1 = a0;
                    if (va) { a0 = L[bi + qa]; b0 = R[ta - qa * nR]; }
                    if (vb) { a1 = L[bi1 + qb]; b1 = R[tb - qb * nR]; }
                    const float s0 = __uint_as_float(a0.y) + __uint_as_float(b0.y);
                    const float s1 = __uint_as_float(a1.y) + __uint_as_float(b1.y);
                    const bool p0 = va && (s0 > p.eps), p1 = vb && (s1 > p.eps);
                    cnt += (uint32_t)__popcll(__ballot(p0)) + (uint32_t)__popcll(__ballot(p1));
                    if (!(p.flags & 2u))
                        app.append2(p0, a0.x * mulR + b0.x, __float_as_uint(s0), p1, a1.x * mulR + b1.x, __float_as_uint(s1));
                    bi = bi1 + q64; bj = bj1 + r64;
                    if (bj >= nR) { bj -= nR; ++bi; }
                }
            } else {
                for (uint32_t i = 0; i < nL; ++i) {
                    const uint2 a = L[i];
                    for (uint32_t jb = 0; jb < nR; jb += 128) {
                        const uint32_t ja = jb + lane, jc = jb + 64 + lane;
                        const bool va = ja < nR, vb = jc < nR;
                        uint2 b0 = make_uint2(0, 0), b1 = b0;
                        if (va) b0 = R[ja];
                        if (vb) b1 = R[jc];
                        const float s0 = __uint_as_float(a.y) + __uint_as_float(b0.y);
                        const float s1 = __uint_as_float(a.y) + __uint_as_float(b1.y);
                        const bool p0 = va && (s0 > p.eps), p1 = vb && (s1 > p.eps);
                        cnt += (uint32_t)__popcll(__ballot(p0)) + (uint32_t)__popcll(__ballot(p1));
                        if (!(p.flags & 2u))
                            app.append2(p0, a.x * mulR + b0.x, __float_as_uint(s0), p1, a.x * mulR + b1.x, __float_as_uint(s1));
                    }
                }
            }
            emitted += cnt;
        }
    }
    wave_lds_sync();
    for (uint32_t b = lane; b < NB * SUB; b += 64) {
        const uint32_t id = cbase[b];
        if (id != CHUNK_NONE) p.desc[id] = ((unsigned long long)(g * NB + b / SUB) << 32) | (unsigned long long)min(cfill[b], CH);
    }
    if (lane == 0 && emitted) atomicAdd(p.emitted, emitted);
}

template <int SIGMA, int K, uint32_t TBL>
__global__ __launch_bounds__(OVF_NW * 64) void score_overflow_stream_kernel(StreamParams p)
{
    extern __shared__ __align__(16) unsigned char smem[];
    constexpr uint32_t CH = chunk_pairs<TBL>();
    constexpr int CAPF = big_capf<SIGMA, K>();
    constexpr uint32_t T = ipow(SIGMA, K);
    constexpr uint32_t NB = (T + TBL - 1) / TBL;
    using TG = TileGeo<SIGMA, K, 1>;
    __shared__ uint32_t sh_n[2];
    float* cols = reinterpret_cast<float*>(smem);
    float* best = cols + TG::COLS_F;
    uint2* scratch = reinterpret_cast<uint2*>(smem + TG::HEAD_BYTES);
    uint32_t* state_all = reinterpret_cast<uint32_t*>(scratch + wave_scratch_entries<SIGMA, K, CAPF>());
    const uint32_t n = *p.ovf_count;
    const uint32_t lane = lane_id(), wave = threadIdx.x >> 6;
    uint32_t* cbase = state_all + (size_t)wave * 2 * NB * SUB;
    uint32_t* cfill = cbase + NB * SUB;
    for (uint32_t b = lane; b < NB * SUB; b += 64) { cbase[b] = CHUNK_NONE; cfill[b] = CH; }
    Appender<TBL, NB> app{p, cbase, cfill, 0u};
    bool have_group = false;
    unsigned long long emitted = 0;
    constexpr uint32_t mulR = ipow(SIGMA, K - K / 2);
    auto close_chunks = [&]() {
        wave_lds_sync();
        for (uint32_t b = lane; b < NB * SUB; b += 64) {
            const uint32_t id = cbase[b];
            if (id != CHUNK_NONE) p.desc[id] = ((unsigned long long)(app.g * NB + b / SUB) << 32) | (unsigned long long)min(cfill[b], CH);
            cbase[b] = CHUNK_NONE; cfill[b] = CH;
        }
        wave_lds_sync();
    };
    const uint32_t per = (n + gridDim.x - 1) / gridDim.x;
    const uint32_t q_lo = min(n, blockIdx.x * per), q_hi = min(n, q_lo + per);
    for (uint32_t q = q_lo; q < q_hi; ++q) {
        const unsigned long long e = p.ovf_queue[q];
        const uint32_t g = (uint32_t)(e >> 42), mat = (uint32_t)(e >> 21) & 0x1FFFFFu, start = (uint32_t)e & 0x1FFFFFu;
        if (have_group && g != app.g) close_chunks();
        app.g = g; have_group = true;
        __syncthreads();
        const float* src = p.logp + ((size_t)mat * p.sites + start) * SIGMA;
        for (uint32_t i = threadIdx.x; i < K * SIGMA; i += OVF_NW * 64) cols[i] = src[i];
        const float* bsrc = p.best + (size_t)mat * (p.sites + 1) + start;
        for (uint32_t i = threadIdx.x; i <= K; i += OVF_NW * 64) best[i] = bsrc[i];
        __syncthreads();
        const uint2 *L = scratch, *R = scratch + Geo<SIGMA, K / 2, CAPF>::CAPH;
        if (wave == 0) {
            WinCtx c{cols, best, 0};
            uint32_t nL = 0, nR = 0;
            const bool fits = build_halves<SIGMA, K, CAPF>(c, p.eps, scratch, L, nL, R, nR);
            if (!fits) { nL = 0; nR = 0; if (lane == 0 && p.big_ovf) atomicOr(p.big_ovf, 1u); }
            if (lane == 0) { sh_n[0] = nL; sh_n[1] = nR; }
        }
        __syncthreads();
        const uint32_t nL = sh_n[0], nR = sh_n[1];
        if (nL == 0 || nR == 0) continue;
        uint32_t cnt = 0;
        for (uint32_t i = wave; i < nL; i += OVF_NW) {
            const uint2 a = L[i];
            for (uint32_t jb = 0; jb < nR; jb += 128) {
                const uint32_t ja = jb + lane, jc = jb + 64 + lane;
                const bool va = ja < nR, vb = jc < nR;
                uint2 b0 = make_uint2(0, 0), b1 = b0;
                if (va) b0 = R[ja];
                if (vb) b1 = R[jc];
                const float s0 = __uint_as_float(a.y) + __uint_as_float(b0.y);
                const float s1 = __uint_as_float(a.y) + __uint_as_float(b1.y);
                const bool p0 = va && (s0 > p.eps), p1 = vb && (s1 > p.eps);
                cnt += (uint32_t)__popcll(__ballot(p0)) + (uint32_t)__popcll(__ballot(p1));
                app.append2(p0, a.x * mulR + b0.x, __float_as_uint(s0), p1, a.x * mulR + b1.x, __float_as_uint(s1));
            }
        }
        emitted += cnt;
    }
    if (have_group) close_chunks();
    if (lane == 0 && emitted) atomicAdd(p.emitted, emitted);
}

__global__ __launch_bounds__(256) void ovf_group_keys_kernel(const unsigned long long* __restrict__ queue, uint32_t n,
                                                             const uint32_t* __restrict__ mat_slot,
                                                             unsigned long long* __restrict__ out)
{
    const uint32_t i = blockIdx.x * 256 + threadIdx.x;
    if (i >= n) return;
    const unsigned long long e = queue[i];
    const uint32_t mat = (uint32_t)(e >> 32), start = (uint32_t)e;
    out[i] = ((unsigned long long)mat_slot[mat] << 42) | ((unsigned long long)mat << 21) | (unsigned long long)start;
}

__global__ __launch_bounds__(256) void chunk_hist_kernel(const unsigned long long* __restrict__ desc, uint32_t n,
                                                         uint32_t* __restrict__ cnt, unsigned long long* __restrict__ pairs,
                                                         uint32_t* __restrict__ gb_pairs ,
                                                         const uint32_t* __restrict__ n_dev = nullptr)
{
    __shared__ unsigned long long wsum[4];
    unsigned long long c = 0;
    if (n_dev) n = min(n, *n_dev);
    for (uint32_t i = blockIdx.x * 256 + threadIdx.x; i < n; i += gridDim.x * 256) {
        const unsigned long long d = desc[i];
        if ((uint32_t)d != 0u) {
            atomicAdd(&cnt[(uint32_t)(d >> 32)], 1u);
            if (gb_pairs) atomicAdd(&gb_pairs[(uint32_t)(d >> 32)], (uint32_t)d);
        }
        c += (uint32_t)d;
    }
    if (pairs) {
        for (int o = 32; o > 0; o >>= 1) c += __shfl_down(c, o, 64);
        if (lane_id() == 0) wsum[threadIdx.x >> 6] = c;
        __syncthreads();
        if (threadIdx.x == 0) {
            const unsigned long long t = wsum[0] + wsum[1] + wsum[2] + wsum[3];
            if (t) atomicAdd(pairs, t);
        }
    }
}
__global__ __launch_bounds__(256) void chunk_scatter_kernel(const unsigned long long* __restrict__ desc, uint32_t n,
                                                            const uint64_t* __restrict__ off, uint32_t* __restrict__ cur,
                                                            uint2* __restrict__ list, const uint32_t* __restrict__ n_dev = nullptr)
{
    if (n_dev) n = min(n, *n_dev);
    for (uint32_t i = blockIdx.x * 256 + threadIdx.x; i < n; i += gridDim.x * 256) {
        const unsigned long long d = desc[i];
        if ((uint32_t)d == 0u) continue;
        const uint32_t gb = (uint32_t)(d >> 32);
        list[off[gb] + atomicAdd(&cur[gb], 1u)] = make_uint2(i, (uint32_t)d);
    }
}

constexpr uint32_t SMALL_EMITTED = 0;
constexpr uint32_t SMALL_OVF_COUNT = 16;
constexpr uint32_t SMALL_POOL_NEXT = 32;
constexpr uint32_t SMALL_POOL_OVF = 36;
constexpr uint32_t SMALL_SLICED = 40;
constexpr uint32_t SMALL_BIG_OVF = 44;
constexpr uint32_t SMALL_OVF_EMITTED = 48;
constexpr uint32_t SMALL_XP_TOO_BIG = 56;
constexpr uint32_t SMALL_REC_BIG = 60;
constexpr uint32_t SMALL_BYTES = 64;

__global__ void small_reset_kernel(uint32_t* __restrict__ small, uint32_t pre_chunks, uint32_t* __restrict__ tile_next, uint32_t n_groups,
                                   uint32_t first_tile)
{
    const uint32_t i = blockIdx.x * blockDim.x + threadIdx.x;
    if (i < SMALL_XP_TOO_BIG / 4) small[i] = i == SMALL_POOL_NEXT / 4 ? pre_chunks : 0u;
    if (tile_next && i < n_groups) tile_next[i] = first_tile;
}

__device__ __forceinline__ void store_slice_mask(const uint32_t* tab, uint32_t nslots, uint32_t* mask_words, uint32_t nthreads)
{
    const uint32_t lane = lane_id(), wave = threadIdx.x >> 6, nwv = nthreads >> 6;
    const uint32_t nblk = (nslots + 63) / 64;
    const uint32_t bpw = (nblk + nwv - 1) / nwv;
    const uint32_t b_lo = min(nblk, wave * bpw), b_hi = min(nblk, b_lo + bpw);
    for (uint32_t b0 = b_lo; b0 < b_hi; b0 += 64) {
        const uint32_t nb = min(64u, b_hi - b0);
        uint64_t mine = 0;
#pragma unroll 4
        for (uint32_t j = 0; j < nb; ++j) {
            const uint32_t c = (b0 + j) * 64;
            const uint32_t v = (c + lane < nslots) ? tab[c + lane] : 0u;
            const uint64_t m = __ballot(v != 0u);
            if (lane == j) mine = m;
        }
        if (lane < nb) *reinterpret_cast<uint2*>(mask_words + 2 * (b0 + lane)) = make_uint2((uint32_t)mine, (uint32_t)(mine >> 32));
    }
}

__global__ __launch_bounds__(256) void comp_slice_room_kernel(const uint32_t* __restrict__ gb_pairs, uint32_t n_gb, uint32_t NB, uint64_t T,
                                                              uint32_t TBL, uint32_t* __restrict__ room)
{
    const uint32_t i = blockIdx.x * 256 + threadIdx.x;
    if (i >= n_gb) return;
    const uint32_t b = i % NB;
    const uint32_t nslots = (uint32_t)min((uint64_t)TBL, T - (uint64_t)b * TBL);
    room[i] = (min(gb_pairs[i], nslots) + 1u) / 2u;
}

#ifndef IPK_RB_ABL
#define IPK_RB_ABL 0
#endif
#ifndef IPK_COMPACT
#define IPK_COMPACT 0
#endif
template <uint32_t LANE>
__device__ __forceinline__ void writelane_imm(uint32_t& v, uint32_t s)
{
    asm("s_nop 1\n\tv_writelane_b32 %0, %1, %2" : "+v"(v) : "s"(s), "n"(LANE));
}
template <uint32_t LANE>
__device__ __forceinline__ void writelane64_imm(uint32_t& vlo, uint32_t& vhi, uint64_t s)
{
    asm("s_nop 1\n\tv_writelane_b32 %0, %2, %4\n\tv_writelane_b32 %1, %3, %4"
        : "+v"(vlo), "+v"(vhi) : "s"((uint32_t)s), "s"((uint32_t)(s >> 32)), "n"(LANE));
}
template <uint32_t N, class F, uint32_t... I>
__device__ __forceinline__ void static_for_impl(F&& f, std::integer_sequence<uint32_t, I...>) { (f(std::integral_constant<uint32_t, I>{}), ...); }
template <uint32_t N, class F>
__device__ __forceinline__ void static_for(F&& f) { static_for_impl<N>(f, std::make_integer_sequence<uint32_t, N>{}); }

template <uint32_t TBL, int NT> constexpr uint32_t comp_bpw() { return ((TBL + 63) / 64 + NT / 64 - 1) / (NT / 64); }
template <uint32_t TBL, int NT> constexpr uint32_t comp_padded_slots() { return comp_bpw<TBL, NT>() * (NT / 64) * 64; }
template <uint32_t TBL, int NT, bool ZERO = false, bool REREAD = false>
__device__ __forceinline__ void compress_slice(uint32_t* tab, uint32_t nslots, uint32_t* vals, uint32_t* mrow, uint32_t* rrow,
                                               uint64_t* arow, uint32_t* ucnt_gb)
{
    constexpr uint32_t NWV = NT / 64, BPW = comp_bpw<TBL, NT>(), PAD = comp_padded_slots<TBL, NT>();
    static_assert(BPW <= 64, "one lane per block of the wave");
    uint32_t* wtot = tab + PAD;
    const uint32_t lane = lane_id(), wave = (uint32_t)__builtin_amdgcn_readfirstlane((int)(threadIdx.x >> 6));
    const uint32_t nblk = (nslots + 63) / 64;
    uint32_t* wb = tab + wave * (BPW * 64) + lane;
    uint32_t vr[REREAD ? 1 : BPW];
    uint32_t mine = 0;
    if constexpr (REREAD) {
#pragma unroll
        for (uint32_t j = 0; j < BPW; ++j) mine += (uint32_t)__popcll(__ballot(wb[j * 64] != 0u));
    } else {
#pragma unroll
        for (uint32_t j = 0; j < BPW; ++j) vr[j] = wb[j * 64];
#pragma unroll
        for (uint32_t j = 0; j < BPW; ++j) mine += (uint32_t)__popcll(__ballot(vr[j] != 0u));
    }
    if (lane == 0) wtot[wave] = mine;
    __syncthreads();
    uint32_t base = 0, all = 0;
#pragma unroll
    for (uint32_t w = 0; w < NWV; ++w) { const uint32_t t = wtot[w]; if (w < wave) base += t; all += t; }
    base = (uint32_t)__builtin_amdgcn_readfirstlane((int)base);
    uint32_t my_base = 0, my_lo = 0, my_hi = 0;
    char* vbytes = reinterpret_cast<char*>(vals);
    if constexpr (IPK_COMPACT != 0) {
        uint32_t* wreg = tab + wave * (BPW * 64);
        uint32_t lp = 0;
        static_for<BPW>([&](auto J) {
            constexpr uint32_t j = decltype(J)::value;
            uint32_t v;
            if constexpr (REREAD) v = wb[j * 64]; else v = vr[j];
            const uint64_t m = __ballot(v != 0u);
            writelane_imm<j>(my_base, base + lp);
            writelane64_imm<j>(my_lo, my_hi, m);
            if (v != 0u) wreg[lp + mbcnt(m)] = v;
            lp += (uint32_t)__popcll(m);
        });
        uint32_t* dst = vals + base;
        for (uint32_t t = lane; t < lp; t += 64) {
            const uint32_t v = wreg[t];
            if (!(IPK_RB_ABL & 4) || v == 0xFFFFFFFEu) dst[t] = v;
        }
        if constexpr (ZERO) {
#pragma unroll
            for (uint32_t j = 0; j < BPW; ++j) wb[j * 64] = 0u;
        }
    } else {
    static_for<BPW>([&](auto J) {
        constexpr uint32_t j = decltype(J)::value;
        uint32_t v;
        if constexpr (REREAD) v = wb[j * 64]; else v = vr[j];
        const uint64_t m = __ballot(v != 0u);
        writelane_imm<j>(my_base, base);
        writelane64_imm<j>(my_lo, my_hi, m);
        if ((IPK_RB_ABL & 4) ? v == 0xFFFFFFFEu : v != 0u) *reinterpret_cast<uint32_t*>(vbytes + ((base + mbcnt(m)) << 2)) = v;
        if constexpr (ZERO) wb[j * 64] = 0u;
        base += (uint32_t)__popcll(m);
    });
    }
    const uint32_t blk = wave * BPW + lane;
    if (lane < BPW && blk < nblk) {
        rrow[blk] = my_base;
        *reinterpret_cast<uint2*>(mrow + 2 * blk) = make_uint2(my_lo, my_hi);
        arow[blk] = (uint64_t)(vals + my_base);
    }
    if (threadIdx.x == 0) *ucnt_gb = all;
}

#ifndef IPK_RB_CPT
#define IPK_RB_CPT 2
#endif
#ifndef IPK_RB_NT
#define IPK_RB_NT 0
#endif
__device__ __forceinline__ uint2 pool_load(const uint2* p)
{
#if IPK_RB_NT
    const unsigned long long v = __builtin_nontemporal_load(reinterpret_cast<const unsigned long long*>(p));
    return make_uint2((uint32_t)v, (uint32_t)(v >> 32));
#else
    return *p;
#endif
}

template <uint32_t TBL, int NT, bool COMPRESS = false>
__global__ __launch_bounds__(NT) void reduce_buckets_kernel(const uint2* __restrict__ pool,
                                                           const uint64_t* __restrict__ off, const uint2* __restrict__ list,
                                                           uint32_t NB, uint64_t T, uint32_t* __restrict__ table,
                                                           uint32_t* __restrict__ mask, uint64_t mask_words,
                                                           uint2* __restrict__ cvals, const uint64_t* __restrict__ coff,
                                                           uint32_t* __restrict__ rank, uint64_t* __restrict__ vaddr,
                                                           uint32_t* __restrict__ ucnt)
{
    constexpr uint32_t CH = chunk_pairs<TBL>();
    extern __shared__ __align__(16) unsigned char smem[];
    uint32_t* tab = reinterpret_cast<uint32_t*>(smem);
    constexpr uint32_t NWV = NT / 64;
    const uint32_t gb = blockIdx.x;
    const uint32_t g = gb / NB, b = gb - g * NB;
    const uint64_t key0 = (uint64_t)b * TBL;
    const uint32_t nslots = (uint32_t)min((uint64_t)TBL, T - key0);
    const uint32_t lane = lane_id(), wave = threadIdx.x >> 6;
    const uint64_t c0 = off[gb], c1 = off[gb + 1];
    constexpr int CPT = IPK_RB_CPT;
    uint64_t ci = c0 + wave;
    uint2 e[CPT];
#pragma unroll
    for (int c = 0; c < CPT; ++c) { e[c] = make_uint2(0, 0); if (ci + (uint64_t)c * NWV < c1) e[c] = list[ci + (uint64_t)c * NWV]; }
    constexpr uint32_t CLR = COMPRESS ? comp_padded_slots<TBL, NT>() : TBL;
    for (uint32_t i = threadIdx.x; i < CLR / 4; i += NT) reinterpret_cast<uint4*>(tab)[i] = make_uint4(0, 0, 0, 0);
    __syncthreads();
    const uint32_t k0 = (uint32_t)key0;
    while (ci < c1) {
        constexpr int PER = CH / 64;
        uint2 v[CPT * PER];
        uint32_t n[CPT];
#pragma unroll
        for (int c = 0; c < CPT; ++c) {
            n[c] = (ci + (uint64_t)c * NWV < c1) ? e[c].y : 0u;
            const uint2* s = pool + (size_t)e[c].x * CH;
#pragma unroll
            for (int j = 0; j < PER; ++j) {
                v[c * PER + j] = make_uint2(0, 0);
                if constexpr (IPK_RB_ABL & 1) { if (lane + 64 * j < n[c]) v[c * PER + j] = make_uint2(k0 + ((lane * 97u + j * 13u + (uint32_t)ci) & (TBL - 1)), lane); }
                else if (lane + 64 * j < n[c]) v[c * PER + j] = pool_load(s + lane + 64 * j);
            }
        }
        ci += (uint64_t)CPT * NWV;
#pragma unroll
        for (int c = 0; c < CPT; ++c) if (ci + (uint64_t)c * NWV < c1) e[c] = list[ci + (uint64_t)c * NWV];
#pragma unroll
        for (int c = 0; c < CPT; ++c)
#pragma unroll
            for (int j = 0; j < PER; ++j)
                if constexpr (IPK_RB_ABL & 2) { if (v[c * PER + j].x == 0xFFFFFFFFu) tab[0] = v[c * PER + j].y; }
                else if (lane + 64 * j < n[c]) atomicMax(&tab[v[c * PER + j].x - k0], enc_score_bits(v[c * PER + j].y));
    }
    __syncthreads();
    if constexpr (COMPRESS) {
        compress_slice<TBL, NT>(tab, nslots, reinterpret_cast<uint32_t*>(cvals + coff[gb]), mask + (size_t)g * mask_words + (key0 >> 5),
                                rank + (size_t)g * (mask_words / 2) + (key0 >> 6), vaddr + (size_t)g * (mask_words / 2) + (key0 >> 6), ucnt + gb);
        return;
    }
    uint32_t* dst = table + (size_t)g * T + key0;
    if ((nslots & 3u) == 0 && ((((size_t)g * T + key0) & 3u) == 0)) {
        for (uint32_t i = threadIdx.x; i < nslots / 4; i += NT) reinterpret_cast<uint4*>(dst)[i] = reinterpret_cast<uint4*>(tab)[i];
    } else {
        for (uint32_t i = threadIdx.x; i < nslots; i += NT) dst[i] = tab[i];
    }
    if (mask) store_slice_mask(tab, nslots, mask + (size_t)g * mask_words + (key0 >> 5), NT);
}


template <int NCH, int RC>
__device__ __forceinline__ void xp_rank_by_counting(uint32_t n, const unsigned long long (&kj)[RC], uint32_t (&rank)[RC])
{
#pragma unroll
    for (int ci = 0; ci < NCH; ++ci) {
        const uint32_t lo = (uint32_t)kj[ci], hi = (uint32_t)(kj[ci] >> 32);
        const uint32_t m = min(64u, n - min(n, (uint32_t)ci * 64u));
        for (uint32_t l = 0; l < m; ++l) {
            const unsigned long long ki = ((unsigned long long)(uint32_t)__builtin_amdgcn_readlane((int)hi, (int)l) << 32) |
                                          (unsigned long long)(uint32_t)__builtin_amdgcn_readlane((int)lo, (int)l);
#pragma unroll
            for (int c = 0; c < NCH; ++c) rank[c] += (ki > kj[c]) ? 1u : 0u;
        }
    }
}

#ifndef IPK_SORT_DPP
#define IPK_SORT_DPP 1
#endif
template <int NCH, int RC>
__device__ __forceinline__ void xp_sort_desc(unsigned long long (&kj)[RC])
{
    static_assert(NCH >= 1 && NCH <= RC && (NCH & (NCH - 1)) == 0, "a power of two of 64-key registers");
    const uint32_t lane = lane_id();
#pragma unroll
    for (int size = 2; size <= NCH * 64; size <<= 1) {
#pragma unroll
        for (int stride = size >> 1; stride >= 1; stride >>= 1) {
            if (stride >= 64) {
                constexpr int dummy = 0; (void)dummy;
                const int cs = stride >> 6;
#pragma unroll
                for (int c = 0; c < NCH; ++c) {
                    if ((c & cs) != 0) continue;
                    const bool desc = ((c * 64) & size) == 0 || size == NCH * 64;
                    const unsigned long long a = kj[c], b = kj[c | cs];
                    const bool sw = desc ? (a < b) : (a > b);
                    kj[c] = sw ? b : a;
                    kj[c | cs] = sw ? a : b;
                }
            } else {
                const int addr = (int)((lane ^ (uint32_t)stride) << 2);
                const bool lower = (lane & (uint32_t)stride) == 0;
#pragma unroll
                for (int c = 0; c < NCH; ++c) {
                    const unsigned long long a = kj[c];
                    uint32_t olo, ohi;
                    if constexpr (IPK_SORT_DPP != 0) {
                        if (stride == 1) {
                            olo = (uint32_t)__builtin_amdgcn_mov_dpp((int)(uint32_t)a, 0xB1, 0xF, 0xF, true);
                            ohi = (uint32_t)__builtin_amdgcn_mov_dpp((int)(uint32_t)(a >> 32), 0xB1, 0xF, 0xF, true);
                        } else if (stride == 2) {
                            olo = (uint32_t)__builtin_amdgcn_mov_dpp((int)(uint32_t)a, 0x4E, 0xF, 0xF, true);
                            ohi = (uint32_t)__builtin_amdgcn_mov_dpp((int)(uint32_t)(a >> 32), 0x4E, 0xF, 0xF, true);
                        } else {
                            olo = (uint32_t)__builtin_amdgcn_ds_bpermute(addr, (int)(uint32_t)a);
                            ohi = (uint32_t)__builtin_amdgcn_ds_bpermute(addr, (int)(uint32_t)(a >> 32));
                        }
                    } else {
                        olo = (uint32_t)__builtin_amdgcn_ds_bpermute(addr, (int)(uint32_t)a);
                        ohi = (uint32_t)__builtin_amdgcn_ds_bpermute(addr, (int)(uint32_t)(a >> 32));
                    }
                    const unsigned long long o = ((unsigned long long)ohi << 32) | olo;
                    const uint32_t e = (uint32_t)c * 64u + lane;
                    const bool desc = (e & (uint32_t)size) == 0 || size == NCH * 64;
                    const bool keep_max = lower == desc;
                    const bool take = keep_max ? (o > a) : (o < a);
                    kj[c] = take ? o : a;
                }
            }
        }
    }
}

struct XpParams {
    StreamParams s;
    uint32_t* cnt;
    const uint64_t* off;
    uint32_t stride;
    uint32_t* ovcur;
    const uint32_t* start;
    uint32_t lead_c = 0;
    uint32_t* seq = nullptr;
    const uint32_t* mat_rank = nullptr;
};

__global__ __launch_bounds__(256) void xp_unit_starts_kernel(const uint64_t* __restrict__ off, uint32_t NB, uint32_t S, uint32_t stride,
                                                             uint64_t n, uint32_t* __restrict__ start, uint32_t* __restrict__ too_big)
{
    const uint64_t i = (uint64_t)blockIdx.x * 256 + threadIdx.x;
    if (i >= n) return;
    const uint32_t b = (uint32_t)(i % NB);
    const uint64_t u = i / NB;
    const uint32_t seg = (uint32_t)(u % S);
    const uint64_t g = u / S;
    const uint64_t rel = off[(g * NB + b) * stride + seg] - off[g * NB * stride];
    if (rel >> 32) atomicOr(too_big, 1u);
    start[i] = (uint32_t)rel;
}

template <int SIGMA, int K, int CAP, int TW, int NW, uint32_t TBL, bool WRITE, int KK = K, bool POS = false>
__global__ __launch_bounds__(NW * 64) void score_xp_kernel(XpParams xp)
{
    extern __shared__ __align__(16) unsigned char smem[];
    const StreamParams& p = xp.s;
    using TG = TileGeo<SIGMA, K, TW>;
    constexpr int LN = K - KK;
    constexpr uint32_t T = ipow(SIGMA, KK);
    constexpr uint32_t NB = (T + TBL - 1) / TBL;
    constexpr uint32_t WS = stream_wave_scratch<SIGMA, K, CAP>();
    constexpr uint32_t mulR = ipow(SIGMA, K - K / 2);
    constexpr uint32_t NSUB = mulR > TBL ? mulR / TBL : 1;
// ... 485 lines not shown
```

Baseline: 129.9 billion.

## Store quad-kernel pool pairs in a 6-byte split-plane layout

Result: faster. 136.4 billion (median of 6 runs) (+5.0%).

```diff
diff --git a/ipk_amd/csrc/ipkgpu.hip b/ipk_amd/csrc/ipkgpu.hip
--- a/ipk_amd/csrc/ipkgpu.hip
+++ b/ipk_amd/csrc/ipkgpu.hip
@@ -569,19 +569,22 @@
     }
 }
 
-template <int SIGMA, int K>
+template <int SIGMA, int K, PairLayout LAYOUT = PairLayout::PAIR8>
 int launch_stream_overflow(ipkgpu_ctx* ctx, const StreamParams& sp)
 {
     constexpr uint32_t TBL = stream_tbl<SIGMA, K>();
     if constexpr (TBL == 0 || ipow(SIGMA, K - K / 2) <= (uint32_t)fast_cap<SIGMA, K>()) {
         (void)ctx; (void)sp;
         return IPKGPU_OK;
+    } else if constexpr (LAYOUT != PairLayout::PAIR8 && (TBL & (TBL - 1)) != 0) {
+        (void)sp;
+        return fail(ctx, IPKGPU_ERR_INVALID, "no 6-byte pair layout for this sigma/k");
     } else {
         constexpr uint32_t NB = (uint32_t)((ipow(SIGMA, K) + TBL - 1) / TBL);
         constexpr size_t lds = TileGeo<SIGMA, K, 1>::HEAD_BYTES + (size_t)wave_scratch_entries<SIGMA, K, big_capf<SIGMA, K>()>() * 8 +
                                (size_t)OVF_NW * 2 * NB * SUB * 4;
         static_assert(lds + 64 <= 160 * 1024, "big-list (stream) LDS budget");
-        auto kern = score_overflow_stream_kernel<SIGMA, K, TBL>;
+        auto kern = score_overflow_stream_kernel<SIGMA, K, TBL, LAYOUT>;
         if (lds > 64 * 1024)
             HIP_TRY(ctx, hipFuncSetAttribute(reinterpret_cast<const void*>(kern), hipFuncAttributeMaxDynamicSharedMemorySize, (int)lds));
         const uint32_t per_cu = (uint32_t)std::max<size_t>(1, std::min<size_t>(32 / OVF_NW, (160 * 1024) / (lds + 64)));
@@ -597,11 +600,12 @@
 #ifndef IPK_RPIPE_D
 #define IPK_RPIPE_D 2
 #endif
+template <int SIGMA, int K> constexpr PairLayout quad_layout();
 template <int SIGMA, int K>
-int launch_stream_pass2(ipkgpu_ctx* ctx, uint32_t n_gb, uint64_t T, uint32_t* table, bool compress)
+int launch_stream_pass2(ipkgpu_ctx* ctx, uint32_t n_gb, uint64_t T, uint32_t* table, bool compress, PairLayout layout)
 {
     constexpr uint32_t TBL = stream_tbl<SIGMA, K>();
-    if constexpr (TBL == 0) { (void)n_gb; (void)T; (void)table; (void)compress; return fail(ctx, IPKGPU_ERR_INVALID, "stream variant unsupported"); }
+    if constexpr (TBL == 0) { (void)n_gb; (void)T; (void)table; (void)compress; (void)layout; return fail(ctx, IPKGPU_ERR_INVALID, "stream variant unsupported"); }
     else {
         constexpr uint32_t NB = (uint32_t)((ipow(SIGMA, K) + TBL - 1) / TBL);
         constexpr int NT = TBL <= 16384 ? 512 : 1024;
@@ -616,7 +620,7 @@
             return IPKGPU_OK;
         };
         if constexpr (TBL * 4 > 80 * 1024) {
-            if (compress && ((IPK_RPIPE_DEFAULT != 0) != ((ctx->opt_flags & 2048) != 0))) {
+            if (layout == PairLayout::PAIR8 && compress && ((IPK_RPIPE_DEFAULT != 0) != ((ctx->opt_flags & 2048) != 0))) {
                 constexpr int PD = IPK_RPIPE_D;
                 auto kern = reduce_buckets_pipe_kernel<TBL, NT, PD>;
                 HIP_TRY(ctx, hipFuncSetAttribute(reinterpret_cast<const void*>(kern), hipFuncAttributeMaxDynamicSharedMemorySize, (int)lds));
@@ -626,6 +630,12 @@
                 HIP_TRY(ctx, hipGetLastError());
                 return IPKGPU_OK;
             }
+        }
+        if (layout == PairLayout::PAIR6) {
+            if constexpr (quad_layout<SIGMA, K>() == PairLayout::PAIR6)
+                return compress ? launch(reduce_buckets_kernel<TBL, NT, true, PairLayout::PAIR6>) : launch(reduce_buckets_kernel<TBL, NT, false, PairLayout::PAIR6>);
+            else
+                return fail(ctx, IPKGPU_ERR_INVALID, "no 6-byte pair layout for this sigma/k");
         }
         return compress ? launch(reduce_buckets_kernel<TBL, NT, true>) : launch(reduce_buckets_kernel<TBL, NT, false>);
     }
@@ -666,6 +676,13 @@
 #define IPK_QONEWIN12 1
 #endif
 template <int SIGMA, int K> constexpr bool quad_onewin() { return K >= 11 && IPK_QONEWIN12 != 0 && quad_rowlane<SIGMA, K>(); }
+#ifndef IPK_PAIR6
+#define IPK_PAIR6 1
+#endif
+template <int SIGMA, int K> constexpr PairLayout quad_layout()
+{
+    return IPK_PAIR6 != 0 && quad_ok<SIGMA, K>() && K <= 10 && !quad_rowlane<SIGMA, K>() ? PairLayout::PAIR6 : PairLayout::PAIR8;
+}
 template <int SIGMA, int K> size_t quad_lds()
 {
     if constexpr (!quad_ok<SIGMA, K>()) return 0;
@@ -678,15 +695,16 @@
     }
 }
 template <int SIGMA, int K, bool COUNT_ONLY = false>
-int launch_quad_pass1(ipkgpu_ctx* ctx, const StreamParams& sp, uint32_t n_wg)
-{
-    if constexpr (!quad_ok<SIGMA, K>()) { (void)sp; (void)n_wg; return fail(ctx, IPKGPU_ERR_INVALID, "quad kernel unsupported for this sigma/k"); }
+int launch_quad_pass1(ipkgpu_ctx* ctx, const StreamParams& sp, uint32_t n_wg, PairLayout layout)
+{
+    if constexpr (!quad_ok<SIGMA, K>()) { (void)sp; (void)n_wg; (void)layout; return fail(ctx, IPKGPU_ERR_INVALID, "quad kernel unsupported for this sigma/k"); }
     else {
+        if (layout != quad_layout<SIGMA, K>()) return fail(ctx, IPKGPU_ERR_INVALID, "the pass' pool layout is not the quad kernel's");
         constexpr int CAP = fast_cap<SIGMA, K>();
         constexpr uint32_t TBL = stream_tbl<SIGMA, K>();
         constexpr int QNW = quad_nw<SIGMA, K>(), QTW = quad_tw<SIGMA, K>();
         const size_t lds = quad_lds<SIGMA, K>();
-        auto kern = score_quad_kernel<SIGMA, K, CAP, QTW, QNW, TBL, COUNT_ONLY, quad_rowlane<SIGMA, K>(), quad_onewin<SIGMA, K>()>;
+        auto kern = score_quad_kernel<SIGMA, K, CAP, QTW, QNW, TBL, COUNT_ONLY, quad_rowlane<SIGMA, K>(), quad_onewin<SIGMA, K>(), quad_layout<SIGMA, K>()>;
         if (lds > 64 * 1024)
             HIP_TRY(ctx, hipFuncSetAttribute(reinterpret_cast<const void*>(kern), hipFuncAttributeMaxDynamicSharedMemorySize, (int)lds));
         hipLaunchKernelGGL(kern, dim3(n_wg), dim3(QNW * 64), lds, ctx->stream, sp);
@@ -841,6 +859,7 @@
     bool quad = false;
     uint32_t quad_nw = NW, quad_tw = TW;
     size_t quad_lds = 0;
+    PairLayout quad_layout = PairLayout::PAIR8;
     uint32_t xp_nb = 0, xp_tbl = 0;
     size_t xp_lds = 0;
 };
@@ -854,6 +873,7 @@
             g.stream_nw = stream_nw<S_, K_>(); g.stream_tw = stream_tw<S_, K_>(); g.stream_lds = stream_lds<S_, K_>();
             g.quad = quad_ok<S_, K_>();
             g.quad_nw = quad_nw<S_, K_>(); g.quad_tw = quad_tw<S_, K_>(); g.quad_lds = quad_lds<S_, K_>();
+            g.quad_layout = quad_layout<S_, K_>();
             return IPKGPU_OK;
         }));
     return with_xp_shape(ctx, sigma, k, lead, [&](auto S_, auto K_, auto KK_) {
@@ -900,6 +920,7 @@
     bool positions = false;
     bool compress = false;
     bool seq = false;
+    PairLayout layout = PairLayout::PAIR8;
     double slot_bytes() const { return positions ? 8.0 : kind == PassKind::xp && compress ? 0.3125 : 4.0; }
 };
 
@@ -915,6 +936,7 @@
         ps.compress = v != 3;
     } else if (g.stream_nb != 0 && g.stream_nb <= 2048 && (v == 0 || v == 2 || v == 5 || v == 6 || v == 7)) {
         ps.kind = v != 2 && g.quad ? PassKind::quad : PassKind::stream;
+        ps.layout = ps.kind == PassKind::quad ? g.quad_layout : PairLayout::PAIR8;
         ps.compress = v == 6 || (v == 0 && g.stream_tbl == 32768u && sigma == 4);
     }
     return ps;
@@ -1268,7 +1290,7 @@
     auto pass1 = [&](const StreamParams& sp, uint32_t n_wg, bool count_only) {
         return with_sigma_k(ctx, pl.sigma, pl.k, [&](auto S_, auto K_) {
             if (!use_quad) return launch_stream_pass1<S_, K_>(ctx, sp, n_wg);
-            return count_only ? launch_quad_pass1<S_, K_, true>(ctx, sp, n_wg) : launch_quad_pass1<S_, K_, false>(ctx, sp, n_wg);
+            return count_only ? launch_quad_pass1<S_, K_, true>(ctx, sp, n_wg, ps.layout) : launch_quad_pass1<S_, K_, false>(ctx, sp, n_wg, ps.layout);
         });
     };
 
@@ -1318,6 +1340,7 @@
     const uint64_t wg_per_cu = std::max<uint64_t>(1, std::min<uint64_t>(32 / SNW, (160 * 1024) / std::max<size_t>(lds_bytes, 1)));
     const uint64_t slots = (uint64_t)ctx->num_cu * wg_per_cu;
     const uint32_t CH = chunk_pairs_rt(TBL);
+    const uint64_t CHB = chunk_bytes_rt(TBL, ps.layout);
     const uint64_t expected_chunks = (uint64_t)((double)windows * ppw_est / CH);
 #ifndef IPK_WG_CHUNKS2
 #define IPK_WG_CHUNKS2 2
@@ -1335,14 +1358,14 @@
     const uint64_t n_gb = (uint64_t)gb * NBK;
 
     const size_t free_b = mem_free_bytes(ctx);
-    uint64_t max_chunks = std::min<uint64_t>(0xFFFFFFF0ull, (uint64_t)(free_b + ctx->pool.cap + ctx->desc.cap) * 9 / 10 / (CH * 8 + 8));
-    if (ctx->opt_pool_limit > 0) max_chunks = std::min<uint64_t>(max_chunks, (uint64_t)ctx->opt_pool_limit / (CH * 8 + 8));
+    uint64_t max_chunks = std::min<uint64_t>(0xFFFFFFF0ull, (uint64_t)(free_b + ctx->pool.cap + ctx->desc.cap) * 9 / 10 / (CHB + 8));
+    if (ctx->opt_pool_limit > 0) max_chunks = std::min<uint64_t>(max_chunks, (uint64_t)ctx->opt_pool_limit / (CHB + 8));
     const double ppw = ctx->pairs_per_window > 0 ? ctx->pairs_per_window : 256.0;
     const uint64_t ovf_waves = (uint64_t)ctx->num_cu * 4 * OVF_NW;
     const uint64_t slack = 2 * (n_waves + ovf_waves) * NBK * SUB + (n_waves + ovf_waves) * ALLOC_BATCH + 1024;
     uint64_t want = (uint64_t)((double)windows * ppw * 1.25 / CH) + slack;
     {
-        const uint64_t have = std::min<uint64_t>(std::max<uint64_t>(ctx->pool.cap / (CH * 8), 1) - 1, ctx->desc.cap / 8);
+        const uint64_t have = std::min<uint64_t>(std::max<uint64_t>(ctx->pool.cap / CHB, 1) - 1, ctx->desc.cap / 8);
         const uint64_t need = (uint64_t)((double)windows * ppw * 1.1 / CH) + (n_waves + ovf_waves) * (NBK * SUB + ALLOC_BATCH) + 1024;
         if (have >= need) want = have;
     }
@@ -1355,9 +1378,9 @@
             if (gb > 1) return IPKGPU_RETRY_SMALLER;
             return fail(ctx, IPKGPU_ERR_NOMEM, "the pair pool of ONE branch group does not fit device memory");
         }
-        RC_TRY(ensure(ctx, ctx->pool, (cap + 1) * CH * 8));
+        RC_TRY(ensure(ctx, ctx->pool, (cap + 1) * CHB));
         RC_TRY(ensure(ctx, ctx->desc, cap * 8));
-        if (!forced) cap = std::min<uint64_t>(ctx->pool.cap / (CH * 8) - 1, ctx->desc.cap / 8);
+        if (!forced) cap = std::min<uint64_t>(ctx->pool.cap / CHB - 1, ctx->desc.cap / 8);
         RC_TRY(ensure(ctx, ctx->gbcnt, 2 * n_gb * 4));
         uint32_t* const d_gbcur = ctx->gbcnt.as<uint32_t>() + n_gb;
         RC_TRY(ensure(ctx, ctx->gboff, (n_gb + 1) * 8));
@@ -1415,7 +1438,11 @@
             StreamParams so = sp;
             so.ovf_queue = ctx->tmp_b.as<unsigned long long>();
             if (use_quad) so.emitted = small_at<unsigned long long>(ctx, SMALL_OVF_EMITTED);
-            RC_TRY(with_sigma_k(ctx, pl.sigma, pl.k, [&](auto S_, auto K_) { return launch_stream_overflow<S_, K_>(ctx, so); }));
+            RC_TRY(with_sigma_k(ctx, pl.sigma, pl.k, [&](auto S_, auto K_) {
+                if constexpr (quad_layout<S_, K_>() == PairLayout::PAIR6) { if (ps.layout == PairLayout::PAIR6) return launch_stream_overflow<S_, K_, PairLayout::PAIR6>(ctx, so); }
+                if (ps.layout != PairLayout::PAIR8) return fail(ctx, IPKGPU_ERR_INVALID, "no big-list kernel for the pass' pool layout");
+                return launch_stream_overflow<S_, K_>(ctx, so);
+            }));
         }
         if (ovf_in_pool) {
             HIP_TRY(ctx, hipMemcpyAsync(ctx->h_rb, ctx->small, SMALL_BYTES, hipMemcpyDeviceToHost, ctx->stream));
@@ -1467,7 +1494,7 @@
         }
         const int ev_c = sw.mark();
         RC_TRY(with_sigma_k(ctx, pl.sigma, pl.k, [&](auto S_, auto K_) {
-            return launch_stream_pass2<S_, K_>(ctx, (uint32_t)n_gb, pl.table_size, ctx->table.as<uint32_t>(), s_compress);
+            return launch_stream_pass2<S_, K_>(ctx, (uint32_t)n_gb, pl.table_size, ctx->table.as<uint32_t>(), s_compress, ps.layout);
         }));
         const int ev_d = sw.mark();
         if ((spec || n_ovf > 0) && !ovf_in_pool)
@@ -2840,6 +2867,7 @@
     if (!strcmp(name, "last_refused_bytes")) { *value = (int64_t)ctx->refused_need; return IPKGPU_OK; }
     if (!strcmp(name, "slice_long_lists")) { *value = ctx->opt_slice; return IPKGPU_OK; }
     if (!strcmp(name, "debug_sliced_windows")) { *value = (int64_t)ctx->sliced_windows; return IPKGPU_OK; }
+    if (!strcmp(name, "debug_pool_bytes")) { *value = (int64_t)ctx->pool.cap; return IPKGPU_OK; }
     return IPKGPU_ERR_INVALID;
 }
 
diff --git a/ipk_amd/csrc/kernels_quad.hpp b/ipk_amd/csrc/kernels_quad.hpp
--- a/ipk_amd/csrc/kernels_quad.hpp
+++ b/ipk_amd/csrc/kernels_quad.hpp
@@ -146,15 +146,47 @@
     return outside;
 }
 
+
+template <uint32_t SLOT_PLANE>
+__device__ __forceinline__ void pool_store6(uint2* wave_base, uint32_t off4, uint32_t off2, uint2 val)
+{
+    static_assert(SLOT_PLANE < 4096, "the slot plane's offset must fit the store's immediate field");
+    asm volatile("global_store_dword %0, %2, %4\n\tglobal_store_short %1, %3, %4 offset:%5"
+                 : : "v"(off4), "v"(off2), "v"(val.y), "v"(val.x), "s"(wave_base), "n"(SLOT_PLANE) : "memory");
+}
+template <int SH>
+__device__ __forceinline__ uint32_t lshl_add(uint32_t x, uint32_t y)
+{
+    uint32_t r;
+    asm("v_lshl_add_u32 %0, %1, %3, %2" : "=v"(r) : "v"(x), "v"(y), "n"(SH));
+    return r;
+}
+template <uint32_t SLOT_PLANE>
+__device__ __forceinline__ uint64_t pool_store_inside6(uint2* wave_base, uint32_t off4, uint32_t off2, uint2 val, uint32_t v, uint64_t pass, uint32_t CH)
+{
+    static_assert(SLOT_PLANE < 4096, "the slot plane's offset must fit the store's immediate field");
+    uint64_t outside;
+    IPK_ASSERT_FULL_EXEC();
+    asm volatile("s_mov_b64 exec, %7\n\t"
+                 "v_cmpx_gt_u32_e32 vcc, %8, %6\n\t"
+                 "global_store_dword %1, %3, %5\n\t"
+                 "global_store_short %2, %4, %5 offset:%9\n\t"
+                 "s_andn2_b64 %0, %7, exec\n\t"
+                 "s_mov_b64 exec, -1"
+                 : "=&s"(outside) : "v"(off4), "v"(off2), "v"(val.y), "v"(val.x), "s"(wave_base), "v"(v), "s"(pass), "s"(CH), "n"(SLOT_PLANE)
+                 : "memory", "vcc");
+    return outside;
+}
+
 constexpr uint32_t QUAD_SPAN_BYTES_LOG2 = 32;
 constexpr uint32_t QUAD_SPAN_TEST = 8;
 
 __device__ __forceinline__ uint32_t div_small(float x_plus_half, float rn) { return (uint32_t)(x_plus_half * rn); }
 
-template <uint32_t NB, uint32_t CH>
+template <uint32_t NB, uint32_t CH, uint32_t PAIR_BYTES = 8u>
 struct RowAppender {
     static constexpr uint32_t NONE = 0xFFFFFFFFu;
-    static constexpr uint32_t CHUNK_BYTES = CH * 8u;
+    static constexpr uint32_t CHUNK_BYTES = CH * PAIR_BYTES;
     static constexpr uint32_t SPAN_CHUNKS = (uint32_t)((1ull << QUAD_SPAN_BYTES_LOG2) / CHUNK_BYTES);
     const StreamParams& p;
     unsigned long long* st;
@@ -172,7 +204,7 @@
         base = p.pool;
         if (pre) {
             base_id = first;
-            const unsigned long long a = (unsigned long long)(p.pool + (size_t)first * CH);
+            const unsigned long long a = (unsigned long long)p.pool + (unsigned long long)first * CHUNK_BYTES;
             base = reinterpret_cast<uint2*>(((unsigned long long)to_sgpr((uint32_t)(a >> 32)) << 32) | to_sgpr((uint32_t)a));
         }
     }
@@ -193,7 +225,7 @@
         }
         wave_lds_sync();
         base_id = nid;
-        const unsigned long long a = (unsigned long long)(p.pool + (size_t)nid * CH);
+        const unsigned long long a = (unsigned long long)p.pool + (unsigned long long)nid * CHUNK_BYTES;
         base = reinterpret_cast<uint2*>(((unsigned long long)to_sgpr((uint32_t)(a >> 32)) << 32) | to_sgpr((uint32_t)a));
     }
     __device__ __forceinline__ uint32_t roll(uint32_t b)
@@ -289,7 +321,8 @@
                  : "+v"(cursor) : "v"(data), "v"(s), "s"(eps) : "vcc");
 }
 
-template <int SIGMA, int K, int CAP, int TW, int NW, uint32_t TBL, bool COUNT_ONLY = false, bool ROWLANE = false, bool ONEWIN = false>
+template <int SIGMA, int K, int CAP, int TW, int NW, uint32_t TBL, bool COUNT_ONLY = false, bool ROWLANE = false, bool ONEWIN = false,
+          PairLayout LAYOUT = PairLayout::PAIR8>
 __global__ __launch_bounds__(NW * 64) void score_quad_kernel(StreamParams p)
 {
     extern __shared__ __align__(16) unsigned char smem[];
@@ -301,6 +334,9 @@
     constexpr uint32_t CH = chunk_pairs<TBL>();
     constexpr uint32_t mulR = Q::mulR;
     static_assert(TBL % mulR == 0, "a row of the final join must stay inside one bucket");
+    using CL = ChunkLayout<TBL, LAYOUT>;
+    static_assert(!ROWLANE || LAYOUT == PairLayout::PAIR8, "the row-per-lane join writes 8-byte pairs");
+    constexpr bool P6 = LAYOUT == PairLayout::PAIR6;
     constexpr uint32_t CAPL = Geo<SIGMA, Q::HL, CAP>::CAPH, CAPR = Geo<SIGMA, Q::HR, CAP>::CAPH;
     constexpr uint32_t WS = quad_wave_entries<SIGMA, K, CAP, ONEWIN>();
     constexpr uint32_t WPW = ONEWIN ? 1u : 2u;
@@ -322,7 +358,7 @@
     uint2* child = scratch_all + (size_t)wave * WS;
     uint2* lp = child + WPW * Q::CW;
     uint2* rp = lp + CAPL;
-    using Appender = std::conditional_t<ROWLANE, LaneAppender<NB, CH>, RowAppender<NB, CH>>;
+    using Appender = std::conditional_t<ROWLANE, LaneAppender<NB, CH>, RowAppender<NB, CH, CL::PAIR_BYTES>>;
     Appender app{p, state_all + (size_t)wave * NB, g};
     app.init(blockIdx.x * NW + wave);
     unsigned long long emitted = 0;
@@ -619,7 +655,10 @@
                             const uint32_t where = (uint32_t)__builtin_amdgcn_ds_bpermute(head_addr, (int)(uint32_t)(got[u] >> 32));
                             v[u] = fill + rank[u];
                             val[u] = make_uint2(a[u].x + b.x, __float_as_uint(s[u]));
-                            ovf[u] = pool_store_inside(app.base, lshl3_add(v[u], where), val[u], v[u], m[u], CH);
+                            if constexpr (P6)
+                                ovf[u] = pool_store_inside6<CL::SLOT_PLANE>(app.base, lshl_add<2>(v[u], where), lshl_add<1>(v[u], where), val[u], v[u], m[u], CH);
+                            else
+                                ovf[u] = pool_store_inside(app.base, lshl3_add(v[u], where), val[u], v[u], m[u], CH);
                             anyo |= ovf[u];
                         }
                         while (anyo) {
@@ -633,7 +672,8 @@
 #pragma unroll
                             for (int u = 0; u < NS; ++u) {
                                 const bool h = ((ovf[u] >> lane) & 1ull) != 0 && bk[u] == bb;
-                                if (h) pool_store(app.base, nwhere + ((v[u] - CH) << 3), val[u]);
+                                if constexpr (P6) { if (h) pool_store6<CL::SLOT_PLANE>(app.base, nwhere + ((v[u] - CH) << 2), nwhere + ((v[u] - CH) << 1), val[u]); }
+                                else if (h) pool_store(app.base, nwhere + ((v[u] - CH) << 3), val[u]);
                                 ovf[u] &= ~ballot64(h);
                                 anyo |= ovf[u];
                             }
diff --git a/ipk_amd/csrc/kernels_score.hpp b/ipk_amd/csrc/kernels_score.hpp
--- a/ipk_amd/csrc/kernels_score.hpp
+++ b/ipk_amd/csrc/kernels_score.hpp
@@ -419,6 +419,18 @@
 #endif
 template <uint32_t TBL> constexpr uint32_t chunk_pairs() { return (TBL == 16384 || TBL == IPK_CH512_TBL) ? 512u : 256u; }
 inline uint32_t chunk_pairs_rt(uint32_t tbl) { return (tbl == 16384 || tbl == IPK_CH512_TBL) ? 512u : 256u; }
+enum class PairLayout : uint32_t { PAIR8 = 0, PAIR6 = 1 };
+template <uint32_t TBL, PairLayout L>
+struct ChunkLayout {
+    static_assert(TBL <= 65536, "a slot of the bucket's table must fit the u16 plane");
+    static_assert(L == PairLayout::PAIR8 || (TBL & (TBL - 1)) == 0, "PAIR6: slot = key mod TBL is taken from the key's low bits");
+    static constexpr uint32_t CH = chunk_pairs<TBL>();
+    static constexpr uint32_t PAIR_BYTES = L == PairLayout::PAIR6 ? 6u : 8u;
+    static constexpr uint32_t BYTES = PAIR_BYTES * CH;
+    static constexpr uint32_t SLOT_PLANE = 4u * CH;
+    static_assert(BYTES % 128 == 0, "chunks start on cache-line boundaries");
+};
+inline uint32_t chunk_bytes_rt(uint32_t tbl, PairLayout l) { return (l == PairLayout::PAIR6 ? 6u : 8u) * chunk_pairs_rt(tbl); }
 constexpr uint32_t CHUNK_NONE = 0xFFFFFFFFu;
 constexpr uint32_t ALLOC_BATCH = 32;
 constexpr uint32_t SUB = 1;
@@ -536,9 +548,10 @@
     return true;
 }
 
-template <uint32_t TBL, uint32_t NB>
+template <uint32_t TBL, uint32_t NB, PairLayout LAYOUT = PairLayout::PAIR8>
 struct Appender {
     static constexpr uint32_t CH = chunk_pairs<TBL>();
+    using CL = ChunkLayout<TBL, LAYOUT>;
     const StreamParams& p;
     uint32_t* cbase;
     uint32_t* cfill;
@@ -566,6 +579,16 @@
         }
         wave_lds_sync();
         return nid;
+    }
+
+    __device__ __forceinline__ void put(uint32_t id, uint32_t slot, uint32_t idx, uint32_t sb)
+    {
+        if constexpr (LAYOUT == PairLayout::PAIR8) p.pool[(size_t)id * CH + slot] = make_uint2(idx, sb);
+        else {
+            unsigned char* c = reinterpret_cast<unsigned char*>(p.pool) + (size_t)id * CL::BYTES;
+            reinterpret_cast<uint32_t*>(c)[slot] = sb;
+            reinterpret_cast<unsigned short*>(c + CL::SLOT_PLANE)[slot] = (unsigned short)idx;
+        }
     }
 
     __device__ __forceinline__ void append2(bool pass0, uint32_t idx0, uint32_t sb0, bool pass1, uint32_t idx1, uint32_t sb1)
@@ -578,8 +601,8 @@
         if (pass0) cb0 = cbase[bk0];
         if (pass1) cb1 = cbase[bk1];
         const bool st = !(p.flags & 1u);
-        if (pass0 && slot0 < CH && cb0 != CHUNK_NONE && st) p.pool[(size_t)cb0 * CH + slot0] = make_uint2(idx0, sb0);
-        if (pass1 && slot1 < CH && cb1 != CHUNK_NONE && st) p.pool[(size_t)cb1 * CH + slot1] = make_uint2(idx1, sb1);
+        if (pass0 && slot0 < CH && cb0 != CHUNK_NONE && st) put(cb0, slot0, idx0, sb0);
+        if (pass1 && slot1 < CH && cb1 != CHUNK_NONE && st) put(cb1, slot1, idx1, sb1);
         const bool o0 = pass0 && slot0 >= CH, o1 = pass1 && slot1 >= CH;
         uint64_t ovf0 = __ballot(o0), ovf1 = __ballot(o1);
         while (ovf0 | ovf1) {
@@ -589,8 +612,8 @@
             const bool h0 = o0 && bk0 == bb, h1 = o1 && bk1 == bb;
             const uint64_t m0 = __ballot(h0), m1 = __ballot(h1);
             const uint32_t nid = roll(bb);
-            if (h0 && nid != CHUNK_NONE && st) p.pool[(size_t)nid * CH + (slot0 - CH)] = make_uint2(idx0, sb0);
-            if (h1 && nid != CHUNK_NONE && st) p.pool[(size_t)nid * CH + (slot1 - CH)] = make_uint2(idx1, sb1);
+            if (h0 && nid != CHUNK_NONE && st) put(nid, slot0 - CH, idx0, sb0);
+            if (h1 && nid != CHUNK_NONE && st) put(nid, slot1 - CH, idx1, sb1);
             ovf0 &= ~m0; ovf1 &= ~m1;
         }
     }
@@ -711,7 +734,7 @@
     if (lane == 0 && emitted) atomicAdd(p.emitted, emitted);
 }
 
-template <int SIGMA, int K, uint32_t TBL>
+template <int SIGMA, int K, uint32_t TBL, PairLayout LAYOUT = PairLayout::PAIR8>
 __global__ __launch_bounds__(OVF_NW * 64) void score_overflow_stream_kernel(StreamParams p)
 {
     extern __shared__ __align__(16) unsigned char smem[];
@@ -730,7 +753,7 @@
     uint32_t* cbase = state_all + (size_t)wave * 2 * NB * SUB;
     uint32_t* cfill = cbase + NB * SUB;
     for (uint32_t b = lane; b < NB * SUB; b += 64) { cbase[b] = CHUNK_NONE; cfill[b] = CH; }
-    Appender<TBL, NB> app{p, cbase, cfill, 0u};
+    Appender<TBL, NB, LAYOUT> app{p, cbase, cfill, 0u};
     bool have_group = false;
     unsigned long long emitted = 0;
     constexpr uint32_t mulR = ipow(SIGMA, K - K / 2);
@@ -1001,7 +1024,7 @@
 #endif
 }
 
-template <uint32_t TBL, int NT, bool COMPRESS = false>
+template <uint32_t TBL, int NT, bool COMPRESS = false, PairLayout LAYOUT = PairLayout::PAIR8>
 __global__ __launch_bounds__(NT) void reduce_buckets_kernel(const uint2* __restrict__ pool,
                                                            const uint64_t* __restrict__ off, const uint2* __restrict__ list,
                                                            uint32_t NB, uint64_t T, uint32_t* __restrict__ table,
@@ -1029,6 +1052,45 @@
     for (uint32_t i = threadIdx.x; i < CLR / 4; i += NT) reinterpret_cast<uint4*>(tab)[i] = make_uint4(0, 0, 0, 0);
     __syncthreads();
     const uint32_t k0 = (uint32_t)key0;
+    if constexpr (LAYOUT == PairLayout::PAIR6) {
+        using CL = ChunkLayout<TBL, LAYOUT>;
+        static_assert(CH % 256 == 0, "PAIR6 reduce: four pairs per lane and load");
+        static_assert(IPK_RB_NT == 0 && IPK_RB_ABL == 0, "the non-temporal and ablation knobs exist for the PAIR8 loads only: a tuning build must not measure PAIR6 by them");
+        constexpr int Q = CH / 256;
+        const unsigned char* bytes = reinterpret_cast<const unsigned char*>(pool);
+        while (ci < c1) {
+            uint4 sc[CPT * Q]; uint2 sl[CPT * Q];
+            uint32_t n[CPT];
+#pragma unroll
+            for (int c = 0; c < CPT; ++c) {
+                n[c] = (ci + (uint64_t)c * NWV < c1) ? e[c].y : 0u;
+                const unsigned char* s = bytes + (size_t)e[c].x * CL::BYTES;
+#pragma unroll
+                for (int j = 0; j < Q; ++j) {
+                    const uint32_t q = lane + 64 * j;
+                    sc[c * Q + j] = make_uint4(0, 0, 0, 0); sl[c * Q + j] = make_uint2(0, 0);
+                    if (4 * q < n[c]) {
+                        sc[c * Q + j] = reinterpret_cast<const uint4*>(s)[q];
+                        sl[c * Q + j] = reinterpret_cast<const uint2*>(s + CL::SLOT_PLANE)[q];
+                    }
+                }
+            }
+            ci += (uint64_t)CPT * NWV;
+#pragma unroll
+            for (int c = 0; c < CPT; ++c) if (ci + (uint64_t)c * NWV < c1) e[c] = list[ci + (uint64_t)c * NWV];
+#pragma unroll
+            for (int c = 0; c < CPT; ++c)
+#pragma unroll
+                for (int j = 0; j < Q; ++j) {
+                    const uint32_t i0 = 4 * (lane + 64 * j);
+                    const uint4 s4 = sc[c * Q + j]; const uint2 k4 = sl[c * Q + j];
+                    if (i0 + 0 < n[c]) atomicMax(&tab[k4.x & (TBL - 1)], enc_score_bits(s4.x));
+                    if (i0 + 1 < n[c]) atomicMax(&tab[(k4.x >> 16) & (TBL - 1)], enc_score_bits(s4.y));
+                    if (i0 + 2 < n[c]) atomicMax(&tab[k4.y & (TBL - 1)], enc_score_bits(s4.z));
+                    if (i0 + 3 < n[c]) atomicMax(&tab[(k4.y >> 16) & (TBL - 1)], enc_score_bits(s4.w));
+                }
+        }
+    } else
     while (ci < c1) {
         constexpr int PER = CH / 64;
         uint2 v[CPT * PER];
```
